# babybirdprd/dia-tts-prune

Hardware: AMD Instinct MI355X
Metric: audio-codec frames/sec (Dia-1.6B decode, whole job) (higher is better)
Workload: dtype bf16; 1 GPU; Dia-1.6B bf16 weights, bf16 K/V, batch 1, 1890 decode steps, text bytes [98], cfg 3.0 / T 1.3 / top-p 0.95 / top-k 35, hipGraph=True; batch_per_gpu=1, parallelism=single

## Files before the change

dia-tts-prune_amd/csrc/attn.hip:

```cpp
#include "common.hpp"
#include "../../include/dia_hip.h"
#include "errors.hpp"
#include "launch.hpp"
#include "tuning.hpp"
#include <cstdlib>

namespace {

constexpr int HD = 128;
constexpr int NT = 256;
constexpr int NWV = NT / 64;
constexpr int U = 4;
constexpr int UNIT = NWV * 16;
constexpr int CHUNK = 128;
constexpr int SLAB = 2 * 8 + 4 * HD;

struct AttnK {
  int mode, n_kv_heads, n_rows, kv_cap;
  const float* q; int ldq, q_off, k_off, v_off;
  void* kc; void* vc;
  const int* cur; const int* len; int enc_len;
  const float* cos_t; const float* sin_t;
  bf16_raw* P; long p_plane_stride; int p_ktiles;
  float* scratch; int* tickets; int max_chunks;
  const int* head_map;
  int v_blocked;
  int gpw;
  int act_f32;
  long kv_plane_stride;
};

#ifdef DIA_DBG_STAMPS
__device__ long long g_astamps[8192 * 8];
#define ASTAMP(i) do { if (threadIdx.x == 0) g_astamps[((blockIdx.z * gridDim.y + blockIdx.y) * gridDim.x + blockIdx.x) * 8 + (i)] = wall_clock64(); } while (0)
#else
#define ASTAMP(i) do {} while (0)
#endif

template <int G>
__device__ __forceinline__ void attn_finish(const AttnK& p, const float* part, const float* pm_s, const float* pl_s,
                                            int* last_s_ptr, int tid, int qrow, int kvh, int head_row, int chunk, int nchunks) {
  int& last_s = *last_s_ptr;
  const bool o_thread = tid < G * 16;
  const int og = tid >> 4, od0 = (tid & 15) * 8;
  float o[8];
  float M = 0.f, Lsum = 1.f;
  if (o_thread) {
    float mm = -INFINITY;
#pragma unroll
    for (int ww = 0; ww < NWV; ++ww) mm = fmaxf(mm, pm_s[ww * 8 + og]);
    float L2 = 0.f;
#pragma unroll
    for (int j = 0; j < 8; ++j) o[j] = 0.f;
#pragma unroll
    for (int ww = 0; ww < NWV; ++ww) {
      const float pmw = pm_s[ww * 8 + og];
      const float f = (pmw == -INFINITY) ? 0.f : expf(pmw - mm);
      L2 += pl_s[ww * 8 + og] * f;
#pragma unroll
      for (int j = 0; j < 8; ++j) o[j] += part[(ww * G + og) * HD + od0 + j] * f;
    }
    M = mm; Lsum = L2;
  }

  if (nchunks > 1) {
    const long pair = (long)head_row * p.n_kv_heads + kvh;
    float* slab = p.scratch + (pair * p.max_chunks + chunk) * SLAB;
    if (o_thread) {
      if ((tid & 15) == 0) st2_agent(slab + 2 * og, M, Lsum);
      const __amdgpu_buffer_rsrc_t sr = agent_rsrc(p.scratch);
      const int so = (int)(((pair * p.max_chunks + chunk) * SLAB + 16 + og * HD + od0) * 4);
      st4_agent(sr, so, f32x4{o[0], o[1], o[2], o[3]});
      st4_agent(sr, so + 16, f32x4{o[4], o[5], o[6], o[7]});
    }
    asm volatile("s_waitcnt vmcnt(0)" ::: "memory");
    __syncthreads();
    if (tid == 0) {
      const int ticket = __hip_atomic_fetch_add(p.tickets + pair, 1, __ATOMIC_RELAXED, __HIP_MEMORY_SCOPE_AGENT);
      const int last = ticket == nchunks - 1;
      if (last) __hip_atomic_store(p.tickets + pair, 0, __ATOMIC_RELAXED, __HIP_MEMORY_SCOPE_AGENT);
      last_s = last;
    }
    __syncthreads();
    ASTAMP(5);
    if (!last_s) return;
    if (o_thread) {
      const float* base = p.scratch + pair * p.max_chunks * SLAB;
      const __amdgpu_buffer_rsrc_t sr = agent_rsrc(p.scratch);
      const int bo = (int)((pair * p.max_chunks * SLAB + 16 + og * HD + od0) * 4);
      constexpr int MB = 12;
      float mrun = -INFINITY, L2 = 0.f;
#pragma unroll
      for (int j = 0; j < 8; ++j) o[j] = 0.f;
      for (int c0 = 0; c0 < nchunks; c0 += MB) {
        float2 ml[MB]; f32x4 oa[MB], ob[MB];
#pragma unroll
        for (int u = 0; u < MB; ++u)
          if (c0 + u < nchunks) {
            const float* sl = base + (long)(c0 + u) * SLAB;
            ml[u] = ld2_agent(sl + 2 * og);
            oa[u] = ld4_agent(sr, bo + (c0 + u) * (SLAB * 4));
            ob[u] = ld4_agent(sr, bo + (c0 + u) * (SLAB * 4) + 16);
          }
        float mm = mrun;
#pragma unroll
        for (int u = 0; u < MB; ++u)
          if (c0 + u < nchunks) mm = fmaxf(mm, ml[u].x);
        const float fr = (mrun == -INFINITY) ? 0.f : expf(mrun - mm);
        L2 *= fr;
#pragma unroll
        for (int j = 0; j < 8; ++j) o[j] *= fr;
#pragma unroll
        for (int u = 0; u < MB; ++u)
          if (c0 + u < nchunks) {
            const float f = (ml[u].x != -INFINITY) ? expf(ml[u].x - mm) : 0.f;
            L2 += ml[u].y * f;
#pragma unroll
            for (int j = 0; j < 4; ++j) { o[j] += oa[u][j] * f; o[4 + j] += ob[u][j] * f; }
          }
        mrun = mm;
      }
      Lsum = L2;
    }
  }

  if (o_thread) {
    const float invl = Lsum > 0.f ? 1.0f / Lsum : 0.f;
#pragma unroll
    for (int j = 0; j < 8; ++j) o[j] *= invl;
    const int hpos = p.head_map ? p.head_map[kvh * G + og] : kvh * G + og;
    const int col = hpos * HD + od0;
    auto emit = [&](int row, const float* v8) {
      if (p.act_f32) emit_f32x8(reinterpret_cast<float*>(p.P), p.p_ktiles, row, col, v8);
      else emit_planes8(p.P, p.p_plane_stride, p.p_ktiles, row, col, v8);
    };
    if (hpos >= 0) emit(qrow, o);
    if (p.mode == DIA_ATTN_CROSS && hpos >= 0) {
      const float z[8] = {0.f, 0.f, 0.f, 0.f, 0.f, 0.f, 0.f, 0.f};
      emit(qrow - 1, z);
    }
  }
  ASTAMP(6);
}

template <typename KVT, int G>
__global__ __launch_bounds__(NT) void k_attn(AttnK p) {
  __shared__ __attribute__((aligned(16))) float q_s[G * HD];
  __shared__ float part[NWV * G * HD];
  __shared__ float pm_s[NWV * 8], pl_s[NWV * 8];
  __shared__ float knew_s[HD], vnew_s[HD];
  __shared__ int last_s;

  const int tid = threadIdx.x, lane = tid & 63, w = tid >> 6;
  const int kvh = blockIdx.x, chunk = blockIdx.z;
  const int by = blockIdx.y;
  const bool is_self = p.mode == DIA_ATTN_SELF, is_cross = p.mode == DIA_ATTN_CROSS;
  const int c_cur = p.cur[is_self ? (by >> 1) : (is_cross ? by : 0)];
  const int c_len = p.len[is_cross ? by : 0];
  const int qrow = is_cross ? 2 * by + 1 : by;
  const int kvrow = (is_self || is_cross) ? by : 0;
  const int pos = (is_self || is_cross) ? c_cur : by;
  const int nkeys = is_self ? c_cur : (is_cross ? c_len : p.enc_len);
  const int slot = is_self ? c_cur - 1 : -1;
  const int head_row = by;
  const int NZ = gridDim.z;
  const int nunits = max(1, (nkeys + UNIT - 1) / UNIT);
  if (chunk >= nunits) return;
  const int nchunks = min(NZ, nunits);
  if (p.head_map) {
    bool any_live = false;
#pragma unroll
    for (int g = 0; g < G; ++g) any_live |= p.head_map[kvh * G + g] >= 0;
    if (!any_live && !(p.mode == DIA_ATTN_SELF)) return;
  }

  KVT* Kc = reinterpret_cast<KVT*>(p.kc) + ((long)kvrow * p.n_kv_heads + kvh) * p.kv_cap * HD;
  KVT* Vc = reinterpret_cast<KVT*>(p.vc) + ((long)kvrow * p.n_kv_heads + kvh) * p.kv_cap * HD;
  const int gr = lane >> 4, sub = lane & 15;
  const int klast = max(nkeys - 1, 0);
  float kv[U][8], vv[U][8];
  auto load_unit = [&](int unit) {
    const int base = unit * UNIT + w * 16 + gr;
#pragma unroll
    for (int u = 0; u < U; ++u) KVElem<KVT>::load8(Kc + (long)min(base + u * 4, klast) * HD + sub * 8, kv[u]);
#pragma unroll
    for (int u = 0; u < U; ++u) KVElem<KVT>::load8(Vc + (long)min(base + u * 4, klast) * HD + sub * 8, vv[u]);
  };
  load_unit(chunk);

  const float* qr = p.q + (long)qrow * p.ldq;
  for (int t = tid; t < G * 64; t += NT) {
    const int g = t >> 6, d = t & 63;
    const float* qh = qr + p.q_off + (kvh * G + g) * HD;
    const float x1 = qh[d], x2 = qh[d + 64];
    const float c = p.cos_t[(long)pos * 64 + d], s = p.sin_t[(long)pos * 64 + d];
    q_s[g * HD + d] = x1 * c - x2 * s;
// ... 73 lines not shown
#pragma unroll
      for (int u = 0; u < U; ++u) { pu[u] = (sc[u] == -INFINITY) ? 0.f : __expf(sc[u] - mnew); ls += pu[u]; }
      lrun[g] = lrun[g] * alpha + ls;
      mrun[g] = mnew;
#pragma unroll
      for (int j = 0; j < 8; ++j) {
        float a = acc[g][j] * alpha;
#pragma unroll
        for (int u = 0; u < U; ++u) a += pu[u] * vv[u][j];
        acc[g][j] = a;
      }
    }
    if constexpr (PREFETCH) {
      if (nu < nunits) {
#pragma unroll
        for (int u = 0; u < U; ++u)
#pragma unroll
          for (int j = 0; j < 8; ++j) { kv[u][j] = kvn[u][j]; vv[u][j] = vvn[u][j]; }
      }
    }
  }

#pragma unroll
  for (int g = 0; g < G; ++g) {
    float mw = mrun[g];
    mw = fmaxf(mw, __shfl_xor(mw, 16, 64));
    mw = fmaxf(mw, __shfl_xor(mw, 32, 64));
    const float f = (mrun[g] == -INFINITY) ? 0.f : expf(mrun[g] - mw);
    float lw = lrun[g] * f;
    lw += __shfl_xor(lw, 16, 64);
    lw += __shfl_xor(lw, 32, 64);
#pragma unroll
    for (int j = 0; j < 8; ++j) {
      float a = acc[g][j] * f;
      a += __shfl_xor(a, 16, 64);
      a += __shfl_xor(a, 32, 64);
      acc[g][j] = a;
    }
    mrun[g] = mw; lrun[g] = lw;
  }
  if (lane < 16) {
#pragma unroll
    for (int g = 0; g < G; ++g) {
#pragma unroll
      for (int j = 0; j < 8; ++j) part[(w * G + g) * HD + sub * 8 + j] = acc[g][j];
      if (sub == 0) { pm_s[w * 8 + g] = mrun[g]; pl_s[w * 8 + g] = lrun[g]; }
    }
  }
  __syncthreads();

  attn_finish<G>(p, part, pm_s, pl_s, &last_s, tid, qrow, kvh, head_row, chunk, nchunks);
}

__device__ __forceinline__ float row16_max(float v) {
  v = fmaxf(v, __builtin_bit_cast(float, __builtin_amdgcn_update_dpp(0, __builtin_bit_cast(int, v), 0xB1, 0xF, 0xF, true)));
  v = fmaxf(v, __builtin_bit_cast(float, __builtin_amdgcn_update_dpp(0, __builtin_bit_cast(int, v), 0x4E, 0xF, 0xF, true)));
  v = fmaxf(v, __builtin_bit_cast(float, __builtin_amdgcn_update_dpp(0, __builtin_bit_cast(int, v), 0x141, 0xF, 0xF, true)));
  v = fmaxf(v, __builtin_bit_cast(float, __builtin_amdgcn_update_dpp(0, __builtin_bit_cast(int, v), 0x140, 0xF, 0xF, true)));
  return v;
}

#ifdef DIA_DBG_KV_NT
#define KVLOAD(ptr) __builtin_nontemporal_load(ptr)
#else
#define KVLOAD(ptr) (*(ptr))
#endif
template <int G, int PL>
struct MfmaFrag { bf16x8 kb[PL][2][4]; bf16x8 vb[PL][8]; };

template <int G, int PL = 1>
__global__ __launch_bounds__(NT, 2) void k_attn_mfma(AttnK p) {
  __shared__ __attribute__((aligned(16))) bf16_raw qf[4][DIA_NPLANES][G][4][8];
  __shared__ float part[NWV * G * HD];
  __shared__ float pm_s[NWV * 8], pl_s[NWV * 8];
  __shared__ __attribute__((aligned(16))) bf16_raw pbuf[NWV][2][16][32];
  __shared__ __attribute__((aligned(16))) bf16_raw knew_s[PL][HD], vnew_s[PL][HD];
  __shared__ int last_s;

  const int tid = threadIdx.x, lane = tid & 63, w = tid >> 6;
  const int kvh = blockIdx.x, chunk = blockIdx.z;
  const int arow = lane & 15, akq = lane >> 4;
  ASTAMP(0);
  const int by = blockIdx.y;
  const bool is_self = p.mode == DIA_ATTN_SELF;
  const int qrow = is_self ? by : 2 * by + 1;
  const float* qr = p.q + (long)qrow * p.ldq;
  const float* qh = qr + p.q_off + (kvh * G + min(w, G - 1)) * HD;
  const float* kh = qr + (is_self ? p.k_off : p.q_off) + kvh * HD;
  const float* vh = qr + (is_self ? p.v_off : p.q_off) + kvh * HD;
  const float qx1 = qh[lane], qx2 = qh[lane + 64];
  const float kx1 = kh[lane], kx2 = kh[lane + 64];
  const float vx1 = vh[lane], vx2 = vh[lane + 64];

  const int c_cur = p.cur[is_self ? (by >> 1) : by];
  const int c_len = p.len[is_self ? 0 : by];
  const int kvrow = by, pos = c_cur;
  const int nkeys = is_self ? c_cur : c_len;
  const int slot = is_self ? c_cur - 1 : -1;
  const int head_row = by;
  const int NZ = gridDim.z;
  const int ngran = (nkeys + 31) >> 5;
  const int gpw = (ngran <= 2 * NWV) ? max(p.gpw, 2) : p.gpw;
  const int nchunks = min(NZ, max(1, (ngran + NWV * gpw - 1) / (NWV * gpw)));
  if (chunk >= nchunks) return;
  ASTAMP(1);
  if (p.head_map) {
    bool any_live = false;
#pragma unroll
    for (int g = 0; g < G; ++g) any_live |= p.head_map[kvh * G + g] >= 0;
    if (!any_live && !is_self) return;
  }
  const float rc = p.cos_t[(long)pos * 64 + lane], rs = p.sin_t[(long)pos * 64 + lane];

  bf16_raw* Kc = reinterpret_cast<bf16_raw*>(p.kc) + ((long)kvrow * p.n_kv_heads + kvh) * p.kv_cap * HD;
  bf16_raw* Vc = reinterpret_cast<bf16_raw*>(p.vc) + ((long)kvrow * p.n_kv_heads + kvh) * p.kv_cap * HD;
  const int klast = max(nkeys - 1, 0);
  const int gstride = NWV * nchunks;
  const int g_first = chunk * NWV + w;
  auto load_gran = [&](MfmaFrag<G, PL>& f, int gi) {
    const int key0 = gi << 5;
#pragma unroll
    for (int pl = 0; pl < PL; ++pl) {
      const bf16_raw* Kp = Kc + pl * p.kv_plane_stride;
#pragma unroll
      for (int t = 0; t < 2; ++t)
#pragma unroll
        for (int ks = 0; ks < 4; ++ks)
          f.kb[pl][t][ks] = KVLOAD(reinterpret_cast<const bf16x8*>(Kp + (long)min(key0 + 16 * t + arow, klast) * HD + 32 * ks + 8 * akq));
    }
#pragma unroll
    for (int pl = 0; pl < PL; ++pl) {
      const bf16_raw* Vblk = Vc + pl * p.kv_plane_stride + (long)gi * HD * 32;
#pragma unroll
      for (int nb = 0; nb < 8; ++nb) f.vb[pl][nb] = KVLOAD(reinterpret_cast<const bf16x8*>(Vblk + (long)(16 * nb + arow) * 32 + 8 * akq));
    }
  };
  MfmaFrag<G, PL> fa, fb;
  const bool have0 = g_first < ngran;
  load_gran(fa, have0 ? g_first : 0);

  if (w < G) {
    const float qv[2] = {qx1 * rc - qx2 * rs, qx1 * rs + qx2 * rc};
#pragma unroll
    for (int e = 0; e < 2; ++e) {
      const int D = lane + 64 * e;
      __bf16 a, b, c;
      split3(qv[e], a, b, c);
      qf[D >> 5][0][w][(D >> 3) & 3][D & 7] = *reinterpret_cast<const bf16_raw*>(&a);
      qf[D >> 5][1][w][(D >> 3) & 3][D & 7] = *reinterpret_cast<const bf16_raw*>(&b);
      qf[D >> 5][2][w][(D >> 3) & 3][D & 7] = *reinterpret_cast<const bf16_raw*>(&c);
    }
  }
  const int gslot = slot >> 5;
  const bool owner = slot >= 0 && (gslot % gstride) == g_first;
  if (owner) {
    float kv4[4] = {kx1 * rc - kx2 * rs, kx1 * rs + kx2 * rc, vx1, vx2};
#pragma unroll
    for (int pl = 0; pl < PL; ++pl) {
      bf16_raw r4[4];
#pragma unroll
      for (int e = 0; e < 4; ++e) {
        const __bf16 b = (__bf16)kv4[e];
        r4[e] = *reinterpret_cast<const bf16_raw*>(&b);
        kv4[e] -= (float)b;
      }
      knew_s[pl][lane] = r4[0]; knew_s[pl][lane + 64] = r4[1]; vnew_s[pl][lane] = r4[2]; vnew_s[pl][lane + 64] = r4[3];
      bf16_raw* Kp = Kc + pl * p.kv_plane_stride;
      Kp[(long)slot * HD + lane] = r4[0]; Kp[(long)slot * HD + lane + 64] = r4[1];
      bf16_raw* vdst = Vc + pl * p.kv_plane_stride + (long)gslot * HD * 32 + (slot & 31);
      vdst[(long)lane * 32] = r4[2]; vdst[(long)(lane + 64) * 32] = r4[3];
    }
  }
  lds_barrier();
  ASTAMP(2);

  const int qrow_l = min(arow, G - 1);
  const float scale = 0.08838834764831845f;
  f32x4 O[8];
#pragma unroll
  for (int nb = 0; nb < 8; ++nb) O[nb] = f32x4{0.f, 0.f, 0.f, 0.f};
  float mrun[4], lrun[4];
#pragma unroll
  for (int g = 0; g < 4; ++g) { mrun[g] = -INFINITY; lrun[g] = 0.f; }

  auto consume = [&](MfmaFrag<G, PL>& f, int gi) {
    const int key0 = gi << 5;
    if (owner && gi == gslot) {
      const int ts = (slot >> 4) & 1, ns = slot & 15, js = slot & 7, kqs = (slot & 31) >> 3;
#pragma unroll
      for (int pl = 0; pl < PL; ++pl) {
#pragma unroll
        for (int ks = 0; ks < 4; ++ks) {
          const bf16x8 kn = *reinterpret_cast<const bf16x8*>(&knew_s[pl][32 * ks + 8 * akq]);
#pragma unroll
          for (int t = 0; t < 2; ++t)
            if (t == ts && arow == ns) f.kb[pl][t][ks] = kn;
        }
#pragma unroll
        for (int nb = 0; nb < 8; ++nb) {
          const bf16_raw vr = vnew_s[pl][16 * nb + arow];
          const __bf16 vn = *reinterpret_cast<const __bf16*>(&vr);
#pragma unroll
          for (int j = 0; j < 8; ++j)
            if (j == js && akq == kqs) f.vb[pl][nb][j] = vn;
        }
      }
    }
    f32x4 S[2] = {f32x4{0.f, 0.f, 0.f, 0.f}, f32x4{0.f, 0.f, 0.f, 0.f}};
#pragma unroll
    for (int ks = 0; ks < 4; ++ks)
#pragma unroll
      for (int pl = 0; pl < DIA_NPLANES; ++pl) {
        const bf16x8 qa = *reinterpret_cast<const bf16x8*>(&qf[ks][pl][qrow_l][akq][0]);
#pragma unroll
        for (int kp = 0; kp < PL; ++kp) {
          if (PL == 2 && (pl + kp > 1)) continue;
#pragma unroll
          for (int t = 0; t < 2; ++t)
            S[t] = __builtin_amdgcn_mfma_f32_16x16x32_bf16(qa, f.kb[kp][t][ks], S[t], 0, 0, 0);
        }
      }
    float alpha[4];
    const bool v0 = key0 + arow < nkeys, v1 = key0 + 16 + arow < nkeys;
#pragma unroll
    for (int g = 0; g < G; ++g) {
      const float s0 = v0 ? S[0][g] * scale : -INFINITY, s1 = v1 ? S[1][g] * scale : -INFINITY;
      const float mnew = fmaxf(mrun[g], row16_max(fmaxf(s0, s1)));
      alpha[g] = (mrun[g] == -INFINITY) ? 0.f : __expf(mrun[g] - mnew);
      const float p0 = (s0 == -INFINITY) ? 0.f : __expf(s0 - mnew), p1 = (s1 == -INFINITY) ? 0.f : __expf(s1 - mnew);
      lrun[g] = lrun[g] * alpha[g] + row16_sum(p0 + p1);
      mrun[g] = mnew;
      if (lane < 16) {
        const __bf16 h0 = (__bf16)p0, h1 = (__bf16)p1;
        const __bf16 l0 = (__bf16)(p0 - (float)h0), l1 = (__bf16)(p1 - (float)h1);
        pbuf[w][0][g][lane] = *reinterpret_cast<const bf16_raw*>(&h0);
        pbuf[w][0][g][16 + lane] = *reinterpret_cast<const bf16_raw*>(&h1);
        pbuf[w][1][g][lane] = *reinterpret_cast<const bf16_raw*>(&l0);
        pbuf[w][1][g][16 + lane] = *reinterpret_cast<const bf16_raw*>(&l1);
      }
    }
    __builtin_amdgcn_wave_barrier();
#pragma unroll
    for (int nb = 0; nb < 8; ++nb)
#pragma unroll
      for (int g = 0; g < G; ++g) O[nb][g] *= alpha[g];
    const bf16x8 pa0 = *reinterpret_cast<const bf16x8*>(&pbuf[w][0][arow][8 * akq]);
    const bf16x8 pa1 = *reinterpret_cast<const bf16x8*>(&pbuf[w][1][arow][8 * akq]);
#pragma unroll
    for (int nb = 0; nb < 8; ++nb)
#pragma unroll
      for (int vp = 0; vp < PL; ++vp) {
        O[nb] = __builtin_amdgcn_mfma_f32_16x16x32_bf16(pa0, f.vb[vp][nb], O[nb], 0, 0, 0);
        if (vp == 0) O[nb] = __builtin_amdgcn_mfma_f32_16x16x32_bf16(pa1, f.vb[vp][nb], O[nb], 0, 0, 0);
      }
    __builtin_amdgcn_wave_barrier();
  };

  if constexpr (PL == 1) {
    int gi = g_first;
    for (; gi + 2 * gstride < ngran; gi += 2 * gstride) {
      load_gran(fb, gi + gstride);
      consume(fa, gi);
      load_gran(fa, gi + 2 * gstride);
      consume(fb, gi + gstride);
    }
    if (gi < ngran) {
      const int g1 = gi + gstride;
      if (g1 < ngran) load_gran(fb, g1);
      consume(fa, gi);
      if (g1 < ngran) consume(fb, g1);
    }
  } else {
    for (int gi = g_first; gi < ngran; gi += gstride) {
      if (gi != g_first) load_gran(fa, gi);
      consume(fa, gi);
    }
  }
  ASTAMP(3);
  if (lane < 16) {
#pragma unroll
    for (int g = 0; g < G; ++g) {
#pragma unroll
      for (int nb = 0; nb < 8; ++nb) part[(w * G + g) * HD + 16 * nb + lane] = O[nb][g];
      if (lane == 0) { pm_s[w * 8 + g] = mrun[g]; pl_s[w * 8 + g] = lrun[g]; }
    }
  }
  __syncthreads();
  ASTAMP(4);
  attn_finish<G>(p, part, pm_s, pl_s, &last_s, tid, qrow, kvh, head_row, chunk, nchunks);
}

struct EncAttnK {
  const float* qkv; int ldq, q_off, k_off, v_off, heads, rows;
  const int* row_b; const int* seg_off; const int* seg_len;
  const float* cos_t; const float* sin_t;
  bf16_raw* kp; bf16_raw* vp;
  bf16_raw* P; long p_plane_stride; int p_ktiles;
};

__global__ __launch_bounds__(256) void k_enc_kv_planes(EncAttnK p) {
  const int h = blockIdx.x, blk = blockIdx.y, tid = threadIdx.x;
  const long plane = (long)p.heads * p.rows * HD;
  bf16_raw* kp = p.kp + ((long)h * p.rows + blk * 32) * HD;
  bf16_raw* vp = p.vp + ((long)h * (p.rows >> 5) + blk) * HD * 32;
  const int r = tid >> 3, d0 = (tid & 7) * 8, m = blk * 32 + r;
  const float* kr = p.qkv + (long)m * p.ldq + p.k_off + h * HD + d0;
  const float4 xa0 = *reinterpret_cast<const float4*>(kr), xa1 = *reinterpret_cast<const float4*>(kr + 4);
  const float4 xb0 = *reinterpret_cast<const float4*>(kr + 64), xb1 = *reinterpret_cast<const float4*>(kr + 68);
  float vv[2][8];
  int4 vb[2][2];
#pragma unroll
  for (int j = 0; j < 2; ++j) {
    const int it = tid + 256 * j, d = it >> 2, r0 = (it & 3) * 8;
    const float* vr = p.qkv + (long)(blk * 32 + r0) * p.ldq + p.v_off + h * HD + d;
#pragma unroll
    for (int e = 0; e < 8; ++e) vv[j][e] = vr[(long)e * p.ldq];
    vb[j][0] = *reinterpret_cast<const int4*>(p.row_b + blk * 32 + r0);
    vb[j][1] = *reinterpret_cast<const int4*>(p.row_b + blk * 32 + r0 + 4);
  }
  const int b = p.row_b[m];
  const int pos = b >= 0 ? m - p.seg_off[b] : 0;
  const float* ct = p.cos_t + (long)pos * 64 + d0;
  const float* st = p.sin_t + (long)pos * 64 + d0;
  const float4 c0 = *reinterpret_cast<const float4*>(ct), c1 = *reinterpret_cast<const float4*>(ct + 4);
  const float4 s0 = *reinterpret_cast<const float4*>(st), s1 = *reinterpret_cast<const float4*>(st + 4);
  {
    const float x1[8] = {xa0.x, xa0.y, xa0.z, xa0.w, xa1.x, xa1.y, xa1.z, xa1.w};
    const float x2[8] = {xb0.x, xb0.y, xb0.z, xb0.w, xb1.x, xb1.y, xb1.z, xb1.w};
    const float c[8] = {c0.x, c0.y, c0.z, c0.w, c1.x, c1.y, c1.z, c1.w};
    const float s[8] = {s0.x, s0.y, s0.z, s0.w, s1.x, s1.y, s1.z, s1.w};
    bf16x8 k1[3], k2[3];
#pragma unroll
    for (int e = 0; e < 8; ++e) {
      const float a1 = b >= 0 ? x1[e] * c[e] - x2[e] * s[e] : 0.f;
      const float a2 = b >= 0 ? x1[e] * s[e] + x2[e] * c[e] : 0.f;
      __bf16 u0, u1, u2;
      split3(a1, u0, u1, u2); k1[0][e] = u0; k1[1][e] = u1; k1[2][e] = u2;
      split3(a2, u0, u1, u2); k2[0][e] = u0; k2[1][e] = u1; k2[2][e] = u2;
    }
#pragma unroll
    for (int pl = 0; pl < 3; ++pl) {
      *reinterpret_cast<bf16x8*>(kp + pl * plane + (long)r * HD + d0) = k1[pl];
      *reinterpret_cast<bf16x8*>(kp + pl * plane + (long)r * HD + d0 + 64) = k2[pl];
// ... 163 lines not shown
  ko[d + 64] = x1 * s + x2 * c;
  vo[d] = vr[d];
  vo[d + 64] = vr[d + 64];
}

template <typename KVT, int G>
int launch_attn(const AttnK& k, int grid_y, int grid_z, hipStream_t st) {
  dia_launch<k_attn<KVT, G>>(dim3(k.n_kv_heads, grid_y, grid_z), dim3(NT), 0, st, k);
  return dia_check_launch("k_attn");
}

template <int G>
int launch_attn_mfma(const AttnK& k, int grid_y, int grid_z, hipStream_t st) {
  if (k.kv_plane_stride > 0) dia_launch<k_attn_mfma<G, 2>>(dim3(k.n_kv_heads, grid_y, grid_z), dim3(NT), 0, st, k);
  else dia_launch<k_attn_mfma<G, 1>>(dim3(k.n_kv_heads, grid_y, grid_z), dim3(NT), 0, st, k);
  return dia_check_launch("k_attn_mfma");
}

}

#ifdef DIA_DBG_STAMPS
extern "C" int dia_dbg_aclear() {
  static long long zeros[8192 * 8];
  return hipMemcpyToSymbol(HIP_SYMBOL(g_astamps), zeros, sizeof(zeros)) == hipSuccess ? 0 : -2;
}
extern "C" int dia_dbg_astamps(long long* host, int n) {
  return hipMemcpyFromSymbol(host, HIP_SYMBOL(g_astamps), sizeof(long long) * n) == hipSuccess ? 0 : -2;
}
#endif

extern "C" int dia_attn_scratch_floats(int n_rows, int n_kv_heads, int kv_cap) {
  const long chunks = (kv_cap + CHUNK - 1) / CHUNK;
  const long n = (long)n_rows * n_kv_heads * chunks * SLAB;
  return n > 0x7fffffffL ? -1 : (int)n;
}

extern "C" int dia_attn(const dia_attn_args* a, void* stream) {
  if (!a || !a->q || !a->kc || !a->vc || !a->P || !a->cos_t || !a->sin_t) return dia_fail(DIA_E_ARG, "dia_attn: null argument");
  if (a->n_rows <= 0 || a->n_kv_heads <= 0) return dia_fail(DIA_E_ARG, "dia_attn: empty problem");
  if (a->p_plane_stride % 8 != 0) return dia_fail(DIA_E_ARG, "dia_attn: plane stride must be a multiple of 8");
  if (a->mode == DIA_ATTN_ENC && (a->n_rows != a->enc_len || a->enc_len <= 0 || a->enc_len > a->kv_cap))
    return dia_fail(DIA_E_ARG, "dia_attn: ENC needs n_rows == enc_len and 0 < enc_len <= kv_cap");
  if (a->rope_rows > 0 && ((a->mode == DIA_ATTN_ENC && a->enc_len > a->rope_rows) || (a->mode == DIA_ATTN_SELF && a->kv_cap + 1 > a->rope_rows)))
    return dia_fail(DIA_E_ARG, "dia_attn: RoPE tables shorter than the positions this launch can reach");
  if (a->kv_cap <= 0) return dia_fail(DIA_E_ARG, "dia_attn: kv_cap must be positive");
  const int cap_keys = a->mode == DIA_ATTN_ENC ? a->enc_len : a->kv_cap;
  const int cap_chunks = (cap_keys + CHUNK - 1) / CHUNK;
  int max_chunks = (512 + a->n_rows * a->n_kv_heads - 1) / (a->n_rows * a->n_kv_heads);
  if (dia_tune(DIA_TUNE_ATTN_NZ) > 0) max_chunks = dia_tune(DIA_TUNE_ATTN_NZ);
  if (max_chunks > cap_chunks) max_chunks = cap_chunks;
  if (max_chunks < 1) max_chunks = 1;
  if (max_chunks > 1 && (!a->scratch || !a->tickets)) return dia_fail(DIA_E_ARG, "dia_attn: more than 128 keys possible: scratch and tickets are required");
  AttnK k;
  k.mode = a->mode; k.n_kv_heads = a->n_kv_heads; k.n_rows = a->n_rows; k.kv_cap = a->kv_cap;
  k.q = a->q; k.ldq = a->ldq; k.q_off = a->q_off; k.k_off = a->k_off; k.v_off = a->v_off;
  k.kc = a->kc; k.vc = a->vc; k.cur = a->cur; k.len = a->len; k.enc_len = a->enc_len;
  k.cos_t = a->cos_t; k.sin_t = a->sin_t;
  k.P = (bf16_raw*)a->P; k.p_plane_stride = a->p_plane_stride; k.p_ktiles = a->p_ktiles; k.act_f32 = a->act_f32;
  k.head_map = a->head_map; k.v_blocked = a->v_blocked;
  k.gpw = 1;
  { const int g = dia_tune(a->mode == DIA_ATTN_CROSS ? DIA_TUNE_ATTN_GPW_CROSS : DIA_TUNE_ATTN_GPW); if (g > 0) k.gpw = g; }
  if (!k.cur) k.cur = reinterpret_cast<const int*>(a->cos_t);
  if (!k.len) k.len = reinterpret_cast<const int*>(a->cos_t);
  k.scratch = a->scratch; k.tickets = a->tickets; k.max_chunks = (a->kv_cap + CHUNK - 1) / CHUNK;
  if ((a->n_kv_heads * a->group * 128 + 31) / 32 > a->p_ktiles) return dia_fail(DIA_E_ARG, "dia_attn: output planes too narrow");
  hipStream_t st = (hipStream_t)stream;
  const bool f32 = a->kv_dtype == DIA_KV_F32;
  k.kv_plane_stride = 0;
  if (a->kv_dtype == DIA_KV_BF16X2) {
    if (!a->v_blocked || a->kv_plane_stride <= 0 || a->kv_plane_stride % 8 != 0)
      return dia_fail(DIA_E_ARG, "dia_attn: two-plane bf16 K/V needs the blocked V layout and the plane stride of the caches");
    k.kv_plane_stride = a->kv_plane_stride;
  }
  if (a->v_blocked) {
    if (f32 || a->mode == DIA_ATTN_ENC || a->kv_cap % 32 != 0) return dia_fail(DIA_E_ARG, "dia_attn: v_blocked needs bf16 K/V, SELF/CROSS mode and kv_cap % 32 == 0");
    if (a->mode == DIA_ATTN_SELF && !a->cur) return dia_fail(DIA_E_ARG, "dia_attn: SELF needs cur");
    if (a->mode == DIA_ATTN_CROSS && (!a->cur || !a->len || a->group != 1)) return dia_fail(DIA_E_ARG, "dia_attn: CROSS needs cur, len and group 1");
    if (a->group == 4) return launch_attn_mfma<4>(k, a->n_rows, max_chunks, st);
    if (a->group == 2) return launch_attn_mfma<2>(k, a->n_rows, max_chunks, st);
    if (a->group == 1) return launch_attn_mfma<1>(k, a->n_rows, max_chunks, st);
    return dia_fail(DIA_E_ARG, "dia_attn: GQA group must be 1, 2 or 4");
  }
  switch (a->mode) {
    case DIA_ATTN_SELF:
      if (!a->cur) return dia_fail(DIA_E_ARG, "dia_attn: SELF needs cur");
      if (a->group == 4) return f32 ? launch_attn<float, 4>(k, a->n_rows, max_chunks, st) : launch_attn<bf16_raw, 4>(k, a->n_rows, max_chunks, st);
      if (a->group == 2) return f32 ? launch_attn<float, 2>(k, a->n_rows, max_chunks, st) : launch_attn<bf16_raw, 2>(k, a->n_rows, max_chunks, st);
      if (a->group == 1) return f32 ? launch_attn<float, 1>(k, a->n_rows, max_chunks, st) : launch_attn<bf16_raw, 1>(k, a->n_rows, max_chunks, st);
      return dia_fail(DIA_E_ARG, "dia_attn: GQA group must be 1, 2 or 4");
    case DIA_ATTN_CROSS:
      if (!a->cur || !a->len || a->group != 1) return dia_fail(DIA_E_ARG, "dia_attn: CROSS needs cur, len and group 1");
      return f32 ? launch_attn<float, 1>(k, a->n_rows, max_chunks, st) : launch_attn<bf16_raw, 1>(k, a->n_rows, max_chunks, st);
    case DIA_ATTN_ENC:
      if (a->group != 1 || a->enc_len <= 0 || a->enc_len > a->kv_cap || !f32) return dia_fail(DIA_E_ARG, "dia_attn: ENC needs group 1, fp32 scratch K/V, 0 < L <= cap");
      return launch_attn<float, 1>(k, a->n_rows, max_chunks, st);
    default:
      return dia_fail(DIA_E_ARG, "dia_attn: unknown mode");
  }
}

extern "C" int dia_enc_kv_prep(const float* qkv, int ldq, int k_off, int v_off, int heads, int L, int cap,
                               const float* cos_t, const float* sin_t, float* kc, float* vc, void* stream) {
  if (!qkv || !kc || !vc || !cos_t || !sin_t || heads <= 0 || L <= 0 || L > cap) return dia_fail(DIA_E_ARG, "dia_enc_kv_prep: bad argument");
  dia_launch<k_enc_kv_prep>(dim3(heads, L), dim3(64), 0, (hipStream_t)stream, qkv, ldq, k_off, v_off, heads, L, cap, cos_t, sin_t, kc, vc);
  return dia_check_launch("k_enc_kv_prep");
}

extern "C" int dia_enc_attn(const dia_enc_attn_args* a, void* stream) {
  if (!a || !a->qkv || !a->row_b || !a->seg_off || !a->seg_len || !a->cos_t || !a->sin_t || !a->kp || !a->vp || !a->P)
    return dia_fail(DIA_E_ARG, "dia_enc_attn: null argument");
  if (a->heads <= 0 || a->rows <= 0 || a->rows % 32 != 0) return dia_fail(DIA_E_ARG, "dia_enc_attn: rows must be a positive multiple of 32");
  if (a->p_plane_stride % 8 != 0 || (a->heads * 128 + 31) / 32 > a->p_ktiles) return dia_fail(DIA_E_ARG, "dia_enc_attn: output planes too narrow");
  if (a->ldq % 4 != 0 || a->k_off % 4 != 0 || a->v_off % 4 != 0 || ((uintptr_t)a->qkv & 15) || ((uintptr_t)a->row_b & 15) || ((uintptr_t)a->kp & 15) ||
      ((uintptr_t)a->vp & 15) || ((uintptr_t)a->cos_t & 15) || ((uintptr_t)a->sin_t & 15))
    return dia_fail(DIA_E_ARG, "dia_enc_attn: qkv / row_b / kp / vp / RoPE tables must be 16-byte aligned, ldq and the k / v offsets multiples of 4");
  EncAttnK k;
  k.qkv = a->qkv; k.ldq = a->ldq; k.q_off = a->q_off; k.k_off = a->k_off; k.v_off = a->v_off; k.heads = a->heads; k.rows = a->rows;
// ... 10 lines not shown
```

dia-tts-prune_amd/csrc/engine.hip:

```cpp
#include "common.hpp"
#include "../../include/dia_hip.h"
#include "errors.hpp"
#include "launch.hpp"
#include "tuning.hpp"
#include <cstdlib>
#include <vector>
#include <algorithm>
#include <utility>

struct dia_engine {
  dia_engine_desc d;
  std::vector<dia_dec_layer> layers;
  hipStream_t stream = nullptr;
  hipGraph_t graph = nullptr;
  hipGraphExec_t exec = nullptr;
  int launches = 0;
  bool seg = false;
  std::vector<const void*> seg_w;
  int mlp_fused = -1;
  std::vector<hipEvent_t> prof;
  int pf_lookahead = 0;
  bool pf_capturing = false;
  hipStream_t side = nullptr;
  std::vector<hipEvent_t> pf_ev;
  std::vector<std::pair<const void*, long>> pf_w;
};

int dia_prefetch_launch(const void* ptr, long nbytes, int nblocks, hipStream_t st);
static int ensure_sink();

static inline void mark(dia_engine* e, int i) {
  if (!e->prof.empty() && i + 1 < (int)e->prof.size()) (void)hipEventRecord(e->prof[i + 1], e->stream);
  if (e->pf_capturing) {
    const int j = i + e->pf_lookahead;
    if (j < (int)e->pf_w.size() && e->pf_w[j].first != nullptr) {
      (void)hipEventRecord(e->pf_ev[i], e->stream);
      (void)hipStreamWaitEvent(e->side, e->pf_ev[i], 0);
      const long bytes = e->pf_w[j].second;
      const int nb = (int)std::min<long>(512, std::max<long>(32, bytes / (256 * 16 * 8)));
      (void)dia_prefetch_launch(e->pf_w[j].first, bytes, nb, e->side);
    }
  }
}

constexpr int MXFP8_DEFAULT = 0x5070;
extern "C" int dia_mxfp8_classes(int rows) {
  if (rows <= 0 || rows > 16) return 0;
  const int knob = dia_tune(DIA_TUNE_MXFP8);
  const int mask = knob >= 0 ? knob : MXFP8_DEFAULT;
  return (rows <= 4 ? mask : mask >> 8) & 0x7f;
}

static int enqueue_step(dia_engine* e, bool with_sampler) {
  const dia_engine_desc& d = e->d;
  void* st = (void*)e->stream;
  const int R = 2 * d.B;
  const int xkt = d.D / 32;
  const int akt = (max(d.q_heads, d.cq_heads) * 128) / 32;
  const int hkt = d.F / 32;
  const long mt = d.rows_pad / 16;
  const long xs = mt * xkt * 512, as = mt * akt * 512, hs = mt * hkt * 512;
  const int nqkv = (d.q_heads + 2 * d.kv_heads) * 128;
  int n = 0, rc;
  const int F = d.act_f32 ? 1 : 0;
  const bool two_tiles = R > 16 && R <= 32 && d.sk_scratch && d.sk_tickets && d.sk_scratch_floats > 0;
  auto lend_scratch = [&](dia_gemm_args& g) {
    if (two_tiles) { g.sk_scratch = d.sk_scratch; g.sk_tickets = d.sk_tickets; g.sk_scratch_floats = d.sk_scratch_floats; }
  };

  const bool seg = e->seg;
  bool diag = (R <= 2 || (R <= 4 && d.F <= 4096)) && d.act_f32 && d.w_planes <= 1 && dia_tune(DIA_TUNE_WO_DIAG) == 1 && !seg;
  for (int l = 0; l < d.n_layer && diag; ++l) diag = e->layers[l].w_wo_diag != nullptr && e->layers[l].cmap_next == nullptr;
// ... 16 lines not shown
    g.W = wf8; g.w_format = DIA_W_MXFP8; g.nw = 0; g.spw = 0;
    g.sk = sk;
    if (sk == 1) { g.sk_scratch = nullptr; g.sk_tickets = nullptr; }
    else { g.sk_scratch = d.sk_scratch; g.sk_tickets = d.sk_tickets; }
  };
  for (int l = 0; l < d.n_layer; ++l) {
    const dia_dec_layer& L = e->layers[l];
    dia_gemm_args g = {};
    if (!seg || l == 0) {
    g.A = d.planes_x; g.a_plane_stride = xs; g.a_ktiles = xkt; g.M = R;
    g.W = L.w_qkv; g.KT = L.kt_qkv; g.nstrips = L.ns_qkv; g.epi = DIA_EPI_SCALE_STORE;
    g.ssq_in = d.ssq; g.ssq_in_n = l > 0 ? xn_wo : d.D / 16; g.ssq_ld = d.rows_pad; g.inv_d = 1.0f / d.D; g.eps = d.eps;
    g.out = d.qkv; g.ldo = nqkv; g.strip_map = L.smap_qkv;
    lend_scratch(g);
  g.act_f32 = F;
  g.w_planes = d.w_planes;
  sparse24(g, L.w_qkv_24);
  mxfp8(g, L.w_qkv_f8, 0);
  if ((rc = dia_gemm(&g, st))) return rc; mark(e, n++);
    }

    dia_attn_args a = {};
    a.mode = DIA_ATTN_SELF; a.kv_dtype = d.kv_dtype; a.n_kv_heads = d.kv_heads; a.group = d.q_heads / d.kv_heads;
    a.n_rows = R; a.kv_cap = d.T; a.q = d.qkv; a.ldq = nqkv; a.q_off = 0; a.k_off = d.q_heads * 128;
    a.v_off = (d.q_heads + d.kv_heads) * 128; a.kc = L.k_self; a.vc = L.v_self; a.cur = d.sample.cur;
    a.head_map = L.hmap_self; a.v_blocked = d.v_blocked; a.rope_rows = d.T + 1; a.kv_plane_stride = d.kv_plane_self;
    a.cos_t = d.cos_t; a.sin_t = d.sin_t; a.P = d.planes_a; a.p_plane_stride = as; a.p_ktiles = akt;
    a.scratch = d.attn_scratch; a.tickets = d.attn_tickets;
    a.act_f32 = F;
    if ((rc = dia_attn(&a, st))) return rc; mark(e, n++);

    g = {};
    g.A = d.planes_a; g.a_plane_stride = as; g.a_ktiles = akt; g.M = R;
    g.W = L.w_o; g.KT = L.kt_o; g.nstrips = L.ns_o; g.epi = DIA_EPI_RESID_EMIT;
    g.ssq_ld = d.rows_pad; g.out = d.x; g.ldo = d.D; g.gnext = L.g_ca; g.cmap = L.cmap_ca;
    g.P = d.planes_x; g.p_plane_stride = xs; g.p_ktiles = xkt; g.ssq_out = d.ssq;
    lend_scratch(g);
  g.act_f32 = 3 * F;
  g.w_planes = d.w_planes;
  sparse24(g, L.w_o_24);
  mxfp8(g, L.w_o_f8, 1);
  if ((rc = dia_gemm(&g, st))) return rc; mark(e, n++);

    g = {};
    g.A = d.planes_x; g.a_plane_stride = xs; g.a_ktiles = xkt; g.M = R;
    g.W = L.w_cq; g.KT = L.kt_cq; g.nstrips = L.ns_cq; g.epi = DIA_EPI_SCALE_STORE;
    g.ssq_in = d.ssq; g.ssq_in_n = d.D / 16; g.ssq_ld = d.rows_pad; g.inv_d = 1.0f / d.D; g.eps = d.eps;
    g.out = d.qc; g.ldo = d.cq_heads * 128; g.strip_map = L.smap_cq;
    lend_scratch(g);
  g.act_f32 = F;
  g.w_planes = d.w_planes;
  sparse24(g, L.w_cq_24);
  mxfp8(g, L.w_cq_f8, 2);
  if ((rc = dia_gemm(&g, st))) return rc; mark(e, n++);

    a = {};
    a.mode = DIA_ATTN_CROSS; a.kv_dtype = d.kv_dtype; a.n_kv_heads = d.cq_heads; a.group = 1;
    a.n_rows = d.B; a.kv_cap = d.S; a.q = d.qc; a.ldq = d.cq_heads * 128; a.q_off = 0;
    a.kc = L.k_cross; a.vc = L.v_cross; a.cur = d.sample.cur; a.len = d.text_len; a.head_map = L.hmap_cross; a.v_blocked = d.v_blocked;
    a.kv_plane_stride = d.kv_plane_cross;
    a.cos_t = d.cos_t; a.sin_t = d.sin_t; a.P = d.planes_a; a.p_plane_stride = as; a.p_ktiles = akt;
    a.scratch = d.attn_scratch; a.tickets = d.attn_tickets;
    a.act_f32 = F;
    if ((rc = dia_attn(&a, st))) return rc; mark(e, n++);

    if (seg) {
      dia_seg_args sa = {};
      sa.a_in = (const float*)d.planes_a; sa.a_ktiles = akt; sa.M = R; sa.W = e->seg_w[l];
      sa.has_qkv = l + 1 < d.n_layer; sa.nslots = dia_seg_slots(sa.has_qkv); sa.D = d.D; sa.F = d.F;
      sa.x = d.x; sa.ldx = d.D; sa.g_mlp = L.g_mlp; sa.g_next = (l + 1 < d.n_layer) ? e->layers[l + 1].g_sa : d.g_final;
      sa.qkv_out = d.qkv; sa.ldq = nqkv; sa.planes_x = (float*)d.planes_x; sa.xkt = xkt; sa.ssq = d.ssq; sa.ssq_ld = d.rows_pad;
      sa.eps = d.eps; sa.ws = d.seg_ws;
      if ((rc = dia_seg_mlp(&sa, st))) return rc; mark(e, n++);
      continue;
    }
    g = {};
    g.A = d.planes_a; g.a_plane_stride = as; g.a_ktiles = akt; g.M = R;
    g.W = L.w_co; g.KT = L.kt_co; g.nstrips = L.ns_co; g.epi = DIA_EPI_RESID_EMIT;
    g.ssq_ld = d.rows_pad; g.out = d.x; g.ldo = d.D; g.gnext = L.g_mlp; g.cmap = L.cmap_mlp;
    g.P = d.planes_x; g.p_plane_stride = xs; g.p_ktiles = xkt; g.ssq_out = d.ssq;
    lend_scratch(g);
  g.act_f32 = 3 * F;
  g.w_planes = d.w_planes;
  sparse24(g, L.w_co_24);
  mxfp8(g, L.w_co_f8, 3);
  if ((rc = dia_gemm(&g, st))) return rc; mark(e, n++);

    dia_gemm_args gi = {};
    gi.A = d.planes_x; gi.a_plane_stride = xs; gi.a_ktiles = xkt; gi.M = R;
    gi.W = L.w_wi; gi.KT = L.kt_wi; gi.nstrips = L.ns_wi; gi.epi = DIA_EPI_SWIGLU_EMIT;
    gi.ssq_in = d.ssq; gi.ssq_in_n = d.D / 16; gi.ssq_ld = d.rows_pad; gi.inv_d = 1.0f / d.D; gi.eps = d.eps;
    gi.P = d.planes_h; gi.p_plane_stride = hs; gi.p_ktiles = hkt;

    g = {};
    g.A = d.planes_h; g.a_plane_stride = hs; g.a_ktiles = hkt; g.M = R;
    g.W = L.w_wo; g.KT = L.kt_wo; g.nstrips = L.ns_wo; g.epi = DIA_EPI_RESID_EMIT;
    int wo_sk = (R <= 4 && L.kt_wo % 2 == 0) ? 2 : ((R <= 16 && L.kt_wo % 4 == 0) ? 4 : 1);
    int wo_spw = 0;
    if (R > 4 && R <= 16) {
      if (L.kt_wo % 64 == 0 && L.kt_wo / 64 >= 2 && L.kt_wo / 64 <= 8) wo_sk = L.kt_wo / 64;
      if (wo_sk > 1 && L.ns_wo * wo_sk >= 512 && L.ns_wo % 2 == 0) wo_spw = 2;
    }
    const int w2_sk = (d.w_planes == 2 && L.kt_wo % 128 == 0 && L.kt_wo / 128 <= 8) ? L.kt_wo / 128 : 1;
    if (d.w_planes == 2) { wo_sk = w2_sk; wo_spw = 0; }
    if (dia_tune(DIA_TUNE_WO_SK) >= 1 && dia_tune(DIA_TUNE_WO_SK) <= 8 && L.kt_wo % dia_tune(DIA_TUNE_WO_SK) == 0) wo_sk = dia_tune(DIA_TUNE_WO_SK);
    g.sk = wo_sk; g.sk_scratch = wo_sk > 1 ? d.sk_scratch : nullptr; g.sk_tickets = wo_sk > 1 ? d.sk_tickets : nullptr;
    bool wo_pair = false;
    if (R > 16 && R <= 128) {
      g.sk_scratch = d.sk_scratch; g.sk_tickets = d.sk_tickets;
      g.sk_scratch_floats = d.sk_scratch_floats > 0 ? d.sk_scratch_floats : (int64_t)(d.D / 16) * 4 * 512;
      wo_pair = L.kt_wo % 4 == 0 && g.sk_scratch_floats >= (int64_t)((R + 15) / 16) * L.ns_wo * 4 * 256 &&
                dia_tune(DIA_TUNE_WO_PAIR) != 0;
      g.sk = wo_pair ? 4 : 1;
      if (d.w_planes == 2) {
        wo_pair = w2_sk > 1 && g.sk_scratch_floats >= (int64_t)((R + 15) / 16) * L.ns_wo * w2_sk * 256;
        g.sk = wo_pair ? w2_sk : 1;
      }
// ... 38 lines not shown
  g.W = d.w_logits; g.KT = d.kt_logits; g.nstrips = d.ns_logits; g.epi = DIA_EPI_SCALE_STORE;
  g.ssq_in = d.ssq; g.ssq_in_n = xn_wo; g.ssq_ld = d.rows_pad; g.inv_d = 1.0f / d.D; g.eps = d.eps;
  g.out = d.logits; g.ldo = d.ld_logits;
  lend_scratch(g);
  g.act_f32 = F;
  g.w_planes = d.w_planes;
  sparse24(g, d.w_logits_24);
  mxfp8(g, d.w_logits_f8, 6);
  if ((rc = dia_gemm(&g, st))) return rc; mark(e, n++);
  if (with_sampler) {
    if ((rc = dia_sample(&d.sample, st))) return rc; mark(e, n++);
  }
  e->launches = n;
  return DIA_OK;
}

extern "C" int dia_engine_create(const dia_engine_desc* d, void* stream, dia_engine** out) {
  if (!d || !out || !d->layers) return dia_fail(DIA_E_ARG, "dia_engine_create: null argument");
  if (d->n_layer <= 0 || d->B <= 0) return dia_fail(DIA_E_ARG, "dia_engine_create: empty model");
  if (d->D % 32 != 0 || d->F % 32 != 0) return dia_fail(DIA_E_ARG, "dia_engine_create: D and F must be multiples of 32");
  if (d->rows_pad < 2 * d->B || d->rows_pad % 16 != 0) return dia_fail(DIA_E_ARG, "dia_engine_create: rows_pad must be 16*ceil(2B/16)");
  if (d->q_heads % d->kv_heads != 0) return dia_fail(DIA_E_ARG, "dia_engine_create: q_heads % kv_heads != 0");
  if (d->act_f32 && !d->sample.embed.act_f32)
    return dia_fail(DIA_E_ARG, "dia_engine_create: act_f32 needs an embedding that writes fp32 tiles too");
  if (!d->act_f32 && d->sample.embed.act_f32) return dia_fail(DIA_E_ARG, "dia_engine_create: the embedding writes fp32 tiles but the engine reads planes");
  if (!d->x || !d->planes_x || !d->planes_a || !d->planes_h || !d->ssq || !d->qkv || !d->qc || !d->logits || !d->cos_t ||
      !d->sin_t || !d->text_len || !d->w_logits || !d->g_final || !d->attn_scratch || !d->attn_tickets)
    return dia_fail(DIA_E_ARG, "dia_engine_create: missing buffer");
  dia_engine* e = new dia_engine();
  e->d = *d;
  e->layers.assign(d->layers, d->layers + d->n_layer);
  e->d.layers = e->layers.data();
  e->stream = (hipStream_t)stream;
  if (d->seg_w && d->seg_ws) {
    const int nqkv = (d->q_heads + 2 * d->kv_heads) * 128;
    if (2 * d->B > 4 || !d->act_f32 || d->w_planes > 1 || !dia_seg_supported(d->D, d->F, max(d->q_heads, d->cq_heads) * 128, nqkv) ||
        d->cq_heads * 128 != 2048) {
      delete e;
      return dia_fail(DIA_E_ARG, "dia_engine_create: persistent segments need <= 4 rows, fp32 activation tiles, one weight plane, Dia-1.6B decoder shapes and 256 CUs");
    }
    for (int l = 0; l < d->n_layer; ++l) {
      const dia_dec_layer& L = d->layers[l];
      if (!d->seg_w[l] || L.cmap_mlp || L.cmap_next || L.smap_qkv) { delete e; return dia_fail(DIA_E_ARG, "dia_engine_create: persistent segments take dense (uncompacted) layers only"); }
    }
    e->seg_w.assign(d->seg_w, d->seg_w + d->n_layer);
    e->d.seg_w = e->seg_w.data();
    e->seg = true;
  }
  e->mlp_fused = dia_tune(DIA_TUNE_MLP_FUSE) > 0 ? -1 : 0;
  *out = e;
  return DIA_OK;
}

extern "C" int dia_engine_destroy(dia_engine* e) {
  if (!e) return DIA_OK;
  hipError_t he = hipSuccess;
  if (e->stream) he = hipStreamSynchronize(e->stream);
  if (e->side) { hipError_t h2 = hipStreamSynchronize(e->side); if (he == hipSuccess) he = h2; }
  if (e->exec) (void)hipGraphExecDestroy(e->exec);
  if (e->graph) (void)hipGraphDestroy(e->graph);
  for (auto& ev : e->pf_ev) if (ev) (void)hipEventDestroy(ev);
  for (auto& ev : e->prof) if (ev) (void)hipEventDestroy(ev);
  if (e->side) (void)hipStreamDestroy(e->side);
  delete e;
  return he == hipSuccess ? DIA_OK : dia_fail_hip(he, "dia_engine_destroy: hipStreamSynchronize");
}

extern "C" int dia_engine_decode(dia_engine* e, int n_steps, int use_graph) {
  if (!e || n_steps < 0) return dia_fail(DIA_E_ARG, "dia_engine_decode: bad argument");
  if (!use_graph) {
    for (int i = 0; i < n_steps; ++i) {
      int rc = enqueue_step(e, true);
      if (rc) return rc;
    }
    return DIA_OK;
  }
  if (!e->exec) {
    if (e->stream == nullptr) return dia_fail(DIA_E_STATE, "dia_engine_decode: graph capture needs a non-default stream");
    if (e->pf_lookahead > 0) {
      int rc0 = ensure_sink();
      if (rc0) return rc0;
      const dia_engine_desc& d = e->d;
      e->pf_w.clear();
      for (int l = 0; l < d.n_layer; ++l) {
        const dia_dec_layer& L = e->layers[l];
        auto add = [&](const void* w, int kt, int ns) { e->pf_w.push_back({w, (long)kt * ns * 1024}); };
        add(L.w_qkv, L.kt_qkv, L.ns_qkv); e->pf_w.push_back({nullptr, 0});
        add(L.w_o, L.kt_o, L.ns_o); add(L.w_cq, L.kt_cq, L.ns_cq); e->pf_w.push_back({nullptr, 0});
        add(L.w_co, L.kt_co, L.ns_co); add(L.w_wi, L.kt_wi, L.ns_wi); add(L.w_wo, L.kt_wo, L.ns_wo);
      }
      e->pf_w.push_back({d.w_logits, (long)d.kt_logits * d.ns_logits * 1024});
      e->pf_w.push_back({nullptr, 0});
      if (!e->side && hipStreamCreateWithFlags(&e->side, hipStreamNonBlocking) != hipSuccess) return dia_fail(DIA_E_HIP, "hipStreamCreate(side)");
      e->pf_ev.assign(e->pf_w.size() + 2, nullptr);
      for (auto& ev : e->pf_ev)
        if (hipEventCreateWithFlags(&ev, hipEventDisableTiming) != hipSuccess) return dia_fail(DIA_E_HIP, "hipEventCreate(prefetch)");
    }
    hipError_t he = hipStreamBeginCapture(e->stream, hipStreamCaptureModeThreadLocal);
    if (he != hipSuccess) return dia_fail_hip(he, "hipStreamBeginCapture");
    if (e->pf_lookahead > 0) {
      (void)hipEventRecord(e->pf_ev[e->pf_w.size()], e->stream);
      (void)hipStreamWaitEvent(e->side, e->pf_ev[e->pf_w.size()], 0);
      e->pf_capturing = true;
    }
    int rc = enqueue_step(e, true);
    if (e->pf_lookahead > 0) {
      e->pf_capturing = false;
      (void)hipEventRecord(e->pf_ev[e->pf_w.size() + 1], e->side);
      (void)hipStreamWaitEvent(e->stream, e->pf_ev[e->pf_w.size() + 1], 0);
    }
    he = hipStreamEndCapture(e->stream, &e->graph);
    if (rc) return rc;
    if (he != hipSuccess) return dia_fail_hip(he, "hipStreamEndCapture");
    he = hipGraphInstantiate(&e->exec, e->graph, nullptr, nullptr, 0);
    if (he != hipSuccess) return dia_fail_hip(he, "hipGraphInstantiate");
  }
  for (int i = 0; i < n_steps; ++i) {
    hipError_t he = hipGraphLaunch(e->exec, e->stream);
    if (he != hipSuccess) return dia_fail_hip(he, "hipGraphLaunch");
  }
  return DIA_OK;
}

extern "C" int dia_engine_step_logits_only(dia_engine* e) {
  if (!e) return dia_fail(DIA_E_ARG, "dia_engine_step_logits_only: null engine");
  return enqueue_step(e, false);
}

__global__ void k_delay(long long ticks) {
  const long long t0 = wall_clock64();
  while (wall_clock64() - t0 < ticks) __builtin_amdgcn_s_sleep(32);
}

extern "C" int dia_engine_profile_step(dia_engine* e, float* ms, int cap) {
  if (!e || !ms) return dia_fail(DIA_E_ARG, "dia_engine_profile_step: null argument");
  const int n = dia_engine_launches_per_step(e);
  if (cap < n) return dia_fail(DIA_E_ARG, "dia_engine_profile_step: output array too small");
  e->prof.resize(n + 1);
  for (auto& ev : e->prof) {
    hipError_t he = hipEventCreate(&ev);
    if (he != hipSuccess) return dia_fail_hip(he, "hipEventCreate");
  }
  int rc = DIA_OK;
  dia_launch<k_delay>(dim3(1), dim3(64), 0, e->stream, 300000LL );
  (void)hipEventRecord(e->prof[0], e->stream);
  rc = enqueue_step(e, true);
  {
    hipError_t he = hipStreamSynchronize(e->stream);
    if (rc == DIA_OK && he != hipSuccess) rc = dia_fail_hip(he, "hipStreamSynchronize");
  }
  if (rc == DIA_OK)
    for (int i = 0; i < n; ++i)
      if (hipEventElapsedTime(&ms[i], e->prof[i], e->prof[i + 1]) != hipSuccess) { ms[i] = -1.f; (void)hipGetLastError(); }
  for (auto& ev : e->prof) (void)hipEventDestroy(ev);
  e->prof.clear();
  return rc;
}

extern "C" int dia_engine_time_step(dia_engine* e, float* ms, float* interval_ms, int cap) {
  if (!e || !ms) return dia_fail(DIA_E_ARG, "dia_engine_time_step: null argument");
  const int n = dia_engine_launches_per_step(e);
  if (cap < n) return dia_fail(DIA_E_ARG, "dia_engine_time_step: output array too small");
  dia_launch<k_delay>(dim3(1), dim3(64), 0, e->stream, 300000LL );
  dia_recorder_arm();
  int rc = enqueue_step(e, true);
  const int got = dia_recorder_collect(ms, cap, interval_ms);
  hipError_t he = hipStreamSynchronize(e->stream);
  if (rc != DIA_OK) return rc;
  if (he != hipSuccess) return dia_fail_hip(he, "dia_engine_time_step: hipStreamSynchronize");
  return got;
}

extern "C" const char* dia_timed_kernel_name(int i) { return dia_recorder_label(i); }

extern "C" int dia_engine_mlp_fused(const dia_engine* e) { return e && e->mlp_fused == 1; }

extern "C" int dia_engine_launches_per_step(const dia_engine* e) {
  if (!e) return dia_fail(DIA_E_ARG, "null engine");
  return e->seg ? e->d.n_layer * 5 + 3 : e->d.n_layer * 8 + 2;
}

__global__ __launch_bounds__(256) void k_prefetch(const uint4* __restrict__ p, long n16, unsigned* sink) {
  uint4 acc = {0, 0, 0, 0};
  const long stride = (long)gridDim.x * 256;
  long i = (long)blockIdx.x * 256 + threadIdx.x;
  for (; i + 3 * stride < n16; i += 4 * stride) {
    const uint4 a = p[i], b = p[i + stride], c = p[i + 2 * stride], d = p[i + 3 * stride];
    acc.x ^= a.x ^ b.x ^ c.x ^ d.x; acc.y ^= a.y ^ b.y ^ c.y ^ d.y;
    acc.z ^= a.z ^ b.z ^ c.z ^ d.z; acc.w ^= a.w ^ b.w ^ c.w ^ d.w;
  }
  for (; i < n16; i += stride) { const uint4 a = p[i]; acc.x ^= a.x; acc.y ^= a.y; acc.z ^= a.z; acc.w ^= a.w; }
  if ((acc.x ^ acc.y ^ acc.z ^ acc.w) == 0x9E3779B9u && sink) *sink = 1;
}

static unsigned* g_sink = nullptr;
static int ensure_sink() {
  if (!g_sink) {
    hipError_t e = hipMalloc(&g_sink, 4);
    if (e != hipSuccess) return dia_fail_hip(e, "hipMalloc(sink)");
  }
  return DIA_OK;
}

int dia_prefetch_launch(const void* ptr, long nbytes, int nblocks, hipStream_t st) {
  dia_launch<k_prefetch>(dim3(nblocks), dim3(256), 0, st, (const uint4*)ptr, (long)(nbytes / 16), g_sink);
  return dia_check_launch("k_prefetch");
}

extern "C" int dia_prefetch(const void* ptr, int64_t nbytes, int nblocks, void* stream) {
  if (!ptr || nbytes <= 0 || nblocks <= 0) return dia_fail(DIA_E_ARG, "dia_prefetch: bad argument");
  int rc = ensure_sink();
  if (rc) return rc;
  return dia_prefetch_launch(ptr, (long)nbytes, nblocks, (hipStream_t)stream);
}

extern "C" int dia_engine_set_prefetch(dia_engine* e, int lookahead) {
  if (!e || lookahead < 0) return dia_fail(DIA_E_ARG, "dia_engine_set_prefetch: bad argument");
  if (e->exec) return dia_fail(DIA_E_STATE, "dia_engine_set_prefetch: the step graph is already captured");
  e->pf_lookahead = lookahead;
  return DIA_OK;
}
```

dia-tts-prune_amd/csrc/gemm.hip:

```cpp
#include "gemm_common.hpp"
#include "gemm_experiments.hpp"

namespace {

template <int MT, int NW, int KPW>
__global__ __launch_bounds__(NW * 64) void k_gemm(GemmK p) {
  extern __shared__ __attribute__((aligned(16))) unsigned char smem_raw[];
  f32x4* red = reinterpret_cast<f32x4*>(smem_raw);
  float* tile = reinterpret_cast<float*>(smem_raw + sizeof(f32x4) * NW * MT * 64);
  float* inv_s = tile + MT * 16 * 17;

  const int tid = threadIdx.x, lane = tid & 63, w = tid >> 6;
  const int strip = blockIdx.x;
  const int mt0 = blockIdx.y * MT;
  const int kpw = (KPW > 0) ? KPW : (p.KT + NW - 1) / NW;
  const int kt0 = w * kpw;

  f32x4 acc[MT];
  long aoff[MT];
#pragma unroll
  for (int i = 0; i < MT; ++i) {
    acc[i] = f32x4{0.f, 0.f, 0.f, 0.f};
    const int mtile = min(mt0 + i, (p.M - 1) >> 4);
    const int rlast = min(15, p.M - 1 - mtile * 16);
    const int alane = (lane & 48) | min(lane & 15, rlast);
    aoff[i] = ((long)mtile * p.a_ktiles * 64 + alane) * 8;
  }

  const bf16x8* Wt = reinterpret_cast<const bf16x8*>(p.W) + ((long)strip * p.KT) * 64 + lane;
  const bf16x8 zero8 = {0, 0, 0, 0, 0, 0, 0, 0};

  const int e_mt = tid >> 5, e_r = (tid >> 1) & 15, half = tid & 1;
  const int m = (mt0 + e_mt) * 16 + e_r;
  const int n0 = strip * 16 + half * 8;
  const bool e_thread = tid < MT * 32;
  const bool live = e_thread && m < p.M;
  float xpre[8], gpre[8];

  if (p.w_planes > 1) {
    prefetch_epilogue<MT, NW * 64>(p, tid, mt0, m, n0, live, xpre, gpre, inv_s);
    const int kt1 = min(kt0 + kpw, p.KT);
    const int npw = p.w_planes == 2 ? 1 : p.w_planes, ash = p.w_planes == 2 ? 1 : 0;
    for (int pw = 0; pw < npw; ++pw) {
      const bf16x8* Wp = Wt + pw * (p.w_plane_stride / 8);
      for (int kt = kt0; kt < kt1; ++kt) {
        const bf16x8 bb = DIA_WLOAD(Wp + (long)kt * 64);
#pragma unroll
        for (int mt = 0; mt < MT; ++mt) {
          bf16x8 a3[DIA_NPLANES];
          load_afrag3(p, aoff[mt] + (long)(kt >> ash) * 512, a3[0], a3[1], a3[2]);
#pragma unroll
          for (int pl = 0; pl < DIA_NPLANES; ++pl)
            acc[mt] = __builtin_amdgcn_mfma_f32_16x16x32_bf16(a3[pl], bb, acc[mt], 0, 0, 0);
        }
// ... 2 lines not shown
  } else if constexpr (KPW > 0) {
    bf16x8 b[KPW];
#pragma unroll
    for (int i = 0; i < KPW; ++i) b[i] = DIA_WLOAD(Wt + (long)(kt0 + i) * 64);
    __builtin_amdgcn_sched_barrier(0);
    constexpr int AP = (KPW >= 8) ? 1 : ((KPW * MT <= 4) ? KPW : ((4 / MT) > 0 ? (4 / MT) : 1));
    bf16x8 a0[AP][MT][DIA_NPLANES];
#pragma unroll
    for (int i = 0; i < AP; ++i)
#pragma unroll
      for (int mt = 0; mt < MT; ++mt)
        load_afrag3(p, aoff[mt] + (long)(kt0 + i) * 512, a0[i][mt][0], a0[i][mt][1], a0[i][mt][2]);
    prefetch_epilogue<MT, NW * 64>(p, tid, mt0, m, n0, live, xpre, gpre, inv_s);
#pragma unroll
    for (int i = 0; i < KPW; ++i) {
#pragma unroll
      for (int mt = 0; mt < MT; ++mt) {
        bf16x8 a3[DIA_NPLANES];
        if (i < AP) { a3[0] = a0[i < AP ? i : 0][mt][0]; a3[1] = a0[i < AP ? i : 0][mt][1]; a3[2] = a0[i < AP ? i : 0][mt][2]; }
        else load_afrag3(p, aoff[mt] + (long)(kt0 + i) * 512, a3[0], a3[1], a3[2]);
#pragma unroll
        for (int pl = 0; pl < DIA_NPLANES; ++pl)
          acc[mt] = __builtin_amdgcn_mfma_f32_16x16x32_bf16(a3[pl], b[i], acc[mt], 0, 0, 0);
      }
    }
  } else {
    prefetch_epilogue<MT, NW * 64>(p, tid, mt0, m, n0, live, xpre, gpre, inv_s);
    const int kt1 = min(kt0 + kpw, p.KT);
    for (int kt = kt0; kt < kt1; kt += 4) {
      bf16x8 b[4];
#pragma unroll
      for (int i = 0; i < 4; ++i) b[i] = (kt + i < kt1) ? DIA_WLOAD(Wt + (long)(kt + i) * 64) : zero8;
#pragma unroll
      for (int i = 0; i < 4; ++i) {
        if (kt + i < kt1) {
#pragma unroll
          for (int mt = 0; mt < MT; ++mt) {
            bf16x8 a3[DIA_NPLANES];
            load_afrag3(p, aoff[mt] + (long)(kt + i) * 512, a3[0], a3[1], a3[2]);
#pragma unroll
            for (int pl = 0; pl < DIA_NPLANES; ++pl)
              acc[mt] = __builtin_amdgcn_mfma_f32_16x16x32_bf16(a3[pl], b[i], acc[mt], 0, 0, 0);
          }
        }
      }
    }
  }

  reduce_to_tile<MT, NW>(acc, red, tile, tid, lane, w);
  if (!e_thread) return;
  run_epilogue(p, tile + (e_mt * 16 + e_r) * 17, inv_s[e_mt * 16 + e_r], m, n0, half, strip, live, xpre, gpre);
}


template <int NW, int KPW, int RS, bool MULTI, bool AF32 = false, bool PF32 = false, bool W2 = false>
__global__ __launch_bounds__(NW * 64) void k_gemv_small(const bf16_raw* a_A, long a_aps, const bf16_raw* a_W, int a_KT, int a_M, int a_epi,
                                                        int a_nstrips, float* a_out, int a_ldo, const float* a_gnext, GemmK p) {
  p.A = a_A; p.a_plane_stride = a_aps; p.W = a_W; p.KT = a_KT; p.M = a_M; p.epi = a_epi; p.nstrips = a_nstrips;
  p.out = a_out; p.ldo = a_ldo; p.gnext = a_gnext;
  extern __shared__ __attribute__((aligned(16))) unsigned char smem_raw[];
  f32x4* red = reinterpret_cast<f32x4*>(smem_raw);
  float* tile = reinterpret_cast<float*>(smem_raw + sizeof(f32x4) * NW * 64);
  float* inv_s = tile + 16 * 17;
  bf16x8* As = reinterpret_cast<bf16x8*>(smem_raw + sizeof(f32x4) * NW * 64 + sizeof(float) * (16 * 17 + 16));

  const int tid = threadIdx.x, lane = tid & 63, w = tid >> 6;
  const int kt0 = w * KPW;
  const int ktg = blockIdx.y * (NW * KPW);
  constexpr int WS = W2 ? 1 : 0;
  const int ktga = ktg >> WS;
  const int G = gridDim.x;
  const bf16x8* Wl = reinterpret_cast<const bf16x8*>(p.W) + (long)(ktg + kt0) * 64 + lane;
  auto load_strip = [&](bf16x8* b, int strip) {
    const bf16x8* Wt = Wl + (long)strip * p.KT * 64;
#pragma unroll
    for (int i = 0; i < KPW; ++i) b[i] = DIA_WLOAD(Wt + (long)i * 64);
  };
  __shared__ int sk_flag;

  STAMP(0);
  bf16x8 b0[KPW], b1[MULTI ? KPW : 1];
  constexpr int KT = (NW * KPW) >> WS;
  constexpr int KPA = KPW >> WS;
  static_assert(!W2 || KPW % 2 == 0, "two-plane weights: whole activation k-tiles per wave");
  constexpr int NT = NW * 64;
#ifdef DIA_X_WFIRST
  load_strip(b0, blockIdx.x);
  __builtin_amdgcn_sched_barrier(0);
#endif

  constexpr int CH = (3 * KPA * RS + 15) / 16;
  constexpr int nchunks = DIA_NPLANES * KT * 4 * RS;
  constexpr int nentries = KT * 4 * RS;
  constexpr int CE = (KPA * RS + 15) / 16;
  bf16x8 v0[AF32 ? 1 : CH];
  float4 ex[AF32 ? CE : 1], ey[AF32 ? CE : 1];
  if constexpr (AF32) {
    const float* Af = reinterpret_cast<const float*>(p.A);
#pragma unroll
    for (int u = 0; u < CE; ++u) {
      const int c = min(tid + u * NT, nentries - 1);
      const int row = c % RS, kq = (c / RS) & 3, kt = c / (4 * RS);
      const float4* src = reinterpret_cast<const float4*>(Af + ((long)(ktga + kt) * 64 + row + 16 * kq) * 8);
      ex[u] = src[0]; ey[u] = src[1];
    }
  } else {
#pragma unroll
    for (int u = 0; u < CH; ++u) {
      const int c = min(tid + u * NT, nchunks - 1);
      const int row = c % RS, kq = (c / RS) & 3, kt = (c / (4 * RS)) % KT, pl = c / (4 * RS * KT);
      v0[u] = *reinterpret_cast<const bf16x8*>(p.A + pl * p.a_plane_stride + ((long)(ktga + kt) * 64 + row + 16 * kq) * 8);
    }
  }
  const bool has_norm = p.ssq_in != nullptr;
  const int s_row = tid >> 3, s_part = tid & 7;
  const bool s_thread = tid < 128 && has_norm;
  float sq[16];
#pragma unroll
  for (int i = 0; i < 16; ++i) sq[i] = 0.f;
  if (s_thread) {
    const float* sp = p.ssq_in + min(s_row, p.M - 1);
#pragma unroll
    for (int i = 0; i < 16; ++i) sq[i] = sp[(long)min(s_part + 8 * i, p.ssq_in_n - 1) * p.ssq_ld];
  }
  const bool resid = p.epi == DIA_EPI_RESID_EMIT;
  const bool r_thread = tid < 16 * RS;
  float xpre1 = 0.f, gpre1 = 1.f;
  auto load_resid = [&](int strip) {
    const int r_m = tid >> 4, n = strip * 16 + (tid & 15);
    xpre1 = p.out[(long)(r_m < p.M ? r_m : 0) * p.ldo + n];
    gpre1 = p.gnext[n];
  };
  if (resid && r_thread) load_resid(blockIdx.x);
  __builtin_amdgcn_sched_barrier(0);
#ifndef DIA_X_WFIRST
  load_strip(b0, blockIdx.x);
  __builtin_amdgcn_sched_barrier(0);
#endif
  STAMP(1);
  if constexpr (AF32) {
#pragma unroll
    for (int u = 0; u < CE; ++u)
      if (tid + u * NT < nentries) {
        const int c = tid + u * NT;
        bf16x8 h, mi, lo;
        split3x8(ex[u], ey[u], h, mi, lo);
        As[c] = h; As[nentries + c] = mi; As[2 * nentries + c] = lo;
      }
  } else {
#pragma unroll
    for (int u = 0; u < CH; ++u)
      if (tid + u * NT < nchunks) As[tid + u * NT] = v0[u];
  }
  {
    float s0 = 0.f;
#pragma unroll
    for (int i = 0; i < 16; ++i) s0 += (s_part + 8 * i < p.ssq_in_n && s_row < p.M) ? sq[i] : 0.f;
    if (s_thread && s_row < p.M)
      for (int idx = s_part + 128; idx < p.ssq_in_n; idx += 8) s0 += p.ssq_in[(long)idx * p.ssq_ld + s_row];
    s0 += __builtin_bit_cast(float, __builtin_amdgcn_update_dpp(0, __builtin_bit_cast(int, s0), 0xB1, 0xF, 0xF, true));
    s0 += __builtin_bit_cast(float, __builtin_amdgcn_update_dpp(0, __builtin_bit_cast(int, s0), 0x4E, 0xF, 0xF, true));
    s0 += __builtin_bit_cast(float, __builtin_amdgcn_update_dpp(0, __builtin_bit_cast(int, s0), 0x141, 0xF, 0xF, true));
    if (tid < 128 && s_part == 0) inv_s[s_row] = has_norm ? rsqrtf(s0 * p.inv_d + p.eps) : 1.0f;
  }
  lds_barrier();
  STAMP(2);

  const int arow = min(lane & 15, RS - 1), akq = lane >> 4;
  f32x4* red16 = red;
  int sbuf = 0;
  auto body = [&](bf16x8* bc, bf16x8* bn, int strip) {
    const int next = strip + G;
    if constexpr (MULTI) load_strip(bn, DIA_PREFETCH_CLAMP(next, p.nstrips));
#ifdef DIA_PIN_PREFETCH
    if constexpr (MULTI) __builtin_amdgcn_sched_barrier(0);
#endif
    f32x4 acc[1] = {f32x4{0.f, 0.f, 0.f, 0.f}};
#pragma unroll
    for (int i = 0; i < KPW; ++i) {
#pragma unroll
      for (int pl = 0; pl < DIA_NPLANES; ++pl) {
        const bf16x8 a = As[((pl * KT + ((kt0 + i) >> WS)) * 4 + akq) * RS + arow];
        acc[0] = __builtin_amdgcn_mfma_f32_16x16x32_bf16(a, bc[i], acc[0], 0, 0, 0);
      }
    }
    STAMP(3);
    float v = 0.f;
    if (MULTI || gridDim.y == 1) {
      f32x4* rb = red16 + sbuf * (NW * 16);
      sbuf ^= 1;
      if (lane < 16) rb[w * 16 + lane] = acc[0];
      lds_barrier();
      if (r_thread) {
        const float* rf = reinterpret_cast<const float*>(rb) + (tid & 15) * 4 + (tid >> 4);
        v = rf[0];
#pragma unroll
        for (int ww = 1; ww < NW; ++ww) v += rf[ww * 64];
      }
      STAMP(4);
    } else {
      reduce_to_tile<1, NW, true>(acc, red, tile, tid, lane, w);
      STAMP(4);
      if (!splitk_combine(p, tile, strip, tid, &sk_flag)) return;
      if (r_thread) v = tile[(tid >> 4) * 17 + (tid & 15)];
    }
    if (r_thread) {
      run_epilogue_rows<RS, PF32>(p, v, inv_s, tid, strip, xpre1, gpre1);
      if (MULTI && next < p.nstrips && resid) load_resid(next);
    }
  };
  if constexpr (MULTI) {
    int strip = blockIdx.x;
    for (; strip + G < p.nstrips; strip += 2 * G) {
      body(b0, b1, strip);
      body(b1, b0, strip + G);
    }
    if (strip < p.nstrips) body(b0, b1, strip);
  } else {
    body(b0, b1, blockIdx.x);
  }
  STAMP(5);
}


#ifndef DIA_Z_TEMPORAL
#define DIA_Z_TEMPORAL 1
#endif
constexpr bool ZTEMPORAL = DIA_Z_TEMPORAL != 0;
#ifndef DIA_ZR_RING3
#define DIA_ZR_RING3 0
#endif
constexpr size_t g16_smem(int nw) { return sizeof(f32x4) * 2 * nw * 64 + 1536 + sizeof(float) * (2 * 16 * 17 + 16); }
constexpr size_t g16_alds(int nw, int kpw) { return (size_t)2 * nw * kpw * 64 * 16; }
template <int NW, int KPW, bool MULTI, bool MZ = false, bool AF32 = false, bool PF32 = false, bool PAIR = false, bool ALDS = false, bool W2 = false>
__global__ __launch_bounds__(NW * 64) void k_gemm16(const bf16_raw* a_A, long a_aps, const bf16_raw* a_W, int a_KT, int a_M, int a_epi,
                                                    int a_nstrips, float* a_out, int a_ldo, const float* a_gnext, GemmK p) {
  p.A = a_A; p.a_plane_stride = a_aps; p.W = a_W; p.KT = a_KT; p.M = a_M; p.epi = a_epi; p.nstrips = a_nstrips;
  p.out = a_out; p.ldo = a_ldo; p.gnext = a_gnext;
  extern __shared__ __attribute__((aligned(16))) unsigned char smem_raw[];
  f32x4* red = reinterpret_cast<f32x4*>(smem_raw);
  bf16_raw* stg = reinterpret_cast<bf16_raw*>(smem_raw + sizeof(f32x4) * 2 * NW * 64);
  float* tile = reinterpret_cast<float*>(smem_raw + sizeof(f32x4) * 2 * NW * 64 + 1536);
  float* inv_s = tile + 16 * 17;
  constexpr int NT = NW * 64;

  int zrow0 = 0;
  if constexpr (MZ) {
    const int z = blockIdx.z;
    zrow0 = 16 * z;
    p.A += (long)z * p.a_ktiles * 512 * (AF32 ? 2 : 1);
    p.M = min(16, p.M - 16 * z);
    if (p.ssq_in) p.ssq_in += 16 * z;
    if (p.out) p.out += (long)16 * z * p.ldo;
    if (p.P) p.P += (long)z * p.p_ktiles * 512 * (PF32 ? 2 : 1);
    if (p.ssq_out) p.ssq_out += 16 * z;
    if (p.sk_scratch) { p.sk_scratch += (long)z * p.nstrips * gridDim.y * 256; p.sk_tickets += z * p.nstrips; }
  }
  const int tid = threadIdx.x, lane = tid & 63, w = tid >> 6;
  const int kt0 = blockIdx.y * (NW * KPW) + w * KPW;
  constexpr int WS = W2 ? 1 : 0;
  constexpr int KPA = KPW >> WS;
  static_assert(!W2 || KPW % 2 == 0, "two-plane weights: whole activation k-tiles per wave");
  const int kta0 = kt0 >> WS;
  const int G = gridDim.x;
  __shared__ int sk_flag;
  const bf16x8* Wl = reinterpret_cast<const bf16x8*>(p.W) + (long)kt0 * 64 + lane;
  auto load_strip = [&](bf16x8* b, int strip) {
    const bf16x8* Wt = Wl + (long)strip * p.KT * 64;
#pragma unroll
    for (int i = 0; i < KPW; ++i) b[i] = (MZ && ZTEMPORAL) ? *(Wt + (long)i * 64) : DIA_WLOAD(Wt + (long)i * 64);
// ... 1623 lines not shown
        else if (uni && a->epi == DIA_EPI_RESID_EMIT) launch_small_kernel<k_gemm2t<8, true, false, 8, false, DIA_EPI_RESID_EMIT>>(grid, blk, g2t_smem(8), st, k);
        else if (uni && a->epi == DIA_EPI_SWIGLU_EMIT) launch_small_kernel<k_gemm2t<8, true, false, 8, false, DIA_EPI_SWIGLU_EMIT>>(grid, blk, g2t_smem(8), st, k);
        else launch_small_kernel<k_gemm2t<8, true, false>>(grid, blk, g2t_smem(8), st, k);
      } else if (ktw == 64) {
        if (sk > 1 && sk <= 4 && a->epi == DIA_EPI_RESID_EMIT && a->gnext && !a->cmap && dia_tune(DIA_TUNE_GEMM_2T) != 6)
          launch_small_kernel<k_gemm2t<8, false, true, 8, false, -1, true>>(grid, blk, g2t_smem(8, 8, true), st, k);
        else if (sk > 1) launch_small_kernel<k_gemm2t<8, false, true>>(grid, blk, g2t_smem(8), st, k);
        else if (puni && a->epi == DIA_EPI_RESID_EMIT) launch_small_kernel<k_gemm2t<8, false, false, 8, false, DIA_EPI_RESID_EMIT>>(grid, blk, g2t_smem(8), st, k);
        else launch_small_kernel<k_gemm2t<8, false, false>>(grid, blk, g2t_smem(8), st, k);
      } else if (half && a->epi == DIA_EPI_CROSSKV && a->kv_dtype == DIA_KV_BF16 && a->kv_vblocked && !a->strip_map && dia_tune(DIA_TUNE_GEMM_2T) != 4) {
        launch_small_kernel<k_gemm2t<8, false, false, 4, true>>(grid, blk, g2t_smem(8, 4), st, k);
      } else if (half && puni && a->epi == DIA_EPI_SCALE_STORE) {
        launch_small_kernel<k_gemm2t<8, false, false, 4, false, DIA_EPI_SCALE_STORE>>(grid, blk, g2t_smem(8, 4), st, k);
      } else if (half && puni && a->epi == DIA_EPI_SWIGLU_EMIT) {
        launch_small_kernel<k_gemm2t<8, false, false, 4, false, DIA_EPI_SWIGLU_EMIT>>(grid, blk, g2t_smem(8, 4), st, k);
      } else if (half) {
        launch_small_kernel<k_gemm2t<8, false, false, 4>>(grid, blk, g2t_smem(8, 4), st, k);
      } else {
        launch_small_kernel<k_gemm2t<4, false, false>>(grid, blk, g2t_smem(4), st, k);
      }
      return dia_check_launch("k_gemm2t");
    }
  }
  const bool z_epi = fast_epi || a->epi == DIA_EPI_CROSSKV;
  if (mtiles >= 2 && mtiles <= mz_max && z_epi && nw16 && (sk == 1 || a->sk_scratch_floats >= (int64_t)mtiles * a->nstrips * sk * 256)) {
    bool handled = false;
    k.mz = mtiles;
    int rc = launch_g16_any(k, nw16, sk, st, handled);
    k.mz = 0;
    if (handled) return rc;
  }
#ifdef DIA_EXPERIMENTS
  if (mtiles == 2 && !a->act_f32) {
    bool handled = false;
    int rc = dia_exp_gemm_two_mtiles(a, stream, handled);
    if (handled) return rc;
  }
#endif
  if (sk > 1) return dia_fail(DIA_E_ARG, "dia_gemm: no split-K kernel for this shape");
  {
    const int blocks = ((mtiles + GT_MT - 1) / GT_MT) * ((a->nstrips + 15) / 16);
    const int min_blocks = dia_tune(DIA_TUNE_TILE_MIN_BLOCKS) >= 0 ? dia_tune(DIA_TUNE_TILE_MIN_BLOCKS) : 48;
    if (mtiles >= 3 && a->KT % 8 == 0 && blocks >= min_blocks && !a->act_f32) {
#ifdef DIA_EXPERIMENTS
      const int v = dia_tune(DIA_TUNE_TILE_V);
      if (v >= 0 && v <= 2) return dia_exp_tile_variant(a, stream, v);
#endif
      return launch_tile(k, st);
    }
  }
  return launch_generic(k, nw, st);
}

extern "C" int dia_gemm_timed(const dia_gemm_args* a, void* stream, float* ms_out) {
  if (!ms_out) return dia_fail(DIA_E_ARG, "dia_gemm_timed: null output");
  dia_recorder_arm();
  int rc = dia_gemm(a, stream);
  float ms[4] = {0.f, 0.f, 0.f, 0.f};
  const int n = dia_recorder_collect(ms, 4);
  if (rc != DIA_OK) return rc;
  if (n < 1) return n < 0 ? n : dia_fail(DIA_E_STATE, "dia_gemm_timed: nothing was launched");
  *ms_out = ms[0];
  return DIA_OK;
}

#ifndef DIA_EXPERIMENTS
extern "C" int dia_mlp_fused(const dia_gemm_args*, const dia_gemm_args*, int32_t*, void*) {
  return dia_fail(DIA_E_ARG, "dia_mlp_fused: experiment, needs a build with EXPERIMENTS=1");
}
extern "C" int dia_mlp_fused_timed(const dia_gemm_args*, const dia_gemm_args*, int32_t*, void*, float*) {
  return dia_fail(DIA_E_ARG, "dia_mlp_fused_timed: experiment, needs a build with EXPERIMENTS=1");
}
#endif
```

dia-tts-prune_amd/csrc/gemm_common.hpp:

```cpp
#pragma once
#include "common.hpp"
#include <type_traits>
#include "../../include/dia_hip.h"
#include "errors.hpp"
#include <hip/hip_ext.h>
#include <cstdlib>
#include <cstring>
#include "tuning.hpp"
#include "launch.hpp"

namespace {


#ifdef DIA_DBG_PLAIN_LOAD
#define DIA_WLOAD(ptr) (*(ptr))
#else
#define DIA_WLOAD(ptr) __builtin_nontemporal_load(ptr)
#endif

#ifdef DIA_DBG_COND_PREFETCH
#define DIA_PREFETCH_CLAMP(next, n) (next)
#else
#define DIA_PREFETCH_CLAMP(next, n) min((next), (n) - 1)
#endif
// ... 131 lines not shown
    float v[8];
#pragma unroll
    for (int j = 0; j < 8; ++j) {
      float g = trow[j] * inv, u = trow[8 + j] * inv;
      v[j] = (g / (1.0f + expf(-g))) * u;
    }
    emit_act8(p, m, strip * 8, v, nullptr);
  } else {
    if (!live) return;
    if (p.strip_map) strip = p.strip_map[strip];
    long lofs = 0;
    if (p.kv_layer_strips > 0) {
      const int layer = strip / p.kv_layer_strips;
      strip -= layer * p.kv_layer_strips;
      lofs = (long)layer * p.kv_layer_stride;
    }
    int kvb = p.kv_batch_index;
    if (p.row_b) {
      kvb = p.row_b[m];
      if (kvb < 0) return;
      m -= p.seg_off[kvb];
    }
    const int nk = p.kv_heads * 8;
    if (strip < nk) {
      const int head = strip >> 3, i0 = (strip & 7) * 8 + half * 4;
      const long base = lofs + (((long)kvb * p.kv_heads + head) * p.kv_cap + m) * 128;
#pragma unroll
      for (int t = 0; t < 4; ++t) {
        const int i = i0 + t;
        const float x1 = trow[half * 8 + 2 * t] * inv, x2 = trow[half * 8 + 2 * t + 1] * inv;
        const float c = pre_cs ? xpre[t] : p.cos_t[(long)m * 64 + i], s = pre_cs ? gpre[t] : p.sin_t[(long)m * 64 + i];
        kv_store(p.kc, p.kv_dtype, base + i, x1 * c - x2 * s, p.kv_plane_stride);
        kv_store(p.kc, p.kv_dtype, base + i + 64, x1 * s + x2 * c, p.kv_plane_stride);
      }
    } else {
      const int sv = strip - nk, head = sv >> 3, d0 = (sv & 7) * 16 + half * 8;
      if (p.kv_vblocked) {
        const long hb = lofs + ((long)kvb * p.kv_heads + head) * p.kv_cap * 128;
        const long blk = hb + (long)(m >> 5) * 128 * 32 + (m & 31);
#pragma unroll
        for (int j = 0; j < 8; ++j) kv_store(p.vc, p.kv_dtype, blk + (long)(d0 + j) * 32, trow[half * 8 + j] * inv, p.kv_plane_stride);
      } else {
        const long base = lofs + (((long)kvb * p.kv_heads + head) * p.kv_cap + m) * 128 + d0;
#pragma unroll
        for (int j = 0; j < 8; ++j) kv_store(p.vc, p.kv_dtype, base + j, trow[half * 8 + j] * inv, p.kv_plane_stride);
      }
    }
  }
}

#define DIA_ROW_SHR(v, n) __builtin_bit_cast(float, __builtin_amdgcn_update_dpp(0, __builtin_bit_cast(int, (v)), 0x110 + (n), 0xF, 0xF, true))
#define DIA_ROW_SHL(v, n) __builtin_bit_cast(float, __builtin_amdgcn_update_dpp(0, __builtin_bit_cast(int, (v)), 0x100 + (n), 0xF, 0xF, true))

template <int RS, bool PF32 = false>
__device__ __forceinline__ void run_epilogue_rows(const GemmK& p, float v_tile, const float* inv_s, int tid, int strip,
                                                  float xpre1, float gpre1) {
  const int m = tid >> 4, c = tid & 15;
  const bool live = m < p.M;
  if (p.epi == DIA_EPI_RESID_EMIT) {
    const int n = strip * 16 + c;
    const float v = xpre1 + v_tile;
    if (live) p.out[(long)m * p.ldo + n] = v;
    const float sq = mul_rn(v, v);
    float acc = sq;
#pragma unroll
    for (int j = 1; j < 8; ++j) {
      const float t = DIA_ROW_SHR(acc, 1);
      if ((c & 7) == j) acc = add_rn(t, sq);
    }
    const float h0 = DIA_ROW_SHR(acc, 8);
    if (live && c == 15) p.ssq_out[(long)strip * p.ssq_ld + m] = h0 + acc;
    const float vg = mul_rn(v, gpre1);
    int cc = n;
    if (p.cmap) cc = p.cmap[n];
    if (live && cc >= 0) {
      const long off = plane_frag_off(m, cc & ~7, p.p_ktiles) + (cc & 7);
      if constexpr (PF32) {
        reinterpret_cast<float*>(p.P)[off] = vg;
      } else {
        __bf16 a, b, d;
        split3(vg, a, b, d);
        p.P[off] = *reinterpret_cast<bf16_raw*>(&a);
        p.P[p.p_plane_stride + off] = *reinterpret_cast<bf16_raw*>(&b);
        p.P[2 * p.p_plane_stride + off] = *reinterpret_cast<bf16_raw*>(&d);
      }
    }
  } else if (p.epi == DIA_EPI_SWIGLU_EMIT) {
    const float up_raw = DIA_ROW_SHL(v_tile, 8);
    if (!live || c >= 8) return;
    const float inv = inv_s[m];
    const float g = v_tile * inv, u = up_raw * inv;
    const float v = (g / (1.0f + expf(-g))) * u;
    const long off = plane_frag_off(m, strip * 8, p.p_ktiles) + c;
    if constexpr (PF32) {
      reinterpret_cast<float*>(p.P)[off] = v;
    } else {
      __bf16 a, b, d;
      split3(v, a, b, d);
      p.P[off] = *reinterpret_cast<bf16_raw*>(&a);
      p.P[p.p_plane_stride + off] = *reinterpret_cast<bf16_raw*>(&b);
      p.P[2 * p.p_plane_stride + off] = *reinterpret_cast<bf16_raw*>(&d);
    }
  } else {
    if (!live) return;
    const int s_out = p.strip_map ? p.strip_map[strip] : strip;
    p.out[(long)m * p.ldo + s_out * 16 + c] = v_tile * inv_s[m];
  }
}

template <int MT, int NW, bool RAW = false>
__device__ __forceinline__ void reduce_to_tile(const f32x4* acc, f32x4* red, float* tile, int tid, int lane, int w) {
#pragma unroll
  for (int mt = 0; mt < MT; ++mt) red[(w * MT + mt) * 64 + lane] = acc[mt];
  if constexpr (RAW) lds_barrier(); else __syncthreads();
  if (tid < MT * 64) {
    const int mt = tid >> 6;
    f32x4 s = red[(0 * MT + mt) * 64 + lane];
#pragma unroll
    for (int ww = 1; ww < NW; ++ww) {
      f32x4 t = red[(ww * MT + mt) * 64 + lane];
      s[0] += t[0]; s[1] += t[1]; s[2] += t[2]; s[3] += t[3];
    }
    const int col = lane & 15, r0 = (lane >> 4) * 4;
#pragma unroll
    for (int r = 0; r < 4; ++r) tile[(mt * 16 + r0 + r) * 17 + col] = s[r];
  }
  if constexpr (RAW) lds_barrier(); else __syncthreads();
}

__device__ __forceinline__ bool splitk_combine(const GemmK& p, float* tile, int strip, int tid, int* flag_s) {
  const int SK = gridDim.y;
  if (SK == 1) return true;
  const int ks = blockIdx.y;
#ifdef DIA_X_NOHANDOFF
  return ks == SK - 1;
#endif
  const __amdgpu_buffer_rsrc_t sr = agent_rsrc(p.sk_scratch);
  const int row = tid >> 2, c4 = (tid & 3) * 4;
  if (tid < 64) {
    const float* t = tile + row * 17 + c4;
    st4_agent(sr, (int)((((long)strip * SK + ks) * 256 + row * 16 + c4) * 4), f32x4{t[0], t[1], t[2], t[3]});
  }
  asm volatile("s_waitcnt vmcnt(0)" ::: "memory");
  __syncthreads();
  if (tid == 0) {
    const int ticket = __hip_atomic_fetch_add(p.sk_tickets + strip, 1, __ATOMIC_RELAXED, __HIP_MEMORY_SCOPE_AGENT);
    const int last = ticket == SK - 1;
    if (last) __hip_atomic_store(p.sk_tickets + strip, 0, __ATOMIC_RELAXED, __HIP_MEMORY_SCOPE_AGENT);
    *flag_s = last;
  }
  __syncthreads();
  if (!*flag_s) return false;
  if (tid < 64) {
    f32x4 v[4];
#pragma unroll
    for (int k = 0; k < 4; ++k)
      if (k < SK) v[k] = ld4_agent(sr, (int)((((long)strip * SK + k) * 256 + row * 16 + c4) * 4));
    f32x4 a = {0.f, 0.f, 0.f, 0.f};
// ... 53 lines not shown
```

dia-tts-prune_amd/csrc/tuning.cpp:

```cpp
#include "tuning.hpp"
#include "errors.hpp"
#include "../../include/dia_hip.h"
#include <cstdio>
#include <cstdlib>
#include <cstring>
#include <string>

static const char* const k_names[DIA_TUNE_COUNT] = {
    "attn_nz", "attn_gpw", "attn_gpw_cross", "gemm_spw", "gemm_mz_max", "tile_min_blocks", "wo_sk", "wo_pair", "wo_nw", "wo_spw", "act_f32", "wo_diag", "gemm_2t", "gemm_zr", "seg", "seg_nb", "seg_dbg", "seg_sleep", "g2t_wgs", "ckv_merge", "mxfp8",
    "mlp_fuse", "tile_v", "blk32_kr", "blk32_ws", "no_g32", "g32_all", "g32m"};
static int g_tune[DIA_TUNE_COUNT] = {-1, -1, -1, -1, -1, -1, -1, -1, -1, -1, -1, -1, -1, -1, -1, -1, -1, -1, -1, -1, -1, -1, -1, -1, -1, -1, -1};

int dia_tune(int id) {
  dia_tuning_init_from_env();
  return (id >= 0 && id < DIA_TUNE_COUNT) ? g_tune[id] : -1;
}

extern "C" int dia_set_tuning(const char* name, int value) {
  if (!name) return dia_fail(DIA_E_ARG, "dia_set_tuning: null name");
  dia_tuning_init_from_env();
  for (int i = 0; i < DIA_TUNE_COUNT; ++i)
    if (strcmp(name, k_names[i]) == 0) { g_tune[i] = value < 0 ? -1 : value; return DIA_OK; }
  return dia_fail(DIA_E_ARG, "dia_set_tuning: unknown knob");
}

extern "C" int dia_get_tuning(const char* name) {
  if (!name) return -1;
  dia_tuning_init_from_env();
  for (int i = 0; i < DIA_TUNE_COUNT; ++i)
    if (strcmp(name, k_names[i]) == 0) return g_tune[i];
  return -1;
}

void dia_tuning_init_from_env() {
  static bool done = false;
  if (done) return;
  done = true;
  const char* e = getenv("DIA_TUNE");
  if (!e) return;
  std::string s(e);
  size_t pos = 0;
  while (pos < s.size()) {
    size_t end = s.find(',', pos);
    if (end == std::string::npos) end = s.size();
    const std::string item = s.substr(pos, end - pos);
    const size_t eq = item.find('=');
    if (eq == std::string::npos) {
      if (!item.empty()) fprintf(stderr, "dia_hip: DIA_TUNE item '%s' ignored (expected name=value)\n", item.c_str());
    } else if (dia_set_tuning(item.substr(0, eq).c_str(), atoi(item.c_str() + eq + 1)) != DIA_OK) {
      fprintf(stderr, "dia_hip: DIA_TUNE knob '%s' unknown, ignored\n", item.substr(0, eq).c_str());
    }
    pos = end + 1;
  }
}
```

dia-tts-prune_amd/csrc/tuning.hpp:

```cpp
#pragma once

enum dia_tune_id {
  DIA_TUNE_ATTN_NZ = 0,
  DIA_TUNE_ATTN_GPW,
  DIA_TUNE_ATTN_GPW_CROSS,
  DIA_TUNE_GEMM_SPW,
  DIA_TUNE_GEMM_MZ_MAX,
  DIA_TUNE_TILE_MIN_BLOCKS,
  DIA_TUNE_WO_SK,
  DIA_TUNE_WO_PAIR,
  DIA_TUNE_WO_NW,
  DIA_TUNE_WO_SPW,
  DIA_TUNE_ACT_F32,
  DIA_TUNE_WO_DIAG,
  DIA_TUNE_GEMM_2T,
  DIA_TUNE_GEMM_ZR,
  DIA_TUNE_SEG,
  DIA_TUNE_SEG_NB,
  DIA_TUNE_SEG_DBG,
  DIA_TUNE_SEG_SLEEP,
  DIA_TUNE_G2T_WGS,
  DIA_TUNE_CKV_MERGE,
  DIA_TUNE_MXFP8,
  DIA_TUNE_MLP_FUSE,
  DIA_TUNE_TILE_V,
  DIA_TUNE_BLK32_KR,
  DIA_TUNE_BLK32_WS,
  DIA_TUNE_NO_G32,
  DIA_TUNE_G32_ALL,
  DIA_TUNE_G32M,
  DIA_TUNE_COUNT
};

int dia_tune(int id);
void dia_tuning_init_from_env();
```

dia-tts-prune_amd/dia_hip/binding.py:

```python

from __future__ import annotations

import ctypes as C
import os
from typing import Optional

_HERE = os.path.dirname(os.path.abspath(__file__))
LIB_PATH = os.environ.get("DIA_HIP_LIB") or os.path.join(_HERE, "libdia_hip.so")

ABI_VERSION = 8
KV_F32, KV_BF16, KV_BF16X2 = 0, 1, 2
EPI_SCALE_STORE, EPI_RESID_EMIT, EPI_SWIGLU_EMIT, EPI_CROSSKV = 0, 1, 2, 3
W_DENSE, W_SPARSE24, W_MXFP8 = 0, 1, 2
ATTN_SELF, ATTN_CROSS, ATTN_ENC = 0, 1, 2

EXPORTS = (
    "dia_last_error", "dia_abi_version", "dia_device_count", "dia_set_tuning", "dia_get_tuning", "dia_has_experiments", "dia_gemm", "dia_gemm_timed", "dia_mlp_fused", "dia_mlp_fused_timed", "dia_engine_mlp_fused", "dia_attn", "dia_attn_scratch_floats", "dia_enc_kv_prep", "dia_enc_attn", "dia_dec_prefill_embed", "dia_dec_prefill_kv", "dia_dec_prefill_attn",
    "dia_embed_text", "dia_embed_tokens", "dia_sample", "dia_prefetch", "dia_engine_create", "dia_engine_destroy",
    "dia_engine_decode", "dia_engine_set_prefetch", "dia_engine_step_logits_only", "dia_engine_profile_step", "dia_engine_time_step", "dia_timed_kernel_name", "dia_engine_launches_per_step", "dia_mxfp8_classes",
    "dia_seg_mlp", "dia_seg_workspace_bytes", "dia_seg_workspace_control_bytes", "dia_seg_slots", "dia_seg_supported", "dia_seg_error",
)


class DiaHipError(RuntimeError):
    pass


class GemmArgs(C.Structure):
    _fields_ = [
        ("A", C.c_void_p), ("a_plane_stride", C.c_int64), ("a_ktiles", C.c_int32), ("M", C.c_int32),
        ("W", C.c_void_p), ("KT", C.c_int32), ("nstrips", C.c_int32), ("epi", C.c_int32), ("nw", C.c_int32),
        ("ssq_in", C.c_void_p), ("ssq_in_n", C.c_int32), ("ssq_ld", C.c_int32), ("inv_d", C.c_float), ("eps", C.c_float),
        ("out", C.c_void_p), ("ldo", C.c_int32), ("spw", C.c_int32),
        ("gnext", C.c_void_p), ("P", C.c_void_p), ("p_plane_stride", C.c_int64), ("p_ktiles", C.c_int32), ("_pad1", C.c_int32),
        ("ssq_out", C.c_void_p),
        ("kc", C.c_void_p), ("vc", C.c_void_p), ("kv_dtype", C.c_int32), ("kv_heads", C.c_int32), ("kv_cap", C.c_int32),
        ("kv_batch_index", C.c_int32), ("cos_t", C.c_void_p), ("sin_t", C.c_void_p),
        ("cmap", C.c_void_p), ("strip_map", C.c_void_p),
        ("sk_scratch", C.c_void_p), ("sk_tickets", C.c_void_p), ("sk", C.c_int32), ("kv_vblocked", C.c_int32),
        ("row_b", C.c_void_p), ("seg_off", C.c_void_p), ("sk_scratch_floats", C.c_int64),
        ("sp_blocks", C.c_void_p), ("sp_toff", C.c_void_p),
        ("act_f32", C.c_int32), ("w_planes", C.c_int32), ("kv_plane_stride", C.c_int64),
        ("w_layout", C.c_int32), ("kv_layer_strips", C.c_int32), ("kv_layer_stride", C.c_int64),
        ("w_format", C.c_int32), ("_pad2", C.c_int32),
    ]


class AttnArgs(C.Structure):
    _fields_ = [
        ("mode", C.c_int32), ("kv_dtype", C.c_int32), ("n_kv_heads", C.c_int32), ("group", C.c_int32),
        ("n_rows", C.c_int32), ("kv_cap", C.c_int32),
        ("q", C.c_void_p), ("ldq", C.c_int32), ("q_off", C.c_int32), ("k_off", C.c_int32), ("v_off", C.c_int32),
        ("kc", C.c_void_p), ("vc", C.c_void_p), ("cur", C.c_void_p), ("len", C.c_void_p),
        ("enc_len", C.c_int32), ("rope_rows", C.c_int32), ("cos_t", C.c_void_p), ("sin_t", C.c_void_p),
        ("P", C.c_void_p), ("p_plane_stride", C.c_int64), ("p_ktiles", C.c_int32), ("_pad1", C.c_int32),
        ("scratch", C.c_void_p), ("tickets", C.c_void_p), ("head_map", C.c_void_p),
        ("v_blocked", C.c_int32), ("act_f32", C.c_int32), ("kv_plane_stride", C.c_int64),
    ]


class EncAttnArgs(C.Structure):
    _fields_ = [
        ("qkv", C.c_void_p), ("ldq", C.c_int32), ("q_off", C.c_int32), ("k_off", C.c_int32), ("v_off", C.c_int32),
        ("heads", C.c_int32), ("rows", C.c_int32),
        ("row_b", C.c_void_p), ("seg_off", C.c_void_p), ("seg_len", C.c_void_p), ("cos_t", C.c_void_p), ("sin_t", C.c_void_p),
        ("kp", C.c_void_p), ("vp", C.c_void_p), ("P", C.c_void_p), ("p_plane_stride", C.c_int64), ("p_ktiles", C.c_int32),
        ("_pad0", C.c_int32),
    ]


class DecPrefillArgs(C.Structure):
    _fields_ = [
# ... 66 lines not shown
        ("act_f32", C.c_int32), ("w_planes", C.c_int32),
        ("sample", SampleArgs),
        ("seg_w", C.POINTER(C.c_void_p)), ("seg_ws", C.c_void_p),
        ("kv_plane_self", C.c_int64), ("kv_plane_cross", C.c_int64),
        ("w_logits_24", C.c_void_p), ("w_logits_f8", C.c_void_p),
    ]


class SegArgs(C.Structure):
    _fields_ = [
        ("a_in", C.c_void_p), ("a_ktiles", C.c_int32), ("M", C.c_int32),
        ("W", C.c_void_p), ("nslots", C.c_int32), ("has_qkv", C.c_int32), ("D", C.c_int32), ("F", C.c_int32),
        ("x", C.c_void_p), ("ldx", C.c_int32), ("_pad0", C.c_int32),
        ("g_mlp", C.c_void_p), ("g_next", C.c_void_p), ("qkv_out", C.c_void_p), ("ldq", C.c_int32), ("_pad1", C.c_int32),
        ("planes_x", C.c_void_p), ("xkt", C.c_int32), ("_pad2", C.c_int32), ("ssq", C.c_void_p), ("ssq_ld", C.c_int32), ("eps", C.c_float),
        ("ws", C.c_void_p), ("timeout_us", C.c_int32), ("_pad3", C.c_int32), ("stamps", C.c_void_p),
    ]


_lib: Optional[C.CDLL] = None


def lib() -> C.CDLL:
    global _lib
    if _lib is not None:
        return _lib
    if not os.path.isfile(LIB_PATH):
        raise DiaHipError(
            f"{LIB_PATH} is missing: build it with `python __graft_entry__.py` or "
            f"`make -C dia-tts-prune_amd/csrc` (hipcc --offload-arch=gfx950). There is no CPU fallback."
        )
    import torch

    try:
        L = C.CDLL(LIB_PATH)
    except OSError as e:
        raise DiaHipError(f"cannot load {LIB_PATH}: {e}") from e
    for name in EXPORTS:
        if not hasattr(L, name):
            raise DiaHipError(f"{LIB_PATH} does not export {name}; rebuild it")
    L.dia_last_error.restype = C.c_char_p
    L.dia_abi_version.restype = C.c_int
    if L.dia_abi_version() != ABI_VERSION:
        raise DiaHipError(f"ABI mismatch: library {L.dia_abi_version()} vs binding {ABI_VERSION}")
    L.dia_set_tuning.argtypes = [C.c_char_p, C.c_int]
    L.dia_get_tuning.argtypes = [C.c_char_p]
    L.dia_has_experiments.restype = C.c_int
    L.dia_gemm.argtypes = [C.POINTER(GemmArgs), C.c_void_p]
    L.dia_gemm_timed.argtypes = [C.POINTER(GemmArgs), C.c_void_p, C.POINTER(C.c_float)]
    L.dia_mlp_fused.argtypes = [C.POINTER(GemmArgs), C.POINTER(GemmArgs), C.c_void_p, C.c_void_p]
    L.dia_mlp_fused_timed.argtypes = [C.POINTER(GemmArgs), C.POINTER(GemmArgs), C.c_void_p, C.c_void_p, C.POINTER(C.c_float)]
    L.dia_engine_mlp_fused.argtypes = [C.c_void_p]
    L.dia_attn.argtypes = [C.POINTER(AttnArgs), C.c_void_p]
    L.dia_attn_scratch_floats.argtypes = [C.c_int, C.c_int, C.c_int]
    L.dia_enc_attn.argtypes = [C.POINTER(EncAttnArgs), C.c_void_p]
    for fn in (L.dia_dec_prefill_embed, L.dia_dec_prefill_kv, L.dia_dec_prefill_attn):
        fn.argtypes = [C.POINTER(DecPrefillArgs), C.c_void_p]
    L.dia_enc_kv_prep.argtypes = [C.c_void_p, C.c_int, C.c_int, C.c_int, C.c_int, C.c_int, C.c_int,
                                  C.c_void_p, C.c_void_p, C.c_void_p, C.c_void_p, C.c_void_p]
    L.dia_embed_text.argtypes = [C.c_void_p, C.c_int, C.c_void_p, C.c_int, C.c_void_p, C.c_void_p, C.c_void_p,
                                 C.c_int64, C.c_int, C.c_void_p, C.c_int, C.c_void_p, C.c_void_p]
    L.dia_embed_tokens.argtypes = [C.POINTER(EmbedArgs), C.c_void_p]
    L.dia_sample.argtypes = [C.POINTER(SampleArgs), C.c_void_p]
    L.dia_prefetch.argtypes = [C.c_void_p, C.c_int64, C.c_int, C.c_void_p]
    L.dia_engine_create.argtypes = [C.POINTER(EngineDesc), C.c_void_p, C.POINTER(C.c_void_p)]
    L.dia_engine_destroy.argtypes = [C.c_void_p]
    L.dia_engine_decode.argtypes = [C.c_void_p, C.c_int, C.c_int]
    L.dia_engine_step_logits_only.argtypes = [C.c_void_p]
    L.dia_engine_set_prefetch.argtypes = [C.c_void_p, C.c_int]
    L.dia_engine_launches_per_step.argtypes = [C.c_void_p]
    L.dia_engine_profile_step.argtypes = [C.c_void_p, C.POINTER(C.c_float), C.c_int]
    L.dia_engine_time_step.argtypes = [C.c_void_p, C.POINTER(C.c_float), C.POINTER(C.c_float), C.c_int]
    L.dia_timed_kernel_name.argtypes = [C.c_int]
    L.dia_timed_kernel_name.restype = C.c_char_p
    L.dia_mxfp8_classes.argtypes = [C.c_int]
    L.dia_seg_mlp.argtypes = [C.POINTER(SegArgs), C.c_void_p]
    L.dia_seg_workspace_bytes.restype = C.c_int64
    L.dia_seg_workspace_control_bytes.restype = C.c_int64
    L.dia_seg_slots.argtypes = [C.c_int]
    L.dia_seg_supported.argtypes = [C.c_int, C.c_int, C.c_int, C.c_int]
    L.dia_seg_error.argtypes = [C.c_void_p, C.c_void_p]
    _lib = L
    return L


def set_tuning(name: str, value: int) -> None:
    check(lib().dia_set_tuning(name.encode(), int(value)), f"dia_set_tuning({name})")


def get_tuning(name: str) -> int:
    return int(lib().dia_get_tuning(name.encode()))


def mxfp8_mask(rows: int) -> int:
    return int(lib().dia_mxfp8_classes(int(rows)))


def has_experiments() -> bool:
    return bool(lib().dia_has_experiments())


def check(rc: int, what: str = "") -> None:
    if rc != 0:
        msg = lib().dia_last_error()
        raise DiaHipError(f"{what} failed ({rc}): {msg.decode() if msg else ''}")

# ... 4 lines not shown
```

dia-tts-prune_amd/dia_hip/engine.py:

```python

from __future__ import annotations

import ctypes as C
from dataclasses import dataclass
from functools import partial
from typing import Dict, List, Optional, Sequence

import numpy as np
import torch

from . import binding as hb
from . import compact as cpt
from . import layout as lay
from .config import DiaConfig
from .pruning import is_2of4
from .quant import is_mxfp8

HEAD_DIM = 128
_TILERS = {1: lay.tile_weight, 2: lay.tile_weight_bf16x2, 3: lay.tile_weight_planes}


def _ceil(v: int, m: int) -> int:
    return (v + m - 1) // m * m

# ... 540 lines not shown
        return s

    def _build_engine(self):
        d = self.cfg.model.decoder
        w = self.w
        n = d.n_layer
        self._layers = (hb.DecLayer * n)()
        for i, L in enumerate(w.dec_layers):
            dl = self._layers[i]
            for f in DEC_MATS:
                setattr(dl, "w_" + f, hb.ptr(L[f].t))
                setattr(dl, "kt_" + f, L[f].kt)
                setattr(dl, "ns_" + f, L[f].ns)
                sp = L[f + "24"]
                setattr(dl, "w_" + f + "_24", hb.ptr(sp.t) if sp is not None else None)
                f8 = L[f + "f8"]
                setattr(dl, "w_" + f + "_f8", hb.ptr(f8.t) if f8 is not None else None)
            dl.g_sa, dl.g_ca, dl.g_mlp = hb.ptr(L["g_sa"]), hb.ptr(L["g_ca"]), hb.ptr(L["g_mlp"])
            dl.k_self, dl.v_self = hb.ptr(self.k_self[i]), hb.ptr(self.v_self[i])
            dl.k_cross, dl.v_cross = hb.ptr(self.k_cross[i]), hb.ptr(self.v_cross[i])
            for f in ("cmap_ca", "cmap_mlp", "cmap_next", "smap_qkv", "smap_cq", "hmap_self", "hmap_cross"):
                setattr(dl, f, hb.ptr(L[f]))
            dl.w_wo_diag = hb.ptr(L["wo_diag"])
        ed = hb.EngineDesc()
        ed.n_layer, ed.D, ed.F = n, self.D, self.F
        ed.q_heads, ed.kv_heads, ed.cq_heads = d.gqa_query_heads, d.kv_heads, d.cross_query_heads
        ed.C, ed.V, ed.B, ed.T, ed.S = self.C, self.V, self.B, self.T, self.S
        ed.kv_dtype, ed.rows_pad, ed.ld_logits = self.kv_code, self.rows_pad, self.ld_logits
        ed.v_blocked = self.v_blocked
        ed.kv_plane_self, ed.kv_plane_cross = self.kv_plane_self, self.kv_plane_cross
        ed.eps = float(self.cfg.model.normalization_layer_epsilon)
        ed.layers = C.cast(self._layers, C.POINTER(hb.DecLayer))
        ed.w_logits, ed.kt_logits, ed.ns_logits = hb.ptr(w.logits.t), w.logits.kt, w.logits.ns
        ed.w_logits_24 = hb.ptr(w.logits24.t) if w.logits24 is not None else None
        ed.w_logits_f8 = hb.ptr(w.logits_f8.t) if w.logits_f8 is not None else None
        ed.g_final = hb.ptr(w.dec_norm)
        ed.x, ed.planes_x, ed.planes_a, ed.planes_h = hb.ptr(self.x), hb.ptr(self.planes_x), hb.ptr(self.planes_a), hb.ptr(self.planes_h)
        ed.ssq, ed.qkv, ed.qc, ed.logits = hb.ptr(self.ssq), hb.ptr(self.qkv), hb.ptr(self.qc), hb.ptr(self.logits)
        ed.cos_t, ed.sin_t, ed.text_len = hb.ptr(w.cos_t), hb.ptr(w.sin_t), hb.ptr(self.text_len)
        ed.attn_scratch, ed.attn_tickets = hb.ptr(self.attn_scratch), hb.ptr(self.attn_tickets)
        ed.sk_scratch, ed.sk_tickets = hb.ptr(self.sk_scratch), hb.ptr(self.sk_tickets)
        ed.sk_scratch_floats = self.sk_scratch.numel()
        ed.mlp_barrier = hb.ptr(self.mlp_barrier)
        ed.act_f32 = self.act_f32
        ed.w_planes = w.weight_planes
        ed.sample = self._sample_args()
        if self.seg:
            self._seg_w = (C.c_void_p * n)(*[hb.ptr(t) for t in w.seg_layers])
            ed.seg_w = C.cast(self._seg_w, C.POINTER(C.c_void_p))
            ed.seg_ws = hb.ptr(self.seg_ws)
        self._desc = ed
        hb.check(hb.lib().dia_engine_create(C.byref(ed), C.c_void_p(self.stream.cuda_stream), C.byref(self._engine)),
                 "dia_engine_create")

    def close(self):
        if self._engine:
            eng, self._engine = self._engine, C.c_void_p()
            self.stream.synchronize()
            hb.check(hb.lib().dia_engine_destroy(eng), "dia_engine_destroy")

    def __del__(self):
        try:
            self.close()
        except Exception:
            pass

    def prefill(self, keep_encoder_out: bool = False):
        L = hb.lib()
        cfg, w, dev = self.cfg, self.w, self.dev
        e, d = cfg.model.encoder, cfg.model.decoder
        st = C.c_void_p(self.stream.cuda_stream)
        E, Fe = e.n_embd, e.n_hidden
        eps = float(cfg.model.normalization_layer_epsilon)
        offs, tot, row_utt = pack_segments(self.lens)
        self.enc_out = [None] * self.B
        with torch.cuda.stream(self.stream):
            if tot > 0:
                Mp, mt = tot, tot // 16
                Lmax = _ceil(max(self.lens), 16)
                Hmax = max(EL["heads"] for EL in w.enc_layers)
                ekt = E // 32
                akt = max(max(1, Hmax * HEAD_DIM // 32), max(EL["o"].a_kt for EL in w.enc_layers))
                hkt = max(EL["wo"].a_kt for EL in w.enc_layers)
                nq_max = 3 * Hmax * HEAD_DIM
                shapes = [((Mp, E), torch.float32), ((3, mt, ekt, 64, 8), torch.bfloat16), ((3, mt, akt, 64, 8), torch.bfloat16),
                          ((3, mt, hkt, 64, 8), torch.bfloat16), ((E // 16, Mp), torch.float32), ((Mp, nq_max), torch.float32),
                          ((3, Hmax, Mp, HEAD_DIM), torch.bfloat16), ((3, Hmax, Mp, HEAD_DIM), torch.bfloat16)]
                sizes = [_ceil(int(np.prod(sh)) * (4 if dt == torch.float32 else 2), 256) for sh, dt in shapes]
                ws = torch.zeros(sum(sizes), dtype=torch.uint8, device=dev)
                views, o_ = [], 0
                for (sh, dt), nb in zip(shapes, sizes):
                    n_el = int(np.prod(sh))
                    views.append(ws[o_: o_ + n_el * (4 if dt == torch.float32 else 2)].view(dt).view(*sh))
                    o_ += nb
                x, px, pa, ph, ssq, qkv, kp, vp = views
                live = [b for b in range(self.B) if self.lens[b] > 0]
                id_off, n_ids = {}, 0
                for b in live:
                    id_off[b] = n_ids
                    n_ids += _ceil(self.lens[b], 4)
                tab = np.zeros((Mp + 2 * _ceil(self.B, 4) + n_ids,), dtype=np.int32)
                tab[:Mp] = row_utt
                o_so, o_sl = Mp, Mp + _ceil(self.B, 4)
                tab[o_so: o_so + self.B] = offs
                tab[o_sl: o_sl + self.B] = self.lens
                o_id = Mp + 2 * _ceil(self.B, 4)
# ... 115 lines not shown
            a.P, a.p_plane_stride, a.p_ktiles = _plane_set(pa, akt)
            hb.check(L.dia_dec_prefill_kv(C.byref(a), st), "dia_dec_prefill_kv")
            hb.check(L.dia_dec_prefill_attn(C.byref(a), st), "dia_dec_prefill_attn(self)")
            gemm(pa, akt, DL["o"], hb.EPI_RESID_EMIT, out=x, ldo=D, gnext=DL["g_ca"], P=px, p_kt=xkt, ssq_out=True)
            gemm(px, xkt, DL["cq"], hb.EPI_SCALE_STORE, ssq_in=True, out=qc, ldo=CH * HEAD_DIM)
            a = pargs()
            a.q, a.ldq, a.q_off = hb.ptr(qc), CH * HEAD_DIM, 0
            a.q_heads, a.kv_heads, a.kv_cap, a.causal = CH, CH, self.S, 0
            a.kc, a.vc, a.text_len = hb.ptr(self.k_cross[i]), hb.ptr(self.v_cross[i]), hb.ptr(self.text_len)
            a.P, a.p_plane_stride, a.p_ktiles = _plane_set(pa, akt)
            hb.check(L.dia_dec_prefill_attn(C.byref(a), st), "dia_dec_prefill_attn(cross)")
            gemm(pa, akt, DL["co"], hb.EPI_RESID_EMIT, out=x, ldo=D, gnext=DL["g_mlp"], P=px, p_kt=xkt, ssq_out=True)
            gemm(px, xkt, DL["wi"], hb.EPI_SWIGLU_EMIT, ssq_in=True, P=ph, p_kt=hkt)
            gnext = w.dec_layers[i + 1]["g_sa"] if i + 1 < len(w.dec_layers) else w.dec_norm
            gemm(ph, hkt, DL["wo"], hb.EPI_RESID_EMIT, out=x, ldo=D, gnext=gnext, P=px, p_kt=xkt, ssq_out=True)
        cur = [fs if fs > 2 else 1 for fs in self.first_steps]
        self.cur.copy_(torch.tensor(cur, dtype=torch.int32))

    def ensure_noise(self, rows: int):
        rows = min(int(rows), self.noise_steps)
        if self._gens is None or rows <= self._noise_rows:
            return
        r0, n = self._noise_rows, rows - self._noise_rows

        def draw(b):
            t = torch.empty(n, self.C, self.V, dtype=torch.float32)
            t.exponential_(1.0, generator=self._gens[b])
            return t

        if self.B > 1:
            from concurrent.futures import ThreadPoolExecutor
            with ThreadPoolExecutor(max_workers=min(self.B, 8)) as pool:
                parts = list(pool.map(draw, range(self.B)))
        else:
            parts = [draw(0)]
        host = torch.stack(parts)
        with torch.cuda.stream(self.stream):
            self.noise[:, r0:rows].copy_(host, non_blocking=False)
        self._noise_rows = rows

    def decode(self, n_steps: int, use_graph: bool = True):
        if not self.prefilled:
            raise hb.DiaHipError("decode() before prefill()")
        self.ensure_noise(self._issued + int(n_steps))
        hb.check(hb.lib().dia_engine_decode(self._engine, int(n_steps), int(bool(use_graph))), "dia_engine_decode")
        self._issued += int(n_steps)

    def profile_step(self) -> np.ndarray:
        n = hb.lib().dia_engine_launches_per_step(self._engine)
        buf = (C.c_float * n)()
        self.ensure_noise(self._issued + 1)
        hb.check(hb.lib().dia_engine_profile_step(self._engine, buf, n), "dia_engine_profile_step")
        self._issued += 1
        return np.array(buf[:], dtype=np.float64)

    def launches_per_step(self) -> int:
        return int(hb.lib().dia_engine_launches_per_step(self._engine))

    def seg_error(self) -> int:
        if not self.seg:
            return 0
        return int(hb.lib().dia_seg_error(hb.ptr(self.seg_ws), C.c_void_p(self.stream.cuda_stream)))

    def time_step(self) -> np.ndarray:
        n = hb.lib().dia_engine_launches_per_step(self._engine)
        buf, ivl = (C.c_float * n)(), (C.c_float * n)()
        self.ensure_noise(self._issued + 1)
        got = hb.lib().dia_engine_time_step(self._engine, buf, ivl, n)
        if got < 0:
            hb.check(got, "dia_engine_time_step")
        self._issued += 1
        self.last_kernel_names = [hb.lib().dia_timed_kernel_name(i).decode() for i in range(got)]
        self.last_intervals_ms = np.array(ivl[:got], dtype=np.float64)
        return np.array(buf[:got], dtype=np.float64)

    def sync(self):
        self.stream.synchronize()

    def steps_total(self) -> int:
        return self.max_tokens - self.prefill_step

    def run(self, use_graph: bool = True, poll: int = 64):
        remaining = self.steps_total()
        first = True
        while remaining > 0:
            n = min(8 if first else poll, remaining)
            first = False
            self.decode(n, use_graph)
            remaining -= n
            self.ensure_noise(self._issued + min(poll, remaining))
            self.sync()
            if self.seg and self.seg_error():
                self.results()
            if bool((self.fsm[:, 3] != 0).all().item()):
                break

    def logits_host(self) -> np.ndarray:
        self.sync()
        lg = self.logits[: self.R, : self.C * self.V].reshape(self.B, 2, self.C, self.V)
        return lg.cpu().numpy()

    def results(self) -> List[UtteranceResult]:
        self.sync()
        if int(self.mlp_barrier[1].item()) != 0:
            raise hb.DiaHipError("fused MLP kernel: a workgroup gave up waiting at the grid barrier; results are invalid")
        code = self.seg_error()
        if code:
            self.seg_ws[: int(hb.lib().dia_seg_workspace_control_bytes())].zero_()
            raise hb.DiaHipError(f"persistent MLP segment: an in-kernel wait timed out (code {code}: 1 x1, 2 hidden, 3 wo partials, "
                                 f"4 x2) — were all 256 workgroups resident?  Results are invalid; set DIA_TUNE=seg=0 to run the launches")
        tok = self.tokens.cpu().numpy()
        prd = self.pred.cpu().numpy()
        fsm = self.fsm.cpu().numpy()
        cur = self.cur.cpu().numpy()
        out = []
        for b in range(self.B):
            last = int(fsm[b, 4]) if fsm[b, 3] else int(cur[b]) - 1
            out.append(UtteranceResult(tok[b], tok[b, self.first_steps[b]: last + 1].copy(), last, prd[b], self.lens[b]))
        return out

    def step_bytes(self, n_keys: Optional[int] = None) -> int:
        d = self.cfg.model.decoder
        kvb = 2 if self.kv_code == hb.KV_BF16 else 4
        if n_keys is None:
            n_keys = int(self.cur.max().item())
        kv_self = 2 * d.n_layer * 2 * d.kv_heads * HEAD_DIM * kvb * n_keys
        kv_cross = d.n_layer * 2 * d.cross_query_heads * HEAD_DIM * kvb
# ... 2 lines not shown
```

include/dia_hip.h:

```cpp
#ifndef DIA_HIP_H
#define DIA_HIP_H

#include <stdint.h>

#ifdef __cplusplus
extern "C" {
#endif

#define DIA_ABI_VERSION 8

#define DIA_OK 0
#define DIA_E_ARG (-1)
#define DIA_E_HIP (-2)
#define DIA_E_STATE (-3)

#define DIA_KV_F32 0
#define DIA_KV_BF16 1
#define DIA_KV_BF16X2 2

#define DIA_EPI_SCALE_STORE 0
#define DIA_EPI_RESID_EMIT 1
#define DIA_EPI_SWIGLU_EMIT 2
#define DIA_EPI_CROSSKV 3

// ... 54 lines not shown
  const int32_t* row_b;
  const int32_t* seg_off;
  int64_t sk_scratch_floats;
  const void* sp_blocks;
  const uint32_t* sp_toff;
  int32_t act_f32;
  int32_t w_planes;
  int64_t kv_plane_stride;
  int32_t w_layout;
  int32_t kv_layer_strips;
  int64_t kv_layer_stride;
  int32_t w_format;
  int32_t _pad2;
} dia_gemm_args;
int dia_gemm(const dia_gemm_args* a, void* stream);
int dia_mlp_fused(const dia_gemm_args* wi, const dia_gemm_args* wo, int32_t* barrier, void* stream);
int dia_mlp_fused_timed(const dia_gemm_args* wi, const dia_gemm_args* wo, int32_t* barrier, void* stream, float* ms_out);


int dia_gemm_timed(const dia_gemm_args* a, void* stream, float* ms_out);

typedef struct {
  int32_t mode;
  int32_t kv_dtype;
  int32_t n_kv_heads;
  int32_t group;
  int32_t n_rows;
  int32_t kv_cap;
  const float* q;
  int32_t ldq;
  int32_t q_off;
  int32_t k_off;
  int32_t v_off;
  void* kc;
  void* vc;
  const int32_t* cur;
  const int32_t* len;
  int32_t enc_len;
  int32_t rope_rows;
  const float* cos_t;
  const float* sin_t;
  void* P;
  int64_t p_plane_stride;
  int32_t p_ktiles;
  int32_t _pad1;
  float* scratch;
  int32_t* tickets;
  const int32_t* head_map;
  int32_t v_blocked;
  int32_t act_f32;
  int64_t kv_plane_stride;
} dia_attn_args;
int dia_attn(const dia_attn_args* a, void* stream);
int dia_attn_scratch_floats(int n_rows, int n_kv_heads, int kv_cap);

typedef struct {
  const float* qkv;
  int32_t ldq, q_off, k_off, v_off;
  int32_t heads;
  int32_t rows;
  const int32_t* row_b;
  const int32_t* seg_off;
  const int32_t* seg_len;
  const float* cos_t;
  const float* sin_t;
  void* kp;
  void* vp;
  void* P;
  int64_t p_plane_stride;
  int32_t p_ktiles;
  int32_t _pad0;
} dia_enc_attn_args;
int dia_enc_attn(const dia_enc_attn_args* a, void* stream);

typedef struct {
  const int32_t* row_seg; const int32_t* seg_off; const int32_t* seg_len; const int32_t* seg_row;
  int32_t rows;
  int32_t _pad0;
  const int32_t* tokens;
  int32_t T, C, V, D;
  const float* emb;
  const float* g;
  float* x;
  void* P; int64_t p_plane_stride; int32_t p_ktiles; int32_t ssq_ld;
  float* ssq;
  const float* q;
  int32_t ldq, q_off, k_off, v_off;
  int32_t q_heads, kv_heads, kv_cap;
  int32_t causal;
  void* kc; void* vc;
  const float* cos_t; const float* sin_t;
  const int32_t* text_len;
} dia_dec_prefill_args;
int dia_dec_prefill_embed(const dia_dec_prefill_args* a, void* stream);
int dia_dec_prefill_kv(const dia_dec_prefill_args* a, void* stream);
int dia_dec_prefill_attn(const dia_dec_prefill_args* a, void* stream);

int dia_enc_kv_prep(const float* qkv, int ldq, int k_off, int v_off, int heads, int L, int cap,
                    const float* cos_t, const float* sin_t, float* kc, float* vc, void* stream);

int dia_embed_text(const int32_t* ids, int L, const float* table, int D, const float* g, float* x,
                   void* P, int64_t p_plane_stride, int p_ktiles, float* ssq, int ssq_ld, const int32_t* cmap, void* stream);

typedef struct {
  const int32_t* tokens;
  const int32_t* cur;
// ... 80 lines not shown
  int32_t kt_qkv, ns_qkv, kt_o, ns_o, kt_cq, ns_cq, kt_co, ns_co, kt_wi, ns_wi, kt_wo, ns_wo;
  const int32_t* cmap_ca;
  const int32_t* cmap_mlp;
  const int32_t* cmap_next;
  const int32_t* smap_qkv;
  const int32_t* smap_cq;
  const int32_t* hmap_self;
  const int32_t* hmap_cross;
  const void *w_qkv_24, *w_o_24, *w_cq_24, *w_co_24, *w_wi_24, *w_wo_24;
  const void *w_qkv_f8, *w_o_f8, *w_cq_f8, *w_co_f8, *w_wi_f8, *w_wo_f8;
} dia_dec_layer;

typedef struct {
  int32_t n_layer, D, F, q_heads, kv_heads, cq_heads, C, V;
  int32_t B;
  int32_t T;
  int32_t S;
  int32_t kv_dtype;
  int32_t rows_pad;
  int32_t ld_logits;
  float eps;
  int32_t v_blocked;
  const dia_dec_layer* layers;
  const void* w_logits;
  int32_t kt_logits, ns_logits;
  const float* g_final;
  float* x;
  void* planes_x;
  void* planes_a;
  void* planes_h;
  float* ssq;
  float* qkv;
  float* qc;
  float* logits;
  const float* cos_t;
  const float* sin_t;
  const int32_t* text_len;
  float* sk_scratch;
  int32_t* sk_tickets;
  float* attn_scratch;
  int32_t* attn_tickets;
  int64_t sk_scratch_floats;
  int32_t* mlp_barrier;
  int32_t act_f32;
  int32_t w_planes;
  dia_sample_args sample;
  const void* const* seg_w;
  void* seg_ws;
  int64_t kv_plane_self, kv_plane_cross;
  const void* w_logits_24;
  const void* w_logits_f8;
} dia_engine_desc;

typedef struct dia_engine dia_engine;
int dia_engine_create(const dia_engine_desc* d, void* stream, dia_engine** out);
int dia_engine_destroy(dia_engine* e);
int dia_engine_mlp_fused(const dia_engine* e);
int dia_engine_decode(dia_engine* e, int n_steps, int use_graph);
int dia_engine_set_prefetch(dia_engine* e, int lookahead);
int dia_engine_step_logits_only(dia_engine* e);
int dia_engine_profile_step(dia_engine* e, float* ms_per_launch, int cap);
int dia_engine_time_step(dia_engine* e, float* ms_per_kernel, float* interval_ms, int cap);
const char* dia_timed_kernel_name(int i);
int dia_mxfp8_classes(int rows);
int dia_engine_launches_per_step(const dia_engine* e);

#ifdef __cplusplus
}
#endif
#endif
```

Baseline: 1027 frames/s.

## Fuse cross-attention query projection GEMM with cross-attention into one kernel

Moves the MFMA attention body into a shared header so it can be reused, then adds a fused cq_attn path that runs the cross-query projection GEMM and the cross-attention in a single launch, used when the text length is short (at most 128). The GEMM epilogue gains a coherent atomic-store variant so attention blocks can read the projected queries within the same kernel. This removes one launch per decoder layer and the global round-trip of the query tensor between kernels. In exchange it needs cross-block synchronisation inside the fused kernel and adds profiling code that splits the fused kernel's time back into its two parts.

```diff
diff --git a/dia-tts-prune_amd/csrc/attn.hip b/dia-tts-prune_amd/csrc/attn.hip
--- a/dia-tts-prune_amd/csrc/attn.hip
+++ b/dia-tts-prune_amd/csrc/attn.hip
@@ -3,145 +3,10 @@
 #include "errors.hpp"
 #include "launch.hpp"
 #include "tuning.hpp"
+#include "attn_mfma.hpp"
 #include <cstdlib>
 
 namespace {
-
-constexpr int HD = 128;
-constexpr int NT = 256;
-constexpr int NWV = NT / 64;
-constexpr int U = 4;
-constexpr int UNIT = NWV * 16;
-constexpr int CHUNK = 128;
-constexpr int SLAB = 2 * 8 + 4 * HD;
-
-struct AttnK {
-  int mode, n_kv_heads, n_rows, kv_cap;
-  const float* q; int ldq, q_off, k_off, v_off;
-  void* kc; void* vc;
-  const int* cur; const int* len; int enc_len;
-  const float* cos_t; const float* sin_t;
-  bf16_raw* P; long p_plane_stride; int p_ktiles;
-  float* scratch; int* tickets; int max_chunks;
-  const int* head_map;
-  int v_blocked;
-  int gpw;
-  int act_f32;
-  long kv_plane_stride;
-};
-
-#ifdef DIA_DBG_STAMPS
-__device__ long long g_astamps[8192 * 8];
-#define ASTAMP(i) do { if (threadIdx.x == 0) g_astamps[((blockIdx.z * gridDim.y + blockIdx.y) * gridDim.x + blockIdx.x) * 8 + (i)] = wall_clock64(); } while (0)
-#else
-#define ASTAMP(i) do {} while (0)
-#endif
-
-template <int G>
-__device__ __forceinline__ void attn_finish(const AttnK& p, const float* part, const float* pm_s, const float* pl_s,
-                                            int* last_s_ptr, int tid, int qrow, int kvh, int head_row, int chunk, int nchunks) {
-  int& last_s = *last_s_ptr;
-  const bool o_thread = tid < G * 16;
-  const int og = tid >> 4, od0 = (tid & 15) * 8;
-  float o[8];
-  float M = 0.f, Lsum = 1.f;
-  if (o_thread) {
-    float mm = -INFINITY;
-#pragma unroll
-    for (int ww = 0; ww < NWV; ++ww) mm = fmaxf(mm, pm_s[ww * 8 + og]);
-    float L2 = 0.f;
-#pragma unroll
-    for (int j = 0; j < 8; ++j) o[j] = 0.f;
-#pragma unroll
-    for (int ww = 0; ww < NWV; ++ww) {
-      const float pmw = pm_s[ww * 8 + og];
-      const float f = (pmw == -INFINITY) ? 0.f : expf(pmw - mm);
-      L2 += pl_s[ww * 8 + og] * f;
-#pragma unroll
-      for (int j = 0; j < 8; ++j) o[j] += part[(ww * G + og) * HD + od0 + j] * f;
-    }
-    M = mm; Lsum = L2;
-  }
-
-  if (nchunks > 1) {
-    const long pair = (long)head_row * p.n_kv_heads + kvh;
-    float* slab = p.scratch + (pair * p.max_chunks + chunk) * SLAB;
-    if (o_thread) {
-      if ((tid & 15) == 0) st2_agent(slab + 2 * og, M, Lsum);
-      const __amdgpu_buffer_rsrc_t sr = agent_rsrc(p.scratch);
-      const int so = (int)(((pair * p.max_chunks + chunk) * SLAB + 16 + og * HD + od0) * 4);
-      st4_agent(sr, so, f32x4{o[0], o[1], o[2], o[3]});
-      st4_agent(sr, so + 16, f32x4{o[4], o[5], o[6], o[7]});
-    }
-    asm volatile("s_waitcnt vmcnt(0)" ::: "memory");
-    __syncthreads();
-    if (tid == 0) {
-      const int ticket = __hip_atomic_fetch_add(p.tickets + pair, 1, __ATOMIC_RELAXED, __HIP_MEMORY_SCOPE_AGENT);
-      const int last = ticket == nchunks - 1;
-      if (last) __hip_atomic_store(p.tickets + pair, 0, __ATOMIC_RELAXED, __HIP_MEMORY_SCOPE_AGENT);
-      last_s = last;
-    }
-    __syncthreads();
-    ASTAMP(5);
-    if (!last_s) return;
-    if (o_thread) {
-      const float* base = p.scratch + pair * p.max_chunks * SLAB;
-      const __amdgpu_buffer_rsrc_t sr = agent_rsrc(p.scratch);
-      const int bo = (int)((pair * p.max_chunks * SLAB + 16 + og * HD + od0) * 4);
-      constexpr int MB = 12;
-      float mrun = -INFINITY, L2 = 0.f;
-#pragma unroll
-      for (int j = 0; j < 8; ++j) o[j] = 0.f;
-      for (int c0 = 0; c0 < nchunks; c0 += MB) {
-        float2 ml[MB]; f32x4 oa[MB], ob[MB];
-#pragma unroll
-        for (int u = 0; u < MB; ++u)
-          if (c0 + u < nchunks) {
-            const float* sl = base + (long)(c0 + u) * SLAB;
-            ml[u] = ld2_agent(sl + 2 * og);
-            oa[u] = ld4_agent(sr, bo + (c0 + u) * (SLAB * 4));
-            ob[u] = ld4_agent(sr, bo + (c0 + u) * (SLAB * 4) + 16);
-          }
-        float mm = mrun;
-#pragma unroll
-        for (int u = 0; u < MB; ++u)
-          if (c0 + u < nchunks) mm = fmaxf(mm, ml[u].x);
-        const float fr = (mrun == -INFINITY) ? 0.f : expf(mrun - mm);
-        L2 *= fr;
-#pragma unroll
-        for (int j = 0; j < 8; ++j) o[j] *= fr;
-#pragma unroll
-        for (int u = 0; u < MB; ++u)
-          if (c0 + u < nchunks) {
-            const float f = (ml[u].x != -INFINITY) ? expf(ml[u].x - mm) : 0.f;
-            L2 += ml[u].y * f;
-#pragma unroll
-            for (int j = 0; j < 4; ++j) { o[j] += oa[u][j] * f; o[4 + j] += ob[u][j] * f; }
-          }
-        mrun = mm;
-      }
-      Lsum = L2;
-    }
-  }
-
-  if (o_thread) {
-    const float invl = Lsum > 0.f ? 1.0f / Lsum : 0.f;
-#pragma unroll
-    for (int j = 0; j < 8; ++j) o[j] *= invl;
-    const int hpos = p.head_map ? p.head_map[kvh * G + og] : kvh * G + og;
-    const int col = hpos * HD + od0;
-    auto emit = [&](int row, const float* v8) {
-      if (p.act_f32) emit_f32x8(reinterpret_cast<float*>(p.P), p.p_ktiles, row, col, v8);
-      else emit_planes8(p.P, p.p_plane_stride, p.p_ktiles, row, col, v8);
-    };
-    if (hpos >= 0) emit(qrow, o);
-    if (p.mode == DIA_ATTN_CROSS && hpos >= 0) {
-      const float z[8] = {0.f, 0.f, 0.f, 0.f, 0.f, 0.f, 0.f, 0.f};
-      emit(qrow - 1, z);
-    }
-  }
-  ASTAMP(6);
-}
 
 template <typename KVT, int G>
 __global__ __launch_bounds__(NT) void k_attn(AttnK p) {
@@ -321,21 +186,6 @@
   attn_finish<G>(p, part, pm_s, pl_s, &last_s, tid, qrow, kvh, head_row, chunk, nchunks);
 }
 
-__device__ __forceinline__ float row16_max(float v) {
-  v = fmaxf(v, __builtin_bit_cast(float, __builtin_amdgcn_update_dpp(0, __builtin_bit_cast(int, v), 0xB1, 0xF, 0xF, true)));
-  v = fmaxf(v, __builtin_bit_cast(float, __builtin_amdgcn_update_dpp(0, __builtin_bit_cast(int, v), 0x4E, 0xF, 0xF, true)));
-  v = fmaxf(v, __builtin_bit_cast(float, __builtin_amdgcn_update_dpp(0, __builtin_bit_cast(int, v), 0x141, 0xF, 0xF, true)));
-  v = fmaxf(v, __builtin_bit_cast(float, __builtin_amdgcn_update_dpp(0, __builtin_bit_cast(int, v), 0x140, 0xF, 0xF, true)));
-  return v;
-}
-
-#ifdef DIA_DBG_KV_NT
-#define KVLOAD(ptr) __builtin_nontemporal_load(ptr)
-#else
-#define KVLOAD(ptr) (*(ptr))
-#endif
-template <int G, int PL>
-struct MfmaFrag { bf16x8 kb[PL][2][4]; bf16x8 vb[PL][8]; };
 
 template <int G, int PL = 1>
 __global__ __launch_bounds__(NT, 2) void k_attn_mfma(AttnK p) {
@@ -345,219 +195,9 @@
   __shared__ __attribute__((aligned(16))) bf16_raw pbuf[NWV][2][16][32];
   __shared__ __attribute__((aligned(16))) bf16_raw knew_s[PL][HD], vnew_s[PL][HD];
   __shared__ int last_s;
-
-  const int tid = threadIdx.x, lane = tid & 63, w = tid >> 6;
-  const int kvh = blockIdx.x, chunk = blockIdx.z;
-  const int arow = lane & 15, akq = lane >> 4;
-  ASTAMP(0);
-  const int by = blockIdx.y;
-  const bool is_self = p.mode == DIA_ATTN_SELF;
-  const int qrow = is_self ? by : 2 * by + 1;
-  const float* qr = p.q + (long)qrow * p.ldq;
-  const float* qh = qr + p.q_off + (kvh * G + min(w, G - 1)) * HD;
-  const float* kh = qr + (is_self ? p.k_off : p.q_off) + kvh * HD;
-  const float* vh = qr + (is_self ? p.v_off : p.q_off) + kvh * HD;
-  const float qx1 = qh[lane], qx2 = qh[lane + 64];
-  const float kx1 = kh[lane], kx2 = kh[lane + 64];
-  const float vx1 = vh[lane], vx2 = vh[lane + 64];
-
-  const int c_cur = p.cur[is_self ? (by >> 1) : by];
-  const int c_len = p.len[is_self ? 0 : by];
-  const int kvrow = by, pos = c_cur;
-  const int nkeys = is_self ? c_cur : c_len;
-  const int slot = is_self ? c_cur - 1 : -1;
-  const int head_row = by;
-  const int NZ = gridDim.z;
-  const int ngran = (nkeys + 31) >> 5;
-  const int gpw = (ngran <= 2 * NWV) ? max(p.gpw, 2) : p.gpw;
-  const int nchunks = min(NZ, max(1, (ngran + NWV * gpw - 1) / (NWV * gpw)));
-  if (chunk >= nchunks) return;
-  ASTAMP(1);
-  if (p.head_map) {
-    bool any_live = false;
-#pragma unroll
-    for (int g = 0; g < G; ++g) any_live |= p.head_map[kvh * G + g] >= 0;
-    if (!any_live && !is_self) return;
-  }
-  const float rc = p.cos_t[(long)pos * 64 + lane], rs = p.sin_t[(long)pos * 64 + lane];
-
-  bf16_raw* Kc = reinterpret_cast<bf16_raw*>(p.kc) + ((long)kvrow * p.n_kv_heads + kvh) * p.kv_cap * HD;
-  bf16_raw* Vc = reinterpret_cast<bf16_raw*>(p.vc) + ((long)kvrow * p.n_kv_heads + kvh) * p.kv_cap * HD;
-  const int klast = max(nkeys - 1, 0);
-  const int gstride = NWV * nchunks;
-  const int g_first = chunk * NWV + w;
-  auto load_gran = [&](MfmaFrag<G, PL>& f, int gi) {
-    const int key0 = gi << 5;
-#pragma unroll
-    for (int pl = 0; pl < PL; ++pl) {
-      const bf16_raw* Kp = Kc + pl * p.kv_plane_stride;
-#pragma unroll
-      for (int t = 0; t < 2; ++t)
-#pragma unroll
-        for (int ks = 0; ks < 4; ++ks)
-          f.kb[pl][t][ks] = KVLOAD(reinterpret_cast<const bf16x8*>(Kp + (long)min(key0 + 16 * t + arow, klast) * HD + 32 * ks + 8 * akq));
-    }
-#pragma unroll
-    for (int pl = 0; pl < PL; ++pl) {
-      const bf16_raw* Vblk = Vc + pl * p.kv_plane_stride + (long)gi * HD * 32;
-#pragma unroll
-      for (int nb = 0; nb < 8; ++nb) f.vb[pl][nb] = KVLOAD(reinterpret_cast<const bf16x8*>(Vblk + (long)(16 * nb + arow) * 32 + 8 * akq));
-    }
-  };
-  MfmaFrag<G, PL> fa, fb;
-  const bool have0 = g_first < ngran;
-  load_gran(fa, have0 ? g_first : 0);
-
-  if (w < G) {
-    const float qv[2] = {qx1 * rc - qx2 * rs, qx1 * rs + qx2 * rc};
-#pragma unroll
-    for (int e = 0; e < 2; ++e) {
-      const int D = lane + 64 * e;
-      __bf16 a, b, c;
-      split3(qv[e], a, b, c);
-      qf[D >> 5][0][w][(D >> 3) & 3][D & 7] = *reinterpret_cast<const bf16_raw*>(&a);
-      qf[D >> 5][1][w][(D >> 3) & 3][D & 7] = *reinterpret_cast<const bf16_raw*>(&b);
-      qf[D >> 5][2][w][(D >> 3) & 3][D & 7] = *reinterpret_cast<const bf16_raw*>(&c);
-    }
-  }
-  const int gslot = slot >> 5;
-  const bool owner = slot >= 0 && (gslot % gstride) == g_first;
-  if (owner) {
-    float kv4[4] = {kx1 * rc - kx2 * rs, kx1 * rs + kx2 * rc, vx1, vx2};
-#pragma unroll
-    for (int pl = 0; pl < PL; ++pl) {
-      bf16_raw r4[4];
-#pragma unroll
-      for (int e = 0; e < 4; ++e) {
-        const __bf16 b = (__bf16)kv4[e];
-        r4[e] = *reinterpret_cast<const bf16_raw*>(&b);
-        kv4[e] -= (float)b;
-      }
-      knew_s[pl][lane] = r4[0]; knew_s[pl][lane + 64] = r4[1]; vnew_s[pl][lane] = r4[2]; vnew_s[pl][lane + 64] = r4[3];
-      bf16_raw* Kp = Kc + pl * p.kv_plane_stride;
-      Kp[(long)slot * HD + lane] = r4[0]; Kp[(long)slot * HD + lane + 64] = r4[1];
-      bf16_raw* vdst = Vc + pl * p.kv_plane_stride + (long)gslot * HD * 32 + (slot & 31);
-      vdst[(long)lane * 32] = r4[2]; vdst[(long)(lane + 64) * 32] = r4[3];
-    }
-  }
-  lds_barrier();
-  ASTAMP(2);
-
-  const int qrow_l = min(arow, G - 1);
-  const float scale = 0.08838834764831845f;
-  f32x4 O[8];
-#pragma unroll
-  for (int nb = 0; nb < 8; ++nb) O[nb] = f32x4{0.f, 0.f, 0.f, 0.f};
-  float mrun[4], lrun[4];
-#pragma unroll
-  for (int g = 0; g < 4; ++g) { mrun[g] = -INFINITY; lrun[g] = 0.f; }
-
-  auto consume = [&](MfmaFrag<G, PL>& f, int gi) {
-    const int key0 = gi << 5;
-    if (owner && gi == gslot) {
-      const int ts = (slot >> 4) & 1, ns = slot & 15, js = slot & 7, kqs = (slot & 31) >> 3;
-#pragma unroll
-      for (int pl = 0; pl < PL; ++pl) {
-#pragma unroll
-        for (int ks = 0; ks < 4; ++ks) {
-          const bf16x8 kn = *reinterpret_cast<const bf16x8*>(&knew_s[pl][32 * ks + 8 * akq]);
-#pragma unroll
-          for (int t = 0; t < 2; ++t)
-            if (t == ts && arow == ns) f.kb[pl][t][ks] = kn;
-        }
-#pragma unroll
-        for (int nb = 0; nb < 8; ++nb) {
-          const bf16_raw vr = vnew_s[pl][16 * nb + arow];
-          const __bf16 vn = *reinterpret_cast<const __bf16*>(&vr);
-#pragma unroll
-          for (int j = 0; j < 8; ++j)
-            if (j == js && akq == kqs) f.vb[pl][nb][j] = vn;
-        }
-      }
-    }
-    f32x4 S[2] = {f32x4{0.f, 0.f, 0.f, 0.f}, f32x4{0.f, 0.f, 0.f, 0.f}};
-#pragma unroll
-    for (int ks = 0; ks < 4; ++ks)
-#pragma unroll
-      for (int pl = 0; pl < DIA_NPLANES; ++pl) {
-        const bf16x8 qa = *reinterpret_cast<const bf16x8*>(&qf[ks][pl][qrow_l][akq][0]);
-#pragma unroll
-        for (int kp = 0; kp < PL; ++kp) {
-          if (PL == 2 && (pl + kp > 1)) continue;
-#pragma unroll
-          for (int t = 0; t < 2; ++t)
-            S[t] = __builtin_amdgcn_mfma_f32_16x16x32_bf16(qa, f.kb[kp][t][ks], S[t], 0, 0, 0);
-        }
-      }
-    float alpha[4];
-    const bool v0 = key0 + arow < nkeys, v1 = key0 + 16 + arow < nkeys;
-#pragma unroll
-    for (int g = 0; g < G; ++g) {
-      const float s0 = v0 ? S[0][g] * scale : -INFINITY, s1 = v1 ? S[1][g] * scale : -INFINITY;
-      const float mnew = fmaxf(mrun[g], row16_max(fmaxf(s0, s1)));
-      alpha[g] = (mrun[g] == -INFINITY) ? 0.f : __expf(mrun[g] - mnew);
-      const float p0 = (s0 == -INFINITY) ? 0.f : __expf(s0 - mnew), p1 = (s1 == -INFINITY) ? 0.f : __expf(s1 - mnew);
-      lrun[g] = lrun[g] * alpha[g] + row16_sum(p0 + p1);
-      mrun[g] = mnew;
-      if (lane < 16) {
-        const __bf16 h0 = (__bf16)p0, h1 = (__bf16)p1;
-        const __bf16 l0 = (__bf16)(p0 - (float)h0), l1 = (__bf16)(p1 - (float)h1);
-        pbuf[w][0][g][lane] = *reinterpret_cast<const bf16_raw*>(&h0);
-        pbuf[w][0][g][16 + lane] = *reinterpret_cast<const bf16_raw*>(&h1);
-        pbuf[w][1][g][lane] = *reinterpret_cast<const bf16_raw*>(&l0);
-        pbuf[w][1][g][16 + lane] = *reinterpret_cast<const bf16_raw*>(&l1);
-      }
-    }
-    __builtin_amdgcn_wave_barrier();
-#pragma unroll
-    for (int nb = 0; nb < 8; ++nb)
-#pragma unroll
-      for (int g = 0; g < G; ++g) O[nb][g] *= alpha[g];
-    const bf16x8 pa0 = *reinterpret_cast<const bf16x8*>(&pbuf[w][0][arow][8 * akq]);
-    const bf16x8 pa1 = *reinterpret_cast<const bf16x8*>(&pbuf[w][1][arow][8 * akq]);
-#pragma unroll
-    for (int nb = 0; nb < 8; ++nb)
-#pragma unroll
-      for (int vp = 0; vp < PL; ++vp) {
-        O[nb] = __builtin_amdgcn_mfma_f32_16x16x32_bf16(pa0, f.vb[vp][nb], O[nb], 0, 0, 0);
-        if (vp == 0) O[nb] = __builtin_amdgcn_mfma_f32_16x16x32_bf16(pa1, f.vb[vp][nb], O[nb], 0, 0, 0);
-      }
-    __builtin_amdgcn_wave_barrier();
-  };
-
-  if constexpr (PL == 1) {
-    int gi = g_first;
-    for (; gi + 2 * gstride < ngran; gi += 2 * gstride) {
-      load_gran(fb, gi + gstride);
-      consume(fa, gi);
-      load_gran(fa, gi + 2 * gstride);
-      consume(fb, gi + gstride);
-    }
-    if (gi < ngran) {
-      const int g1 = gi + gstride;
-      if (g1 < ngran) load_gran(fb, g1);
-      consume(fa, gi);
-      if (g1 < ngran) consume(fb, g1);
-    }
-  } else {
-    for (int gi = g_first; gi < ngran; gi += gstride) {
-      if (gi != g_first) load_gran(fa, gi);
-      consume(fa, gi);
-    }
-  }
-  ASTAMP(3);
-  if (lane < 16) {
-#pragma unroll
-    for (int g = 0; g < G; ++g) {
-#pragma unroll
-      for (int nb = 0; nb < 8; ++nb) part[(w * G + g) * HD + 16 * nb + lane] = O[nb][g];
-      if (lane == 0) { pm_s[w * 8 + g] = mrun[g]; pl_s[w * 8 + g] = lrun[g]; }
-    }
-  }
-  __syncthreads();
-  ASTAMP(4);
-  attn_finish<G>(p, part, pm_s, pl_s, &last_s, tid, qrow, kvh, head_row, chunk, nchunks);
-}
+  attn_mfma_body<G, PL, false>(p, qf, part, pm_s, pl_s, pbuf, knew_s, vnew_s, last_s, threadIdx.x, blockIdx.x, blockIdx.y, blockIdx.z, gridDim.z, 0, 0);
+}
+
 
 struct EncAttnK {
   const float* qkv; int ldq, q_off, k_off, v_off, heads, rows;
@@ -827,17 +467,7 @@
   if (max_chunks < 1) max_chunks = 1;
   if (max_chunks > 1 && (!a->scratch || !a->tickets)) return dia_fail(DIA_E_ARG, "dia_attn: more than 128 keys possible: scratch and tickets are required");
   AttnK k;
-  k.mode = a->mode; k.n_kv_heads = a->n_kv_heads; k.n_rows = a->n_rows; k.kv_cap = a->kv_cap;
-  k.q = a->q; k.ldq = a->ldq; k.q_off = a->q_off; k.k_off = a->k_off; k.v_off = a->v_off;
-  k.kc = a->kc; k.vc = a->vc; k.cur = a->cur; k.len = a->len; k.enc_len = a->enc_len;
-  k.cos_t = a->cos_t; k.sin_t = a->sin_t;
-  k.P = (bf16_raw*)a->P; k.p_plane_stride = a->p_plane_stride; k.p_ktiles = a->p_ktiles; k.act_f32 = a->act_f32;
-  k.head_map = a->head_map; k.v_blocked = a->v_blocked;
-  k.gpw = 1;
-  { const int g = dia_tune(a->mode == DIA_ATTN_CROSS ? DIA_TUNE_ATTN_GPW_CROSS : DIA_TUNE_ATTN_GPW); if (g > 0) k.gpw = g; }
-  if (!k.cur) k.cur = reinterpret_cast<const int*>(a->cos_t);
-  if (!k.len) k.len = reinterpret_cast<const int*>(a->cos_t);
-  k.scratch = a->scratch; k.tickets = a->tickets; k.max_chunks = (a->kv_cap + CHUNK - 1) / CHUNK;
+  fill_attnk(a, k);
   if ((a->n_kv_heads * a->group * 128 + 31) / 32 > a->p_ktiles) return dia_fail(DIA_E_ARG, "dia_attn: output planes too narrow");
   hipStream_t st = (hipStream_t)stream;
   const bool f32 = a->kv_dtype == DIA_KV_F32;
diff --git a/dia-tts-prune_amd/csrc/attn_mfma.hpp b/dia-tts-prune_amd/csrc/attn_mfma.hpp
--- /dev/null
+++ b/dia-tts-prune_amd/csrc/attn_mfma.hpp
@@ -0,0 +1,409 @@
+#pragma once
+#include "common.hpp"
+#include "../../include/dia_hip.h"
+#include "tuning.hpp"
+
+namespace {
+
+constexpr int HD = 128;
+constexpr int NT = 256;
+constexpr int NWV = NT / 64;
+constexpr int U = 4;
+constexpr int UNIT = NWV * 16;
+constexpr int CHUNK = 128;
+constexpr int SLAB = 2 * 8 + 4 * HD;
+
+struct AttnK {
+  int mode, n_kv_heads, n_rows, kv_cap;
+  const float* q; int ldq, q_off, k_off, v_off;
+  void* kc; void* vc;
+  const int* cur; const int* len; int enc_len;
+  const float* cos_t; const float* sin_t;
+  bf16_raw* P; long p_plane_stride; int p_ktiles;
+  float* scratch; int* tickets; int max_chunks;
+  const int* head_map;
+  int v_blocked;
+  int gpw;
+  int act_f32;
+  long kv_plane_stride;
+};
+
+inline void fill_attnk(const dia_attn_args* a, AttnK& k) {
+  k.mode = a->mode; k.n_kv_heads = a->n_kv_heads; k.n_rows = a->n_rows; k.kv_cap = a->kv_cap;
+  k.q = a->q; k.ldq = a->ldq; k.q_off = a->q_off; k.k_off = a->k_off; k.v_off = a->v_off;
+  k.kc = a->kc; k.vc = a->vc; k.cur = a->cur; k.len = a->len; k.enc_len = a->enc_len;
+  k.cos_t = a->cos_t; k.sin_t = a->sin_t;
+  k.P = (bf16_raw*)a->P; k.p_plane_stride = a->p_plane_stride; k.p_ktiles = a->p_ktiles; k.act_f32 = a->act_f32;
+  k.head_map = a->head_map; k.v_blocked = a->v_blocked;
+  k.gpw = 1;
+  { const int g = dia_tune(a->mode == DIA_ATTN_CROSS ? DIA_TUNE_ATTN_GPW_CROSS : DIA_TUNE_ATTN_GPW); if (g > 0) k.gpw = g; }
+  if (!k.cur) k.cur = reinterpret_cast<const int*>(a->cos_t);
+  if (!k.len) k.len = reinterpret_cast<const int*>(a->cos_t);
+  k.scratch = a->scratch; k.tickets = a->tickets; k.max_chunks = (a->kv_cap + CHUNK - 1) / CHUNK;
+  k.kv_plane_stride = 0;
+}
+
+#ifdef DIA_DBG_STAMPS
+__device__ long long g_astamps[8192 * 8];
+#define ASTAMP(i) do { if (threadIdx.x == 0) g_astamps[((blockIdx.z * gridDim.y + blockIdx.y) * gridDim.x + blockIdx.x) * 8 + (i)] = wall_clock64(); } while (0)
+#else
+#define ASTAMP(i) do {} while (0)
+#endif
+
+template <int G>
+__device__ __forceinline__ void attn_finish(const AttnK& p, const float* part, const float* pm_s, const float* pl_s,
+                                            int* last_s_ptr, int tid, int qrow, int kvh, int head_row, int chunk, int nchunks) {
+  int& last_s = *last_s_ptr;
+  const bool o_thread = tid < G * 16;
+  const int og = tid >> 4, od0 = (tid & 15) * 8;
+  float o[8];
+  float M = 0.f, Lsum = 1.f;
+  if (o_thread) {
+    float mm = -INFINITY;
+#pragma unroll
+    for (int ww = 0; ww < NWV; ++ww) mm = fmaxf(mm, pm_s[ww * 8 + og]);
+    float L2 = 0.f;
+#pragma unroll
+    for (int j = 0; j < 8; ++j) o[j] = 0.f;
+#pragma unroll
+    for (int ww = 0; ww < NWV; ++ww) {
+      const float pmw = pm_s[ww * 8 + og];
+      const float f = (pmw == -INFINITY) ? 0.f : expf(pmw - mm);
+      L2 += pl_s[ww * 8 + og] * f;
+#pragma unroll
+      for (int j = 0; j < 8; ++j) o[j] += part[(ww * G + og) * HD + od0 + j] * f;
+    }
+    M = mm; Lsum = L2;
+  }
+
+  if (nchunks > 1) {
+    const long pair = (long)head_row * p.n_kv_heads + kvh;
+    float* slab = p.scratch + (pair * p.max_chunks + chunk) * SLAB;
+    if (o_thread) {
+      if ((tid & 15) == 0) st2_agent(slab + 2 * og, M, Lsum);
+      const __amdgpu_buffer_rsrc_t sr = agent_rsrc(p.scratch);
+      const int so = (int)(((pair * p.max_chunks + chunk) * SLAB + 16 + og * HD + od0) * 4);
+      st4_agent(sr, so, f32x4{o[0], o[1], o[2], o[3]});
+      st4_agent(sr, so + 16, f32x4{o[4], o[5], o[6], o[7]});
+    }
+    asm volatile("s_waitcnt vmcnt(0)" ::: "memory");
+    __syncthreads();
+    if (tid == 0) {
+      const int ticket = __hip_atomic_fetch_add(p.tickets + pair, 1, __ATOMIC_RELAXED, __HIP_MEMORY_SCOPE_AGENT);
+      const int last = ticket == nchunks - 1;
+      if (last) __hip_atomic_store(p.tickets + pair, 0, __ATOMIC_RELAXED, __HIP_MEMORY_SCOPE_AGENT);
+      last_s = last;
+    }
+    __syncthreads();
+    ASTAMP(5);
+    if (!last_s) return;
+    if (o_thread) {
+      const float* base = p.scratch + pair * p.max_chunks * SLAB;
+      const __amdgpu_buffer_rsrc_t sr = agent_rsrc(p.scratch);
+      const int bo = (int)((pair * p.max_chunks * SLAB + 16 + og * HD + od0) * 4);
+      constexpr int MB = 12;
+      float mrun = -INFINITY, L2 = 0.f;
+#pragma unroll
+      for (int j = 0; j < 8; ++j) o[j] = 0.f;
+      for (int c0 = 0; c0 < nchunks; c0 += MB) {
+        float2 ml[MB]; f32x4 oa[MB], ob[MB];
+#pragma unroll
+        for (int u = 0; u < MB; ++u)
+          if (c0 + u < nchunks) {
+            const float* sl = base + (long)(c0 + u) * SLAB;
+            ml[u] = ld2_agent(sl + 2 * og);
+            oa[u] = ld4_agent(sr, bo + (c0 + u) * (SLAB * 4));
+            ob[u] = ld4_agent(sr, bo + (c0 + u) * (SLAB * 4) + 16);
+          }
+        float mm = mrun;
+#pragma unroll
+        for (int u = 0; u < MB; ++u)
+          if (c0 + u < nchunks) mm = fmaxf(mm, ml[u].x);
+        const float fr = (mrun == -INFINITY) ? 0.f : expf(mrun - mm);
+        L2 *= fr;
+#pragma unroll
+        for (int j = 0; j < 8; ++j) o[j] *= fr;
+#pragma unroll
+        for (int u = 0; u < MB; ++u)
+          if (c0 + u < nchunks) {
+            const float f = (ml[u].x != -INFINITY) ? expf(ml[u].x - mm) : 0.f;
+            L2 += ml[u].y * f;
+#pragma unroll
+            for (int j = 0; j < 4; ++j) { o[j] += oa[u][j] * f; o[4 + j] += ob[u][j] * f; }
+          }
+        mrun = mm;
+      }
+      Lsum = L2;
+    }
+  }
+
+  if (o_thread) {
+    const float invl = Lsum > 0.f ? 1.0f / Lsum : 0.f;
+#pragma unroll
+    for (int j = 0; j < 8; ++j) o[j] *= invl;
+    const int hpos = p.head_map ? p.head_map[kvh * G + og] : kvh * G + og;
+    const int col = hpos * HD + od0;
+    auto emit = [&](int row, const float* v8) {
+      if (p.act_f32) emit_f32x8(reinterpret_cast<float*>(p.P), p.p_ktiles, row, col, v8);
+      else emit_planes8(p.P, p.p_plane_stride, p.p_ktiles, row, col, v8);
+    };
+    if (hpos >= 0) emit(qrow, o);
+    if (p.mode == DIA_ATTN_CROSS && hpos >= 0) {
+      const float z[8] = {0.f, 0.f, 0.f, 0.f, 0.f, 0.f, 0.f, 0.f};
+      emit(qrow - 1, z);
+    }
+  }
+  ASTAMP(6);
+}
+
+__device__ __forceinline__ float row16_max(float v) {
+  v = fmaxf(v, __builtin_bit_cast(float, __builtin_amdgcn_update_dpp(0, __builtin_bit_cast(int, v), 0xB1, 0xF, 0xF, true)));
+  v = fmaxf(v, __builtin_bit_cast(float, __builtin_amdgcn_update_dpp(0, __builtin_bit_cast(int, v), 0x4E, 0xF, 0xF, true)));
+  v = fmaxf(v, __builtin_bit_cast(float, __builtin_amdgcn_update_dpp(0, __builtin_bit_cast(int, v), 0x141, 0xF, 0xF, true)));
+  v = fmaxf(v, __builtin_bit_cast(float, __builtin_amdgcn_update_dpp(0, __builtin_bit_cast(int, v), 0x140, 0xF, 0xF, true)));
+  return v;
+}
+
+#ifdef DIA_DBG_KV_NT
+#define KVLOAD(ptr) __builtin_nontemporal_load(ptr)
+#else
+#define KVLOAD(ptr) (*(ptr))
+#endif
+template <int G, int PL>
+struct MfmaFrag { bf16x8 kb[PL][2][4]; bf16x8 vb[PL][8]; };
+
+template <int G, int PL>
+struct AttnMfmaSmem {
+  __attribute__((aligned(16))) bf16_raw qf[4][DIA_NPLANES][G][4][8];
+  float part[NWV * G * HD];
+  float pm_s[NWV * 8], pl_s[NWV * 8];
+  __attribute__((aligned(16))) bf16_raw pbuf[NWV][2][16][32];
+  __attribute__((aligned(16))) bf16_raw knew_s[PL][HD], vnew_s[PL][HD];
+  int last_s;
+};
+
+template <int G, int PL, bool FUSED>
+__device__ __forceinline__ void attn_mfma_body(const AttnK& p, bf16_raw (&qf)[4][DIA_NPLANES][G][4][8], float (&part)[NWV * G * HD],
+                                               float (&pm_s)[NWV * 8], float (&pl_s)[NWV * 8], bf16_raw (&pbuf)[NWV][2][16][32],
+                                               bf16_raw (&knew_s)[PL][HD], bf16_raw (&vnew_s)[PL][HD], int& last_s,
+                                               const int tid, const int kvh, const int by, const int chunk, const int NZ,
+                                               int c_cur_pre, int c_len_pre) {
+
+  const int lane = tid & 63, w = tid >> 6;
+  const int arow = lane & 15, akq = lane >> 4;
+  ASTAMP(0);
+  const bool is_self = !FUSED && p.mode == DIA_ATTN_SELF;
+  const int qrow = is_self ? by : 2 * by + 1;
+  const float* qr = p.q + (long)qrow * p.ldq;
+  const float* qh = qr + p.q_off + (kvh * G + min(w, G - 1)) * HD;
+  const float* kh = qr + (is_self ? p.k_off : p.q_off) + kvh * HD;
+  const float* vh = qr + (is_self ? p.v_off : p.q_off) + kvh * HD;
+  float qx1, qx2, kx1 = 0.f, kx2 = 0.f, vx1 = 0.f, vx2 = 0.f;
+  int c_cur, c_len;
+  if constexpr (FUSED) {
+    qx1 = __hip_atomic_load(qh + lane, __ATOMIC_RELAXED, __HIP_MEMORY_SCOPE_AGENT);
+    qx2 = __hip_atomic_load(qh + lane + 64, __ATOMIC_RELAXED, __HIP_MEMORY_SCOPE_AGENT);
+    c_cur = c_cur_pre; c_len = c_len_pre;
+  } else {
+    qx1 = qh[lane]; qx2 = qh[lane + 64];
+    kx1 = kh[lane]; kx2 = kh[lane + 64];
+    vx1 = vh[lane]; vx2 = vh[lane + 64];
+    c_cur = p.cur[is_self ? (by >> 1) : by];
+    c_len = p.len[is_self ? 0 : by];
+  }
+  const int kvrow = by, pos = c_cur;
+  const int nkeys = is_self ? c_cur : c_len;
+  const int slot = is_self ? c_cur - 1 : -1;
+  const int head_row = by;
+  const int ngran = (nkeys + 31) >> 5;
+  const int gpw = (ngran <= 2 * NWV) ? max(p.gpw, 2) : p.gpw;
+  const int nchunks = min(NZ, max(1, (ngran + NWV * gpw - 1) / (NWV * gpw)));
+  if (chunk >= nchunks) return;
+  ASTAMP(1);
+  if (p.head_map) {
+    bool any_live = false;
+#pragma unroll
+    for (int g = 0; g < G; ++g) any_live |= p.head_map[kvh * G + g] >= 0;
+    if (!any_live && !is_self) return;
+  }
+  const float rc = p.cos_t[(long)pos * 64 + lane], rs = p.sin_t[(long)pos * 64 + lane];
+
+  bf16_raw* Kc = reinterpret_cast<bf16_raw*>(p.kc) + ((long)kvrow * p.n_kv_heads + kvh) * p.kv_cap * HD;
+  bf16_raw* Vc = reinterpret_cast<bf16_raw*>(p.vc) + ((long)kvrow * p.n_kv_heads + kvh) * p.kv_cap * HD;
+  const int klast = max(nkeys - 1, 0);
+  const int gstride = NWV * nchunks;
+  const int g_first = chunk * NWV + w;
+  auto load_gran = [&](MfmaFrag<G, PL>& f, int gi) {
+    const int key0 = gi << 5;
+#pragma unroll
+    for (int pl = 0; pl < PL; ++pl) {
+      const bf16_raw* Kp = Kc + pl * p.kv_plane_stride;
+#pragma unroll
+      for (int t = 0; t < 2; ++t)
+#pragma unroll
+        for (int ks = 0; ks < 4; ++ks)
+          f.kb[pl][t][ks] = KVLOAD(reinterpret_cast<const bf16x8*>(Kp + (long)min(key0 + 16 * t + arow, klast) * HD + 32 * ks + 8 * akq));
+    }
+#pragma unroll
+    for (int pl = 0; pl < PL; ++pl) {
+      const bf16_raw* Vblk = Vc + pl * p.kv_plane_stride + (long)gi * HD * 32;
+#pragma unroll
+      for (int nb = 0; nb < 8; ++nb) f.vb[pl][nb] = KVLOAD(reinterpret_cast<const bf16x8*>(Vblk + (long)(16 * nb + arow) * 32 + 8 * akq));
+    }
+  };
+  MfmaFrag<G, PL> fa, fb;
+  const bool have0 = g_first < ngran;
+  load_gran(fa, have0 ? g_first : 0);
+
+  if (w < G) {
+    const float qv[2] = {qx1 * rc - qx2 * rs, qx1 * rs + qx2 * rc};
+#pragma unroll
+    for (int e = 0; e < 2; ++e) {
+      const int D = lane + 64 * e;
+      __bf16 a, b, c;
+      split3(qv[e], a, b, c);
+      qf[D >> 5][0][w][(D >> 3) & 3][D & 7] = *reinterpret_cast<const bf16_raw*>(&a);
+      qf[D >> 5][1][w][(D >> 3) & 3][D & 7] = *reinterpret_cast<const bf16_raw*>(&b);
+      qf[D >> 5][2][w][(D >> 3) & 3][D & 7] = *reinterpret_cast<const bf16_raw*>(&c);
+    }
+  }
+  const int gslot = slot >> 5;
+  const bool owner = slot >= 0 && (gslot % gstride) == g_first;
+  if (owner) {
+    float kv4[4] = {kx1 * rc - kx2 * rs, kx1 * rs + kx2 * rc, vx1, vx2};
+#pragma unroll
+    for (int pl = 0; pl < PL; ++pl) {
+      bf16_raw r4[4];
+#pragma unroll
+      for (int e = 0; e < 4; ++e) {
+        const __bf16 b = (__bf16)kv4[e];
+        r4[e] = *reinterpret_cast<const bf16_raw*>(&b);
+        kv4[e] -= (float)b;
+      }
+      knew_s[pl][lane] = r4[0]; knew_s[pl][lane + 64] = r4[1]; vnew_s[pl][lane] = r4[2]; vnew_s[pl][lane + 64] = r4[3];
+      bf16_raw* Kp = Kc + pl * p.kv_plane_stride;
+      Kp[(long)slot * HD + lane] = r4[0]; Kp[(long)slot * HD + lane + 64] = r4[1];
+      bf16_raw* vdst = Vc + pl * p.kv_plane_stride + (long)gslot * HD * 32 + (slot & 31);
+      vdst[(long)lane * 32] = r4[2]; vdst[(long)(lane + 64) * 32] = r4[3];
+    }
+  }
+  lds_barrier();
+  ASTAMP(2);
+
+  const int qrow_l = min(arow, G - 1);
+  const float scale = 0.08838834764831845f;
+  f32x4 O[8];
+#pragma unroll
+  for (int nb = 0; nb < 8; ++nb) O[nb] = f32x4{0.f, 0.f, 0.f, 0.f};
+  float mrun[4], lrun[4];
+#pragma unroll
+  for (int g = 0; g < 4; ++g) { mrun[g] = -INFINITY; lrun[g] = 0.f; }
+
+  auto consume = [&](MfmaFrag<G, PL>& f, int gi) {
+    const int key0 = gi << 5;
+    if (owner && gi == gslot) {
+      const int ts = (slot >> 4) & 1, ns = slot & 15, js = slot & 7, kqs = (slot & 31) >> 3;
+#pragma unroll
+      for (int pl = 0; pl < PL; ++pl) {
+#pragma unroll
+        for (int ks = 0; ks < 4; ++ks) {
+          const bf16x8 kn = *reinterpret_cast<const bf16x8*>(&knew_s[pl][32 * ks + 8 * akq]);
+#pragma unroll
+          for (int t = 0; t < 2; ++t)
+            if (t == ts && arow == ns) f.kb[pl][t][ks] = kn;
+        }
+#pragma unroll
+        for (int nb = 0; nb < 8; ++nb) {
+          const bf16_raw vr = vnew_s[pl][16 * nb + arow];
+          const __bf16 vn = *reinterpret_cast<const __bf16*>(&vr);
+#pragma unroll
+          for (int j = 0; j < 8; ++j)
+            if (j == js && akq == kqs) f.vb[pl][nb][j] = vn;
+        }
+      }
+    }
+    f32x4 S[2] = {f32x4{0.f, 0.f, 0.f, 0.f}, f32x4{0.f, 0.f, 0.f, 0.f}};
+#pragma unroll
+    for (int ks = 0; ks < 4; ++ks)
+#pragma unroll
+      for (int pl = 0; pl < DIA_NPLANES; ++pl) {
+        const bf16x8 qa = *reinterpret_cast<const bf16x8*>(&qf[ks][pl][qrow_l][akq][0]);
+#pragma unroll
+        for (int kp = 0; kp < PL; ++kp) {
+          if (PL == 2 && (pl + kp > 1)) continue;
+#pragma unroll
+          for (int t = 0; t < 2; ++t)
+            S[t] = __builtin_amdgcn_mfma_f32_16x16x32_bf16(qa, f.kb[kp][t][ks], S[t], 0, 0, 0);
+        }
+      }
+    float alpha[4];
+    const bool v0 = key0 + arow < nkeys, v1 = key0 + 16 + arow < nkeys;
+#pragma unroll
+    for (int g = 0; g < G; ++g) {
+      const float s0 = v0 ? S[0][g] * scale : -INFINITY, s1 = v1 ? S[1][g] * scale : -INFINITY;
+      const float mnew = fmaxf(mrun[g], row16_max(fmaxf(s0, s1)));
+      alpha[g] = (mrun[g] == -INFINITY) ? 0.f : __expf(mrun[g] - mnew);
+      const float p0 = (s0 == -INFINITY) ? 0.f : __expf(s0 - mnew), p1 = (s1 == -INFINITY) ? 0.f : __expf(s1 - mnew);
+      lrun[g] = lrun[g] * alpha[g] + row16_sum(p0 + p1);
+      mrun[g] = mnew;
+      if (lane < 16) {
+        const __bf16 h0 = (__bf16)p0, h1 = (__bf16)p1;
+        const __bf16 l0 = (__bf16)(p0 - (float)h0), l1 = (__bf16)(p1 - (float)h1);
+        pbuf[w][0][g][lane] = *reinterpret_cast<const bf16_raw*>(&h0);
+        pbuf[w][0][g][16 + lane] = *reinterpret_cast<const bf16_raw*>(&h1);
+        pbuf[w][1][g][lane] = *reinterpret_cast<const bf16_raw*>(&l0);
+        pbuf[w][1][g][16 + lane] = *reinterpret_cast<const bf16_raw*>(&l1);
+      }
+    }
+    __builtin_amdgcn_wave_barrier();
+#pragma unroll
+    for (int nb = 0; nb < 8; ++nb)
+#pragma unroll
+      for (int g = 0; g < G; ++g) O[nb][g] *= alpha[g];
+    const bf16x8 pa0 = *reinterpret_cast<const bf16x8*>(&pbuf[w][0][arow][8 * akq]);
+    const bf16x8 pa1 = *reinterpret_cast<const bf16x8*>(&pbuf[w][1][arow][8 * akq]);
+#pragma unroll
+    for (int nb = 0; nb < 8; ++nb)
+#pragma unroll
+      for (int vp = 0; vp < PL; ++vp) {
+        O[nb] = __builtin_amdgcn_mfma_f32_16x16x32_bf16(pa0, f.vb[vp][nb], O[nb], 0, 0, 0);
+        if (vp == 0) O[nb] = __builtin_amdgcn_mfma_f32_16x16x32_bf16(pa1, f.vb[vp][nb], O[nb], 0, 0, 0);
+      }
+    __builtin_amdgcn_wave_barrier();
+  };
+
+  if constexpr (PL == 1) {
+    int gi = g_first;
+    for (; gi + 2 * gstride < ngran; gi += 2 * gstride) {
+      load_gran(fb, gi + gstride);
+      consume(fa, gi);
+      load_gran(fa, gi + 2 * gstride);
+      consume(fb, gi + gstride);
+    }
+    if (gi < ngran) {
+      const int g1 = gi + gstride;
+      if (g1 < ngran) load_gran(fb, g1);
+      consume(fa, gi);
+      if (g1 < ngran) consume(fb, g1);
+    }
+  } else {
+    for (int gi = g_first; gi < ngran; gi += gstride) {
+      if (gi != g_first) load_gran(fa, gi);
+      consume(fa, gi);
+    }
+  }
+  ASTAMP(3);
+  if (lane < 16) {
+#pragma unroll
+    for (int g = 0; g < G; ++g) {
+#pragma unroll
+      for (int nb = 0; nb < 8; ++nb) part[(w * G + g) * HD + 16 * nb + lane] = O[nb][g];
+      if (lane == 0) { pm_s[w * 8 + g] = mrun[g]; pl_s[w * 8 + g] = lrun[g]; }
+    }
+  }
+  __syncthreads();
+  ASTAMP(4);
+  attn_finish<G>(p, part, pm_s, pl_s, &last_s, tid, qrow, kvh, head_row, chunk, nchunks);
+}
+
+}
diff --git a/dia-tts-prune_amd/csrc/engine.hip b/dia-tts-prune_amd/csrc/engine.hip
--- a/dia-tts-prune_amd/csrc/engine.hip
+++ b/dia-tts-prune_amd/csrc/engine.hip
@@ -18,6 +18,8 @@
   bool seg = false;
   std::vector<const void*> seg_w;
   int mlp_fused = -1;
+  bool cq_attn = false;
+  int max_text_len = 0;
   std::vector<hipEvent_t> prof;
   int pf_lookahead = 0;
   bool pf_capturing = false;
@@ -140,7 +142,7 @@
   g.w_planes = d.w_planes;
   sparse24(g, L.w_cq_24);
   mxfp8(g, L.w_cq_f8, 2);
-  if ((rc = dia_gemm(&g, st))) return rc; mark(e, n++);
+  if (!e->cq_attn) { if ((rc = dia_gemm(&g, st))) return rc; mark(e, n++); }
 
     a = {};
     a.mode = DIA_ATTN_CROSS; a.kv_dtype = d.kv_dtype; a.n_kv_heads = d.cq_heads; a.group = 1;
@@ -150,7 +152,8 @@
     a.cos_t = d.cos_t; a.sin_t = d.sin_t; a.P = d.planes_a; a.p_plane_stride = as; a.p_ktiles = akt;
     a.scratch = d.attn_scratch; a.tickets = d.attn_tickets;
     a.act_f32 = F;
-    if ((rc = dia_attn(&a, st))) return rc; mark(e, n++);
+    if (e->cq_attn) { a.enc_len = e->max_text_len; if ((rc = dia_cq_attn(&g, &a, st))) return rc; mark(e, n++); }
+    else { if ((rc = dia_attn(&a, st))) return rc; mark(e, n++); }
 
     if (seg) {
       dia_seg_args sa = {};
@@ -295,6 +298,26 @@
   return DIA_OK;
 }
 
+extern "C" int dia_engine_set_max_text_len(dia_engine* e, int max_text_len) {
+  if (!e || max_text_len < 0) return dia_fail(DIA_E_ARG, "dia_engine_set_max_text_len: bad argument");
+  if (e->exec) return dia_fail(DIA_E_STATE, "dia_engine_set_max_text_len: the step graph is already captured");
+  e->max_text_len = max_text_len;
+  const dia_engine_desc* d = &e->d;
+  {
+    const int R = 2 * d->B;
+    bool ok = dia_tune(DIA_TUNE_CQ_ATTN) != 0 && (R == 2 || R == 4) && d->kv_dtype == DIA_KV_BF16 && d->v_blocked && d->w_planes <= 1 && !e->seg &&
+              dia_tune(DIA_TUNE_WO_DIAG) != 1 && max_text_len > 0 && max_text_len <= DIA_CQ_ATTN_XL && max_text_len <= d->S && d->S % 32 == 0 &&
+              d->D == 2048;
+    const int f8 = (d->act_f32 && d->w_planes <= 1) ? dia_mxfp8_classes(R) : 0;
+    for (int l = 0; l < d->n_layer && ok; ++l) {
+      const dia_dec_layer& L = e->layers[l];
+      ok = L.kt_cq == 64 && L.ns_cq == d->cq_heads * 8 && !L.smap_cq && !L.hmap_cross && !(L.w_cq_24 && d->act_f32) && !(L.w_cq_f8 && (f8 >> 2 & 1));
+    }
+    e->cq_attn = ok;
+  }
+  return DIA_OK;
+}
+
 extern "C" int dia_engine_destroy(dia_engine* e) {
   if (!e) return DIA_OK;
   hipError_t he = hipSuccess;
@@ -329,7 +352,7 @@
         const dia_dec_layer& L = e->layers[l];
         auto add = [&](const void* w, int kt, int ns) { e->pf_w.push_back({w, (long)kt * ns * 1024}); };
         add(L.w_qkv, L.kt_qkv, L.ns_qkv); e->pf_w.push_back({nullptr, 0});
-        add(L.w_o, L.kt_o, L.ns_o); add(L.w_cq, L.kt_cq, L.ns_cq); e->pf_w.push_back({nullptr, 0});
+        add(L.w_o, L.kt_o, L.ns_o); add(L.w_cq, L.kt_cq, L.ns_cq); if (!e->cq_attn) e->pf_w.push_back({nullptr, 0});
         add(L.w_co, L.kt_co, L.ns_co); add(L.w_wi, L.kt_wi, L.ns_wi); add(L.w_wo, L.kt_wo, L.ns_wo);
       }
       e->pf_w.push_back({d.w_logits, (long)d.kt_logits * d.ns_logits * 1024});
@@ -418,9 +441,11 @@
 
 extern "C" int dia_engine_mlp_fused(const dia_engine* e) { return e && e->mlp_fused == 1; }
 
+extern "C" int dia_engine_cq_attn(const dia_engine* e) { return e && e->cq_attn; }
+
 extern "C" int dia_engine_launches_per_step(const dia_engine* e) {
   if (!e) return dia_fail(DIA_E_ARG, "null engine");
-  return e->seg ? e->d.n_layer * 5 + 3 : e->d.n_layer * 8 + 2;
+  return e->seg ? e->d.n_layer * 5 + 3 : e->d.n_layer * (e->cq_attn ? 7 : 8) + 2;
 }
 
 __global__ __launch_bounds__(256) void k_prefetch(const uint4* __restrict__ p, long n16, unsigned* sink) {
diff --git a/dia-tts-prune_amd/csrc/gemm.hip b/dia-tts-prune_amd/csrc/gemm.hip
--- a/dia-tts-prune_amd/csrc/gemm.hip
+++ b/dia-tts-prune_amd/csrc/gemm.hip
@@ -1,5 +1,6 @@
 #include "gemm_common.hpp"
 #include "gemm_experiments.hpp"
+#include "attn_mfma.hpp"
 
 namespace {
 
@@ -108,12 +109,42 @@
   run_epilogue(p, tile + (e_mt * 16 + e_r) * 17, inv_s[e_mt * 16 + e_r], m, n0, half, strip, live, xpre, gpre);
 }
 
-
-template <int NW, int KPW, int RS, bool MULTI, bool AF32 = false, bool PF32 = false, bool W2 = false>
+__device__ __forceinline__ void cq_attn_head(const AttnK& ap, int& strip, int& c_cur, int& c_len) {
+  strip = (blockIdx.x % ap.n_kv_heads) * 8 + blockIdx.x / ap.n_kv_heads;
+  const int by = min((int)(threadIdx.x >> 8), ap.n_rows - 1);
+  c_cur = ap.cur[by]; c_len = ap.len[by];
+}
+template <int RS>
+__device__ __forceinline__ void cq_attn_tail(const AttnK& ap, int tid, int c_cur, int c_len) {
+  __shared__ AttnMfmaSmem<1, 1> sm[RS / 2];
+  __shared__ int last_s;
+  const int head = blockIdx.x % ap.n_kv_heads, team = tid >> 8;
+  asm volatile("s_waitcnt vmcnt(0)" ::: "memory");
+  __syncthreads();
+  if (tid == 0) {
+    const int ticket = __hip_atomic_fetch_add(ap.tickets + head, 1, __ATOMIC_RELAXED, __HIP_MEMORY_SCOPE_AGENT);
+    const int last = ticket == 7;
+    if (last) __hip_atomic_store(ap.tickets + head, 0, __ATOMIC_RELAXED, __HIP_MEMORY_SCOPE_AGENT);
+    last_s = last;
+  }
+  __syncthreads();
+  STAMP(6);
+  if (!last_s || team >= ap.n_rows) return;
+  AttnMfmaSmem<1, 1>& s = sm[team];
+  attn_mfma_body<1, 1, true>(ap, s.qf, s.part, s.pm_s, s.pl_s, s.pbuf, s.knew_s, s.vnew_s, s.last_s, tid & 255, head, team, 0, 1, c_cur, c_len);
+  STAMP(7);
+}
+
+
+template <int NW, int KPW, int RS, bool MULTI, bool AF32 = false, bool PF32 = false, bool W2 = false, typename... FA>
 __global__ __launch_bounds__(NW * 64) void k_gemv_small(const bf16_raw* a_A, long a_aps, const bf16_raw* a_W, int a_KT, int a_M, int a_epi,
-                                                        int a_nstrips, float* a_out, int a_ldo, const float* a_gnext, GemmK p) {
+                                                        int a_nstrips, float* a_out, int a_ldo, const float* a_gnext, GemmK p, FA... fa) {
+  constexpr bool CQA = sizeof...(FA) > 0;
+  static_assert(!CQA || (NW == 8 && KPW == 8 && !MULTI && !W2 && AF32 == PF32), "the fold rides the cq form only");
   p.A = a_A; p.a_plane_stride = a_aps; p.W = a_W; p.KT = a_KT; p.M = a_M; p.epi = a_epi; p.nstrips = a_nstrips;
   p.out = a_out; p.ldo = a_ldo; p.gnext = a_gnext;
+  int cq_s = 0, cq_cur = 0, cq_len = 0;
+  if constexpr (CQA) cq_attn_head(fa..., cq_s, cq_cur, cq_len);
   extern __shared__ __attribute__((aligned(16))) unsigned char smem_raw[];
   f32x4* red = reinterpret_cast<f32x4*>(smem_raw);
   float* tile = reinterpret_cast<float*>(smem_raw + sizeof(f32x4) * NW * 64);
@@ -190,6 +221,8 @@
   if (resid && r_thread) load_resid(blockIdx.x);
   __builtin_amdgcn_sched_barrier(0);
 #ifndef DIA_X_WFIRST
+  if constexpr (CQA) load_strip(b0, cq_s);
+  else
   load_strip(b0, blockIdx.x);
   __builtin_amdgcn_sched_barrier(0);
 #endif
@@ -261,7 +294,7 @@
       if (r_thread) v = tile[(tid >> 4) * 17 + (tid & 15)];
     }
     if (r_thread) {
-      run_epilogue_rows<RS, PF32>(p, v, inv_s, tid, strip, xpre1, gpre1);
+      run_epilogue_rows<RS, PF32, CQA>(p, v, inv_s, tid, strip, xpre1, gpre1);
       if (MULTI && next < p.nstrips && resid) load_resid(next);
     }
   };
@@ -272,6 +305,10 @@
       body(b1, b0, strip + G);
     }
     if (strip < p.nstrips) body(b0, b1, strip);
+  } else if constexpr (CQA) {
+    body(b0, b1, cq_s);
+    STAMP(5);
+    cq_attn_tail<RS>(fa..., tid, cq_cur, cq_len);
   } else {
     body(b0, b1, blockIdx.x);
   }
@@ -2001,6 +2038,36 @@
   return launch_generic(k, nw, st);
 }
 
+extern "C" int dia_cq_attn(const dia_gemm_args* g, const dia_attn_args* a, void* stream) {
+  if (!g || !a || !g->A || !g->W || !g->out || !a->q || !a->kc || !a->vc || !a->P || !a->cos_t || !a->sin_t || !a->cur || !a->len || !a->tickets)
+    return dia_fail(DIA_E_ARG, "dia_cq_attn: null argument (tickets: n_kv_heads int32, zero before the first launch)");
+  if (g->epi != DIA_EPI_SCALE_STORE || g->w_format != DIA_W_DENSE || g->w_planes > 1 || g->w_layout != 0 || g->sp_blocks || g->sp_toff ||
+      g->cmap || g->strip_map || g->sk > 1 || g->spw > 1 || (g->nw != 0 && g->nw != 8) || (g->act_f32 & ~1))
+    return dia_fail(DIA_E_ARG, "dia_cq_attn: the projection must be a dense one-plane SCALE_STORE GEMV without maps or split-K");
+  if ((g->M != 2 && g->M != 4) || g->KT != 64 || g->a_ktiles < g->KT || g->nstrips <= 0 || g->nstrips % 8 != 0 || g->ldo < g->nstrips * 16 ||
+      g->a_plane_stride % 8 != 0 || (g->ssq_in && g->ssq_ld < 16))
+    return dia_fail(DIA_E_ARG, "dia_cq_attn: 2 or 4 rows, K = 2048, whole heads of 8 strips, ldo covering them");
+  if (a->mode != DIA_ATTN_CROSS || a->kv_dtype != DIA_KV_BF16 || !a->v_blocked || a->group != 1 || a->head_map || a->kv_cap <= 0 || a->kv_cap % 32 != 0)
+    return dia_fail(DIA_E_ARG, "dia_cq_attn: CROSS mode over bf16 K/V with blocked V, group 1, no head map, kv_cap % 32 == 0");
+  if (a->n_rows * 2 != g->M || a->n_kv_heads * 8 != g->nstrips || a->q != g->out || a->ldq != g->ldo || a->q_off != 0)
+    return dia_fail(DIA_E_ARG, "dia_cq_attn: the attention must read the projection's output (rows = 2 x utterances, heads = strips / 8)");
+  if (a->enc_len < 0 || a->enc_len > a->kv_cap) return dia_fail(DIA_E_ARG, "dia_cq_attn: enc_len (the longest text, when stated) exceeds kv_cap");
+  if (a->p_plane_stride % 8 != 0 || (a->n_kv_heads * 128 + 31) / 32 > a->p_ktiles) return dia_fail(DIA_E_ARG, "dia_cq_attn: output planes too narrow");
+  GemmK k;
+  fill_gemmk(g, k);
+  AttnK ak;
+  fill_attnk(a, ak);
+  const int rs = g->M <= 2 ? 2 : 4;
+  const size_t smem = small_smem(8, 64, rs);
+  const dim3 grid(g->nstrips), blk(512);
+  hipStream_t st = (hipStream_t)stream;
+#define DIA_CQ_ATTN_LAUNCH(RS, F) dia_launch<k_gemv_small<8, 8, RS, false, F, F, false, AttnK>>(grid, blk, smem, st, k.A, k.a_plane_stride, k.W, k.KT, k.M, k.epi, k.nstrips, k.out, k.ldo, k.gnext, k, ak)
+  if (k.a_f32) { if (rs == 2) DIA_CQ_ATTN_LAUNCH(2, true); else DIA_CQ_ATTN_LAUNCH(4, true); }
+  else { if (rs == 2) DIA_CQ_ATTN_LAUNCH(2, false); else DIA_CQ_ATTN_LAUNCH(4, false); }
+#undef DIA_CQ_ATTN_LAUNCH
+  return dia_check_launch("k_gemv_small (cq + cross-attention)");
+}
+
 extern "C" int dia_gemm_timed(const dia_gemm_args* a, void* stream, float* ms_out) {
   if (!ms_out) return dia_fail(DIA_E_ARG, "dia_gemm_timed: null output");
   dia_recorder_arm();
diff --git a/dia-tts-prune_amd/csrc/gemm_common.hpp b/dia-tts-prune_amd/csrc/gemm_common.hpp
--- a/dia-tts-prune_amd/csrc/gemm_common.hpp
+++ b/dia-tts-prune_amd/csrc/gemm_common.hpp
@@ -207,7 +207,7 @@
 #define DIA_ROW_SHR(v, n) __builtin_bit_cast(float, __builtin_amdgcn_update_dpp(0, __builtin_bit_cast(int, (v)), 0x110 + (n), 0xF, 0xF, true))
 #define DIA_ROW_SHL(v, n) __builtin_bit_cast(float, __builtin_amdgcn_update_dpp(0, __builtin_bit_cast(int, (v)), 0x100 + (n), 0xF, 0xF, true))
 
-template <int RS, bool PF32 = false>
+template <int RS, bool PF32 = false, bool COH = false>
 __device__ __forceinline__ void run_epilogue_rows(const GemmK& p, float v_tile, const float* inv_s, int tid, int strip,
                                                   float xpre1, float gpre1) {
   const int m = tid >> 4, c = tid & 15;
@@ -259,6 +259,8 @@
   } else {
     if (!live) return;
     const int s_out = p.strip_map ? p.strip_map[strip] : strip;
+    if constexpr (COH) __hip_atomic_store(p.out + (long)m * p.ldo + s_out * 16 + c, v_tile * inv_s[m], __ATOMIC_RELAXED, __HIP_MEMORY_SCOPE_AGENT);
+    else
     p.out[(long)m * p.ldo + s_out * 16 + c] = v_tile * inv_s[m];
   }
 }
diff --git a/dia-tts-prune_amd/csrc/tuning.cpp b/dia-tts-prune_amd/csrc/tuning.cpp
--- a/dia-tts-prune_amd/csrc/tuning.cpp
+++ b/dia-tts-prune_amd/csrc/tuning.cpp
@@ -7,9 +7,9 @@
 #include <string>
 
 static const char* const k_names[DIA_TUNE_COUNT] = {
-    "attn_nz", "attn_gpw", "attn_gpw_cross", "gemm_spw", "gemm_mz_max", "tile_min_blocks", "wo_sk", "wo_pair", "wo_nw", "wo_spw", "act_f32", "wo_diag", "gemm_2t", "gemm_zr", "seg", "seg_nb", "seg_dbg", "seg_sleep", "g2t_wgs", "ckv_merge", "mxfp8",
+    "attn_nz", "attn_gpw", "attn_gpw_cross", "gemm_spw", "gemm_mz_max", "tile_min_blocks", "wo_sk", "wo_pair", "wo_nw", "wo_spw", "act_f32", "wo_diag", "gemm_2t", "gemm_zr", "seg", "seg_nb", "seg_dbg", "seg_sleep", "g2t_wgs", "ckv_merge", "mxfp8", "cq_attn",
     "mlp_fuse", "tile_v", "blk32_kr", "blk32_ws", "no_g32", "g32_all", "g32m"};
-static int g_tune[DIA_TUNE_COUNT] = {-1, -1, -1, -1, -1, -1, -1, -1, -1, -1, -1, -1, -1, -1, -1, -1, -1, -1, -1, -1, -1, -1, -1, -1, -1, -1, -1};
+static int g_tune[DIA_TUNE_COUNT] = {-1, -1, -1, -1, -1, -1, -1, -1, -1, -1, -1, -1, -1, -1, -1, -1, -1, -1, -1, -1, -1, -1, -1, -1, -1, -1, -1, -1};
 
 int dia_tune(int id) {
   dia_tuning_init_from_env();
diff --git a/dia-tts-prune_amd/csrc/tuning.hpp b/dia-tts-prune_amd/csrc/tuning.hpp
--- a/dia-tts-prune_amd/csrc/tuning.hpp
+++ b/dia-tts-prune_amd/csrc/tuning.hpp
@@ -22,6 +22,7 @@
   DIA_TUNE_G2T_WGS,
   DIA_TUNE_CKV_MERGE,
   DIA_TUNE_MXFP8,
+  DIA_TUNE_CQ_ATTN,
   DIA_TUNE_MLP_FUSE,
   DIA_TUNE_TILE_V,
   DIA_TUNE_BLK32_KR,
diff --git a/dia-tts-prune_amd/dia_hip/binding.py b/dia-tts-prune_amd/dia_hip/binding.py
--- a/dia-tts-prune_amd/dia_hip/binding.py
+++ b/dia-tts-prune_amd/dia_hip/binding.py
@@ -13,11 +13,12 @@
 EPI_SCALE_STORE, EPI_RESID_EMIT, EPI_SWIGLU_EMIT, EPI_CROSSKV = 0, 1, 2, 3
 W_DENSE, W_SPARSE24, W_MXFP8 = 0, 1, 2
 ATTN_SELF, ATTN_CROSS, ATTN_ENC = 0, 1, 2
+CQ_ATTN_XL = 128
 
 EXPORTS = (
-    "dia_last_error", "dia_abi_version", "dia_device_count", "dia_set_tuning", "dia_get_tuning", "dia_has_experiments", "dia_gemm", "dia_gemm_timed", "dia_mlp_fused", "dia_mlp_fused_timed", "dia_engine_mlp_fused", "dia_attn", "dia_attn_scratch_floats", "dia_enc_kv_prep", "dia_enc_attn", "dia_dec_prefill_embed", "dia_dec_prefill_kv", "dia_dec_prefill_attn",
+    "dia_last_error", "dia_abi_version", "dia_device_count", "dia_set_tuning", "dia_get_tuning", "dia_has_experiments", "dia_gemm", "dia_gemm_timed", "dia_mlp_fused", "dia_mlp_fused_timed", "dia_engine_mlp_fused", "dia_attn", "dia_cq_attn", "dia_attn_scratch_floats", "dia_enc_kv_prep", "dia_enc_attn", "dia_dec_prefill_embed", "dia_dec_prefill_kv", "dia_dec_prefill_attn",
     "dia_embed_text", "dia_embed_tokens", "dia_sample", "dia_prefetch", "dia_engine_create", "dia_engine_destroy",
-    "dia_engine_decode", "dia_engine_set_prefetch", "dia_engine_step_logits_only", "dia_engine_profile_step", "dia_engine_time_step", "dia_timed_kernel_name", "dia_engine_launches_per_step", "dia_mxfp8_classes",
+    "dia_engine_decode", "dia_engine_set_prefetch", "dia_engine_step_logits_only", "dia_engine_profile_step", "dia_engine_time_step", "dia_timed_kernel_name", "dia_engine_launches_per_step", "dia_engine_set_max_text_len", "dia_engine_cq_attn", "dia_mxfp8_classes",
     "dia_seg_mlp", "dia_seg_workspace_bytes", "dia_seg_workspace_control_bytes", "dia_seg_slots", "dia_seg_supported", "dia_seg_error",
 )
 
@@ -190,6 +191,9 @@
     L.dia_mlp_fused_timed.argtypes = [C.POINTER(GemmArgs), C.POINTER(GemmArgs), C.c_void_p, C.c_void_p, C.POINTER(C.c_float)]
     L.dia_engine_mlp_fused.argtypes = [C.c_void_p]
     L.dia_attn.argtypes = [C.POINTER(AttnArgs), C.c_void_p]
+    L.dia_cq_attn.argtypes = [C.POINTER(GemmArgs), C.POINTER(AttnArgs), C.c_void_p]
+    L.dia_engine_cq_attn.argtypes = [C.c_void_p]
+    L.dia_engine_set_max_text_len.argtypes = [C.c_void_p, C.c_int]
     L.dia_attn_scratch_floats.argtypes = [C.c_int, C.c_int, C.c_int]
     L.dia_enc_attn.argtypes = [C.POINTER(EncAttnArgs), C.c_void_p]
     for fn in (L.dia_dec_prefill_embed, L.dia_dec_prefill_kv, L.dia_dec_prefill_attn):
diff --git a/dia-tts-prune_amd/dia_hip/engine.py b/dia-tts-prune_amd/dia_hip/engine.py
--- a/dia-tts-prune_amd/dia_hip/engine.py
+++ b/dia-tts-prune_amd/dia_hip/engine.py
@@ -616,6 +616,7 @@
         self._desc = ed
         hb.check(hb.lib().dia_engine_create(C.byref(ed), C.c_void_p(self.stream.cuda_stream), C.byref(self._engine)),
                  "dia_engine_create")
+        hb.check(hb.lib().dia_engine_set_max_text_len(self._engine, max(self.lens + [0])), "dia_engine_set_max_text_len")
 
     def close(self):
         if self._engine:
@@ -837,10 +838,33 @@
         self.ensure_noise(self._issued + 1)
         hb.check(hb.lib().dia_engine_profile_step(self._engine, buf, n), "dia_engine_profile_step")
         self._issued += 1
-        return np.array(buf[:], dtype=np.float64)
+        return self._unfold_cq_attn(np.array(buf[:], dtype=np.float64))[0]
 
     def launches_per_step(self) -> int:
         return int(hb.lib().dia_engine_launches_per_step(self._engine))
+
+    @property
+    def cq_attn(self) -> bool:
+        return bool(hb.lib().dia_engine_cq_attn(self._engine))
+
+    def _unfold_cq_attn(self, per_launch: np.ndarray, names: Optional[List[str]] = None):
+        nl = self.cfg.model.decoder.n_layer
+        if not self.cq_attn or len(per_launch) != 7 * nl + 2:
+            return per_launch, names
+        kvb = 2 if self.kv_code == hb.KV_BF16 else 4
+        kv = 2 * self.cfg.model.decoder.cross_query_heads * HEAD_DIM * kvb * sum(self.lens)
+        out, out_names = [], []
+        for l, L in enumerate(self.w.dec_layers):
+            v = list(per_launch[7 * l: 7 * l + 7])
+            share = kv / float(kv + L["cq"].nbytes)
+            out += v[:3] + [v[3] * (1.0 - share), v[3] * share] + v[4:]
+            if names is not None:
+                nm = names[7 * l: 7 * l + 7]
+                out_names += nm[:4] + [nm[3]] + nm[4:]
+        out += list(per_launch[7 * nl:])
+        if names is not None:
+            out_names += names[7 * nl:]
+        return np.array(out, dtype=np.float64), (out_names if names is not None else None)
 
     def seg_error(self) -> int:
         if not self.seg:
@@ -855,9 +879,10 @@
         if got < 0:
             hb.check(got, "dia_engine_time_step")
         self._issued += 1
-        self.last_kernel_names = [hb.lib().dia_timed_kernel_name(i).decode() for i in range(got)]
-        self.last_intervals_ms = np.array(ivl[:got], dtype=np.float64)
-        return np.array(buf[:got], dtype=np.float64)
+        names = [hb.lib().dia_timed_kernel_name(i).decode() for i in range(got)]
+        self.last_intervals_ms, _ = self._unfold_cq_attn(np.array(ivl[:got], dtype=np.float64))
+        ms, self.last_kernel_names = self._unfold_cq_attn(np.array(buf[:got], dtype=np.float64), names)
+        return ms
 
     def sync(self):
         self.stream.synchronize()
diff --git a/include/dia_hip.h b/include/dia_hip.h
--- a/include/dia_hip.h
+++ b/include/dia_hip.h
@@ -130,6 +130,7 @@
   int64_t kv_plane_stride;
 } dia_attn_args;
 int dia_attn(const dia_attn_args* a, void* stream);
+int dia_cq_attn(const dia_gemm_args* g, const dia_attn_args* a, void* stream);
 int dia_attn_scratch_floats(int n_rows, int n_kv_heads, int kv_cap);
 
 typedef struct {
@@ -316,6 +317,8 @@
   const void* w_logits_f8;
 } dia_engine_desc;
 
+#define DIA_CQ_ATTN_XL 128
+
 typedef struct dia_engine dia_engine;
 int dia_engine_create(const dia_engine_desc* d, void* stream, dia_engine** out);
 int dia_engine_destroy(dia_engine* e);
@@ -327,6 +330,8 @@
 int dia_engine_time_step(dia_engine* e, float* ms_per_kernel, float* interval_ms, int cap);
 const char* dia_timed_kernel_name(int i);
 int dia_mxfp8_classes(int rows);
+int dia_engine_set_max_text_len(dia_engine* e, int max_text_len);
+int dia_engine_cq_attn(const dia_engine* e);
 int dia_engine_launches_per_step(const dia_engine* e);
 
 #ifdef __cplusplus
```

After: 1016 frames/s. 1.1% lower.
